# imkaywu/MVSKit

Measured on AMD Instinct MI355X. Metric: patches/s (propagate+optim iteration), 12-view 1080p, higher is better.
Workload: dtype f32

## Files before the change

mvskit_amd/csrc/mvs_engine.cpp:

```cpp
#include <hip/hip_runtime.h>
#include <dlfcn.h>
#include <rccl/rccl.h>

#include <algorithm>
#include <climits>
#include <cmath>
#include <cstdio>
#include <cstdlib>
#include <cstring>
#include <string>
#include <vector>

#include "mvskit_engine.h"
#include "mvs_kernels.h"
#include "mvs_types.h"

static_assert(sizeof(mvs_patch) == sizeof(DPatch), "mvs_patch and DPatch must be the same bytes");
static_assert((MVS_LISTCAP == 16 || MVS_LISTCAP == 32 || MVS_LISTCAP == 64) && MVS_LISTCAP <= MVS_MAXI && MVS_MAX_IMAGES == MVS_MAXI, "limits out of sync");

namespace {
thread_local std::string g_err;

#define HIPCHK(expr)                                                                                       \
    do {                                                                                                   \
        hipError_t _e = (expr);                                                                            \
        if (_e != hipSuccess) {                                                                            \
            g_err = std::string(#expr) + ": " + hipGetErrorString(_e);                                     \
            return MVS_ERR_HIP;                                                                            \
        }                                                                                                  \
    } while (0)

template <typename T> struct DevBuf {
    T* p = nullptr;
    int64_t cap = 0;
    bool headroom = false;
    DevBuf() = default;
    DevBuf(const DevBuf&) = delete;
    DevBuf(DevBuf&& o) noexcept : p(o.p), cap(o.cap), headroom(o.headroom) { o.p = nullptr; o.cap = 0; }
    ~DevBuf() { release(); }
    void swap(DevBuf& o) { std::swap(p, o.p); std::swap(cap, o.cap); }
    int ensure(int64_t n) {
        if (n <= cap) return MVS_OK;
        const int64_t exact = std::max<int64_t>(n, 16);
        int64_t want = (p && headroom) ? exact + exact / 2 : exact;
        T* q = nullptr;
        hipError_t e = hipMalloc((void**)&q, (size_t)want * sizeof(T));
        if (e != hipSuccess && want > exact) { (void)hipGetLastError(); want = exact; e = hipMalloc((void**)&q, (size_t)want * sizeof(T)); }
        if (e != hipSuccess && p) {
            (void)hipGetLastError();
            (void)hipFree(p); p = nullptr; cap = 0;
            e = hipMalloc((void**)&q, (size_t)want * sizeof(T));
        }
        if (e != hipSuccess) { (void)hipGetLastError(); g_err = std::string("hipMalloc: ") + hipGetErrorString(e); return MVS_ERR_HIP; }
        if (p) (void)hipFree(p);
        p = q; cap = want;
        return MVS_OK;
    }
    void release() { if (p) (void)hipFree(p); p = nullptr; cap = 0; }
};

namespace misc {
constexpr int stage_counter = 0;
constexpr int fill_evals = 1;
constexpr int neighbor_retry = 4;
constexpr int sweep_retry = 5;
constexpr int geo_bad = 6;
constexpr int group_edges = 7;
constexpr int trim_parts = 8;
constexpr int trim_nparts = 256;
constexpr int words = trim_parts + trim_nparts;
}
namespace fstat {
constexpr int neighbor_parts = 0;
constexpr int neighbor_cycles = 4096;
constexpr int exact_evals = 4112;
constexpr int words = exact_evals + 2048;
}

struct Rccl {
    void* h = nullptr;
    ncclResult_t (*GetUniqueId)(ncclUniqueId*) = nullptr;
    ncclResult_t (*CommInitRank)(ncclComm_t*, int, ncclUniqueId, int) = nullptr;
    ncclResult_t (*CommDestroy)(ncclComm_t) = nullptr;
    ncclResult_t (*CommCount)(const ncclComm_t, int*) = nullptr;
    ncclResult_t (*CommUserRank)(const ncclComm_t, int*) = nullptr;
    ncclResult_t (*AllGather)(const void*, void*, size_t, ncclDataType_t, ncclComm_t, hipStream_t) = nullptr;
    ncclResult_t (*Broadcast)(const void*, void*, size_t, ncclDataType_t, int, ncclComm_t, hipStream_t) = nullptr;
    ncclResult_t (*GroupStart)() = nullptr;
    ncclResult_t (*GroupEnd)() = nullptr;
    const char* (*GetErrorString)(ncclResult_t) = nullptr;
    bool ok = false;
};
Rccl& rccl() {
    static Rccl r;
    static bool tried = false;
    if (tried) return r;
    tried = true;
    if (const char* over = getenv("MVS_CCL_LIBRARY")) {
        if (*over) { r.h = dlopen(over, RTLD_NOW | RTLD_LOCAL); if (!r.h) return r; }
    }
    const char* names[] = {"librccl.so", "librccl.so.1"};
    for (const char* n : names) if (!r.h) r.h = dlopen(n, RTLD_NOW | RTLD_NOLOAD);
    const char* paths[] = {"/opt/rocm/lib/librccl.so.1", "librccl.so.1", "librccl.so"};
    for (const char* n : paths) if (!r.h) r.h = dlopen(n, RTLD_NOW | RTLD_LOCAL);
    if (!r.h) return r;
#define MVS_SYM(field, name) r.field = reinterpret_cast<decltype(r.field)>(dlsym(r.h, name))
    MVS_SYM(GetUniqueId, "ncclGetUniqueId"); MVS_SYM(CommInitRank, "ncclCommInitRank"); MVS_SYM(CommDestroy, "ncclCommDestroy");
    MVS_SYM(AllGather, "ncclAllGather"); MVS_SYM(Broadcast, "ncclBroadcast"); MVS_SYM(GroupStart, "ncclGroupStart");
    MVS_SYM(GroupEnd, "ncclGroupEnd"); MVS_SYM(GetErrorString, "ncclGetErrorString");
    MVS_SYM(CommCount, "ncclCommCount"); MVS_SYM(CommUserRank, "ncclCommUserRank");
#undef MVS_SYM
    r.ok = r.GetUniqueId && r.CommInitRank && r.CommDestroy && r.AllGather && r.Broadcast && r.GroupStart && r.GroupEnd && r.GetErrorString;
    return r;
}
#define NCCLCHK(expr)                                                                                      \
    do {                                                                                                   \
        ncclResult_t _r = (expr);                                                                          \
        if (_r != ncclSuccess) {                                                                           \
            g_err = std::string(#expr) + ": " + rccl().GetErrorString(_r);                                 \
            return MVS_ERR_HIP;                                                                            \
        }                                                                                                  \
    } while (0)

struct Roctx {
    int (*push)(const char*) = nullptr;
    int (*pop)() = nullptr;
};
Roctx& roctx() {
    static Roctx r;
    static bool tried = false;
    if (tried) return r;
    tried = true;
    void* h = nullptr;
    const char* names[] = {"libroctx64.so", "libroctx64.so.4", "/opt/rocm/lib/libroctx64.so.4"};
    for (const char* n : names) if (!h) h = dlopen(n, RTLD_NOW | RTLD_NOLOAD);
    for (const char* n : names) if (!h) h = dlopen(n, RTLD_NOW | RTLD_LOCAL);
    if (!h) return r;
    r.push = reinterpret_cast<int (*)(const char*)>(dlsym(h, "roctxRangePushA"));
    r.pop = reinterpret_cast<int (*)()>(dlsym(h, "roctxRangePop"));
    if (!r.push || !r.pop) { r.push = nullptr; r.pop = nullptr; }
    return r;
}
struct Range {
    bool on;
    explicit Range(const char* name) : on(roctx().push != nullptr) { if (on) roctx().push(name); }
    ~Range() { if (on) roctx().pop(); }
    Range(const Range&) = delete;
    Range& operator=(const Range&) = delete;
};
}

struct mvs_engine {
    mvs_config cfg{};
    mvs_refiner refiner{MVS_REFINE_HALVING, 500, 1e-4f};
    DParams prm{};
    hipStream_t stream = nullptr;
    bool have_views = false;
    std::vector<DView> hviews;
    DevBuf<DView> dviews;
    std::vector<DevBuf<uint32_t>> img_bufs;
    std::vector<DevBuf<uint8_t>> mask_bufs;
    int total_cells = 0;
    DevBuf<DPatch> pool, pool_alt;
    DevBuf<uint8_t> kill;
    int64_t pool_n = 0;
    bool ncc_dirty = false;
    DevBuf<int32_t> cnt, cursor, vcnt, vcursor;
    DevBuf<csr_off_t> start, vstart;
    DevBuf<csr_off_t> start_raw;
    DevBuf<int32_t> id32_raw;
    DevBuf<int64_t> scan_tmp;
    DevBuf<unsigned long long> ids;
    DevBuf<ListKey> key;
    DevBuf<int32_t> id32, vid32;
    DevBuf<int32_t> uf_parent, uf_size;
    DevBuf<int32_t> group_edges;
    DevBuf<int32_t> cnt_alive, vcnt_alive;
    DevBuf<unsigned long long> dpgrid, best;
    DevBuf<uint32_t> dirty;
    bool dirty_marked = false;
    DevBuf<float4> geo;
    DevBuf<uint8_t> geo_ref;
    bool geo_valid = false;
    bool lists_dense[2] = {false, false};
    DevBuf<DPatch> staging;
    DevBuf<int32_t> job_stage, job_nstage, job_cnt, job_base_scan, kill_cnt, kill_base;
    DevBuf<unsigned long long> misc;
    DevBuf<DCounters> counters;
    DevBuf<int32_t> error_flag;
    DevBuf<int32_t> big_tables, retry_jobs;
    int64_t retried_cells = 0;
    int64_t pass_retried = 0;
    SweepArgs sa{};
    bool staged = false;
    bool counted = false;
    int64_t n_new = 0, n_kill = 0;
    std::vector<int32_t> h_per_view;
    DevBuf<DPatch> tmp_rec_in, tmp_rec_out;
    DevBuf<float> tmp_f_in, tmp_f_out;
    DevBuf<int32_t> tmp_i;
    DevBuf<uint8_t> tmp_bytes;
    hipEvent_t ev[6] = {nullptr, nullptr, nullptr, nullptr, nullptr, nullptr};
    mvs_timing timing{};
    mvs_filter_stats fstats{};
    int64_t fstats_exchange_bytes = 0;
    DevBuf<unsigned long long> fstat_buf;
    hipEvent_t fev[10] = {nullptr, nullptr, nullptr, nullptr, nullptr, nullptr, nullptr, nullptr, nullptr, nullptr};
    ncclComm_t comm = nullptr;
    bool comm_owned = false;
    int comm_rank = 0, comm_world = 1;
    DevBuf<int64_t> comm_counts;
    DevBuf<int32_t> comm_kill_ids;
    int pass_status = MVS_OK;
    std::string pass_error;
    bool fault_fired = false;
};

namespace {

RefineSel refine_sel(const mvs_engine* e) {
    return RefineSel{e->refiner.mode == MVS_REFINE_CONVERGED ? 1 : 0, e->refiner.max_evals, e->refiner.xtol};
}

void derive_params(mvs_engine* e) {
    const mvs_config& c = e->cfg;
    DParams& p = e->prm;
    p.nviews = c.nviews; p.level = c.level; p.csize = c.csize; p.wsize = c.wsize; p.wsz = c.wsize * c.wsize;
    p.minImageNum = c.minImageNum;
    p.tau = std::min(c.minImageNum * 2, c.nviews);
    p.max_propag = c.max_propag;
    p.cap = c.max_propag * c.csize * c.csize;
    p.depth = c.depth; p.enable_check = c.enable_check; p.view_propagation = c.view_propagation ? 1 : 0;
    p.seed = c.seed; p.refine_steps = c.refine_steps; p.rd0 = c.refine_rd0; p.ra0 = c.refine_ra0;
    p.nccThreshold = c.nccThreshold;
    p.nccThresholdBefore = c.nccThreshold - 0.3f;
    volatile float a0 = (float)(60.0f * M_PI / 180.0f), a1 = (float)(60.0f * M_PI / 180.0f);
    volatile double amin = (double)c.maxAngleThreshold, amax = (double)a1;
    volatile float typo = (float)(120.0f / M_PI * 180.0f);
    volatile double d120 = 120.0f * M_PI / 180.0f, d10 = 10.0f * M_PI / 180.0f;
    p.cosAngle0 = cosf(a0);
    p.cosAngle1 = cosf(a1);
    p.cosMinAngle = (float)cos(amin);
    p.cosMaxAngle = (float)cos(amax);
    p.cosNeighborTypo = cosf(typo);
    p.cosNeighbor120 = (float)cos(d120);
    p.sortThreshold = (float)(1.0f - cos(d10));
    p.ascaleConst = (float)(M_PI / 48.0f);
    p.inv_sz = 1.0f / (float)(c.wsize * c.wsize);
    p.inv_3sz = 1.0f / (float)(3 * c.wsize * c.wsize);
    p.neighborThreshold = 0.5f; p.neighborThreshold1 = 1.0f;
    p.quadThreshold = c.quadThreshold;
    p.list_n = std::min<int>(MVS_LISTCAP, c.nviews);
    p.gram_ld = (p.list_n + 15) / 16 * 16;
}

void invert3(const float* P, float* Minv) {
    double a = P[0], b = P[1], c = P[2], d = P[4], e = P[5], f = P[6], g = P[8], h = P[9], i = P[10];
    double A = e * i - f * h, B = -(d * i - f * g), C = d * h - e * g;
    double det = a * A + b * B + c * C;
    double inv[9] = {A, -(b * i - c * h), b * f - c * e, B, a * i - c * g, -(a * f - c * d), C, -(a * h - b * g), a * e - b * d};
    for (int k = 0; k < 9; ++k) Minv[k] = (float)(inv[k] / det);
}
inline float hfma(float a, float b, float c) { return __builtin_fmaf(a, b, c); }
inline float hdot3(const float* a, const float* b) { return hfma(a[2], b[2], hfma(a[1], b[1], a[0] * b[0])); }
inline float hdot4(const float* a, const float* b) { return hfma(a[3], b[3], hfma(a[2], b[2], hfma(a[1], b[1], a[0] * b[0]))); }
inline void hcross(const float* a, const float* b, float* o) {
    o[0] = a[1] * b[2] - a[2] * b[1]; o[1] = a[2] * b[0] - a[0] * b[2]; o[2] = a[0] * b[1] - a[1] * b[0];
}

void setup_camera(const mvs_engine* e, DView& vw, const float* P0) {
    const int maxLevel = e->cfg.level + 3;
    for (int k = 0; k < 12; ++k) vw.P[0][k] = P0[k];
    for (int l = 1; l < maxLevel; ++l) {
        for (int k = 0; k < 12; ++k) vw.P[l][k] = vw.P[l - 1][k];
        for (int k = 0; k < 8; ++k) vw.P[l][k] /= 2.0f;
    }
    invert3(vw.P[e->cfg.level], vw.Minv);
    const float* r2 = &vw.P[0][8];
    const float n = sqrtf(hdot3(r2, r2));
    for (int k = 0; k < 4; ++k) vw.oaxis[k] = r2[k] / n;
    {
        const float* P = vw.P[0];
        double a = P[0], b = P[1], c = P[2], d = P[4], ee = P[5], f = P[6], g = P[8], h = P[9], i = P[10];
        double A = ee * i - f * h, B = -(d * i - f * g), C = d * h - ee * g;
        double det = a * A + b * B + c * C;
        double inv[9] = {A, -(b * i - c * h), b * f - c * ee, B, a * i - c * g, -(a * f - c * d), C, -(a * h - b * g), a * ee - b * d};
        double q[3] = {P[3], P[7], P[11]};
        vw.center[0] = (float)(-(inv[0] * q[0] + inv[1] * q[1] + inv[2] * q[2]) / det);
        vw.center[1] = (float)(-(inv[3] * q[0] + inv[4] * q[1] + inv[5] * q[2]) / det);
        vw.center[2] = (float)(-(inv[6] * q[0] + inv[7] * q[1] + inv[8] * q[2]) / det);
        vw.center[3] = 1.0f;
    }
    for (int k = 0; k < 3; ++k) vw.zaxis[k] = vw.oaxis[k];
    float xa[3] = {vw.P[0][0], vw.P[0][1], vw.P[0][2]};
    hcross(vw.zaxis, xa, vw.yaxis);
    const float yn = sqrtf(hdot3(vw.yaxis, vw.yaxis));
    for (int k = 0; k < 3; ++k) vw.yaxis[k] /= yn;
    hcross(vw.yaxis, vw.zaxis, vw.xaxis);
    const float x4[4] = {vw.xaxis[0], vw.xaxis[1], vw.xaxis[2], 0.0f}, y4[4] = {vw.yaxis[0], vw.yaxis[1], vw.yaxis[2], 0.0f};
    vw.ipscale = hdot4(&vw.P[0][0], x4) + hdot4(&vw.P[0][4], y4);
}

DParams current_params(mvs_engine* e) {
    DParams p = e->prm;
    p.views = e->dviews.p;
    p.pool = e->pool.p;
    p.pool_n = e->pool_n;
    p.total_cells = e->total_cells;
    p.csr_start = e->start.p; p.csr_cnt = e->cnt_alive.p; p.csr_key = e->key.p; p.csr_id32 = e->id32.p;
    p.vcsr_start = e->vstart.p; p.vcsr_cnt = e->vcnt_alive.p; p.vcsr_id32 = e->vid32.p;
    p.dpgrid = e->dpgrid.p;
    p.geo = e->geo_valid ? e->geo.p : nullptr;
    p.geo_ref = e->geo_valid ? e->geo_ref.p : nullptr;
    return p;
}

bool want_vgrid(const mvs_engine* e) { return e->prm.depth >= 2 && e->prm.enable_check; }

int build_list(mvs_engine* e, bool vgrid, bool trim, bool unordered = false) {
    hipStream_t st = e->stream;
    const int64_t nc = e->total_cells;
    DParams p = current_params(e);
    DevBuf<int32_t>& cnt = vgrid ? e->vcnt : e->cnt;
    DevBuf<csr_off_t>& start = vgrid ? e->vstart : e->start;
    DevBuf<int32_t>& cursor = vgrid ? e->vcursor : e->cursor;
    DevBuf<unsigned long long>& ids = e->ids;
    DevBuf<int32_t>& id32 = vgrid ? e->vid32 : e->id32;
    DevBuf<int32_t>& cnt_alive = vgrid ? e->vcnt_alive : e->cnt_alive;
    HIPCHK(hipMemsetAsync(cnt.p, 0, (size_t)(nc + 1) * sizeof(int32_t), st));
    mvsk_index_count(p, vgrid ? nullptr : cnt.p, vgrid ? cnt.p : nullptr, nullptr, st);
    const bool direct = unordered && !trim;
    DevBuf<csr_off_t>& raw = e->start_raw;
    csr_off_t* const first_scan = direct ? start.p : raw.p;
    mvsk_exclusive_scan_off(cnt.p, first_scan, nc, reinterpret_cast<csr_off_t*>(e->scan_tmp.p), st);
    csr_off_t tot64 = 0;
    HIPCHK(hipMemcpyAsync(&tot64, first_scan + nc, sizeof tot64, hipMemcpyDeviceToHost, st));
    HIPCHK(hipStreamSynchronize(st));
    const int64_t tot = (int64_t)tot64;
    if (!unordered) { if (int r = ids.ensure(tot + 16)) return r; }
    if (!vgrid && !unordered) { if (int r = e->key.ensure(tot + 16)) return r; }
    if (int r = id32.ensure(tot + 16)) return r;
    p = current_params(e);
    HIPCHK(hipMemsetAsync(cursor.p, 0, (size_t)(nc + 1) * sizeof(int32_t), st));
    if (direct) {
        mvsk_index_fill_direct(p, vgrid ? 1 : 0, start.p, cursor.p, id32.p, st);
        cnt.swap(cnt_alive);
        e->lists_dense[vgrid ? 1 : 0] = true;
        return MVS_OK;
    }
    if (int r = e->id32_raw.ensure(tot + 16)) return r;
    mvsk_index_fill(p, vgrid ? 1 : 0, raw.p, cursor.p, ids.p, st);
    mvsk_index_sort_trim(p, raw.p, ids.p, trim ? 1 : 0, e->misc.p + misc::trim_parts, st);
    mvsk_index_finalize(p, vgrid ? 1 : 0, raw.p, ids.p, e->id32_raw.p, cnt_alive.p, st);
    mvsk_exclusive_scan_off(cnt_alive.p, start.p, nc, reinterpret_cast<csr_off_t*>(e->scan_tmp.p), st);
    mvsk_index_pack(p, raw.p, start.p, cnt_alive.p, ids.p, e->id32_raw.p, vgrid ? nullptr : e->key.p, id32.p, st);
    e->lists_dense[vgrid ? 1 : 0] = true;
    return MVS_OK;
}
int build_depth(mvs_engine* e) {
    const DParams p = current_params(e);
    HIPCHK(hipMemsetAsync(e->dpgrid.p, 0xff, (size_t)e->total_cells * sizeof(unsigned long long), e->stream));
    mvsk_depth_maps(p, e->dpgrid.p, nullptr, e->stream);
    return MVS_OK;
}
int build_index(mvs_engine* e, unsigned long long* trimmed_out) {
    hipStream_t st = e->stream;
    const DParams p = current_params(e);
    HIPCHK(hipMemsetAsync(e->misc.p + misc::fill_evals, 0, 2 * sizeof(unsigned long long), st));
    HIPCHK(hipMemsetAsync(e->misc.p + misc::trim_parts, 0, misc::trim_nparts * sizeof(unsigned long long), st));
    mvsk_fill_ncc(p, e->misc.p + misc::fill_evals, st);
    e->ncc_dirty = false;
    if (int r = build_list(e, false, true)) return r;
    if (want_vgrid(e)) if (int r = build_list(e, true, false, true)) return r;
    if (int r = build_depth(e)) return r;
    if (trimmed_out) {
        unsigned long long part[misc::trim_nparts];
        HIPCHK(hipMemcpyAsync(part, e->misc.p + misc::trim_parts, sizeof part, hipMemcpyDeviceToHost, st));
        HIPCHK(hipStreamSynchronize(st));
        *trimmed_out = 0;
        for (unsigned long long v : part) *trimmed_out += v;
    }
    HIPCHK(hipGetLastError());
    return MVS_OK;
}
void filter_range(const mvs_engine* e, int64_t& first, int64_t& last) {
    first = 0; last = e->pool_n;
    if (e->comm && e->comm_world > 1) {
        first = e->pool_n * e->comm_rank / e->comm_world;
        last = e->pool_n * (e->comm_rank + 1) / e->comm_world;
    }
}
struct FilterRun {
    mvs_engine* e;
    int local = MVS_OK;
    std::string err;
    int agreed = MVS_OK;
    bool multi() const { return e->comm && e->comm_world > 1; }
    bool live() const { return local == MVS_OK && agreed == MVS_OK; }
    void note(int r) { if (r != MVS_OK && local == MVS_OK) { local = r; err = g_err; } }
};
#define FR(expr) do { if (fr.live()) fr.note(expr); } while (0)
int hip_status(hipError_t e, const char* what) {
    if (e == hipSuccess) return MVS_OK;
    g_err = std::string(what) + ": " + hipGetErrorString(e);
    return MVS_ERR_HIP;
}
#define FRHIP(expr) FR(hip_status((expr), #expr))
#ifdef MVS_FAULT_INJECTION
void filter_fault_point(FilterRun& fr, int point) {
    const char* f = getenv("MVS_FAULT_FILTER");
    int r = -1, p = -1;
    if (f && fr.live() && sscanf(f, "%d:%d", &r, &p) == 2 && r == fr.e->comm_rank && p == point) {
        g_err = "mvs_engine_filter: failure injected by MVS_FAULT_FILTER";
        fr.note(MVS_ERR_CAPACITY);
    }
}
#else
inline void filter_fault_point(FilterRun&, int) {}
#endif
int filter_agree(FilterRun& fr) {
    mvs_engine* e = fr.e;
    if (fr.agreed != MVS_OK) return fr.agreed;
    if (!fr.multi()) {
        if (fr.local != MVS_OK) { fr.agreed = fr.local; g_err = fr.err; }
        return fr.agreed;
    }
    const int64_t mine = fr.local;
    std::vector<int64_t> all((size_t)e->comm_world, 0);
    hipStream_t st = e->stream;
    if (hipMemcpyAsync(e->comm_counts.p, &mine, sizeof mine, hipMemcpyHostToDevice, st) != hipSuccess ||
        rccl().AllGather(e->comm_counts.p, e->comm_counts.p + 1, 1, ncclInt64, e->comm, st) != ncclSuccess ||
        hipMemcpyAsync(all.data(), e->comm_counts.p + 1, all.size() * sizeof(int64_t), hipMemcpyDeviceToHost, st) != hipSuccess ||
        hipStreamSynchronize(st) != hipSuccess) {
        g_err = "mvs_engine_filter: the status all-gather itself failed (the communicator is unusable; the job must be torn down)";
        fr.agreed = MVS_ERR_HIP;
        return fr.agreed;
    }
    for (int r = 0; r < e->comm_world; ++r) {
        if (all[r] == MVS_OK) continue;
        fr.agreed = (int)all[r];
        if (r == e->comm_rank) g_err = fr.err.empty() ? std::string("mvs_engine_filter: this rank failed") : fr.err;
        else g_err = "mvs_engine_filter: rank " + std::to_string(r) + " reported status " + std::to_string((int)all[r]) + "; all ranks give the call up";
        break;
    }
    return fr.agreed;
}
template <typename Blocks> ncclResult_t broadcast_blocks(mvs_engine* e, Blocks&& blocks) {
    const Rccl& R = rccl();
    ncclResult_t first = R.GroupStart();
    for (int r = 0; r < e->comm_world && first == ncclSuccess; ++r)
        blocks(r, [&](void* p, int64_t n, ncclDataType_t type) {
            if (n > 0 && first == ncclSuccess) first = R.Broadcast(p, p, (size_t)n, type, r, e->comm, e->stream);
        });
    const ncclResult_t end = R.GroupEnd();
    return first == ncclSuccess ? end : first;
}
int filter_exchange(FilterRun& fr, bool kills, bool records) {
    mvs_engine* e = fr.e;
    if (!fr.multi()) return filter_agree(fr);
    if (int a = filter_agree(fr)) return a;
    if (e->pool_n == 0) return MVS_OK;
    const int N = e->comm_world;
    const ncclResult_t first_err = broadcast_blocks(e, [&](int r, auto&& send) {
        const int64_t lo = e->pool_n * r / N, hi = e->pool_n * (r + 1) / N;
        if (kills) send(e->kill.p + lo, hi - lo, ncclUint8);
        if (records) send(e->pool.p + lo, (hi - lo) * (int64_t)sizeof(DPatch), ncclUint8);
        e->fstats_exchange_bytes += (r == e->comm_rank) ? 0 : (kills ? (hi - lo) : 0) + (records ? (hi - lo) * (int64_t)sizeof(DPatch) : 0);
    });
    if (first_err != ncclSuccess) {
        g_err = std::string("Filter::run exchange: ") + rccl().GetErrorString(first_err);
        fr.note(MVS_ERR_HIP); fr.agreed = MVS_ERR_HIP;
        return fr.agreed;
    }
    return MVS_OK;
}
int literal_small_groups(mvs_engine* e, int threshold) {
    hipStream_t st = e->stream;
    const DParams p = current_params(e);
    const int cap = 8 << 20;
    if (int r = e->group_edges.ensure(2 * (int64_t)cap)) return r;
    int32_t* nedges = reinterpret_cast<int32_t*>(e->misc.p + misc::group_edges);
    HIPCHK(hipMemsetAsync(nedges, 0, sizeof(unsigned long long), st));
    mvsk_groups_literal_edges(p, e->uf_parent.p, e->uf_size.p, e->group_edges.p, nedges, cap, st);
    int32_t ne = 0;
    HIPCHK(hipMemcpyAsync(&ne, nedges, sizeof ne, hipMemcpyDeviceToHost, st));
    HIPCHK(hipStreamSynchronize(st));
    HIPCHK(hipGetLastError());
    if (ne > cap) { g_err = "Filter::filterSmallGroups (literal labelling): more than 8 M one-way edges between sets"; return MVS_ERR_CAPACITY; }
    if (ne > 0) {
        std::vector<int32_t> pairs(2 * (size_t)ne);
        HIPCHK(hipMemcpy(pairs.data(), e->group_edges.p, pairs.size() * sizeof(int32_t), hipMemcpyDeviceToHost));
        std::vector<int32_t> nodes(pairs);
        std::sort(nodes.begin(), nodes.end());
        nodes.erase(std::unique(nodes.begin(), nodes.end()), nodes.end());
        const size_t nn = nodes.size();
        auto idx = [&](int32_t root) { return (size_t)(std::lower_bound(nodes.begin(), nodes.end(), root) - nodes.begin()); };
        std::vector<int32_t> sizes(nn);
        if (int r = e->tmp_i.ensure((int64_t)2 * nn + 16)) return r;
        HIPCHK(hipMemcpy(e->tmp_i.p, nodes.data(), nn * sizeof(int32_t), hipMemcpyHostToDevice));
        mvsk_gather_i32(e->uf_size.p, e->tmp_i.p, e->tmp_i.p + nn, (int64_t)nn, st);
        HIPCHK(hipMemcpyAsync(sizes.data(), e->tmp_i.p + nn, nn * sizeof(int32_t), hipMemcpyDeviceToHost, st));
        HIPCHK(hipStreamSynchronize(st));
        std::vector<std::vector<uint32_t>> adj(nn);
        for (int32_t k = 0; k < ne; ++k) adj[idx(pairs[2 * k])].push_back((uint32_t)idx(pairs[2 * k + 1]));
        std::vector<int32_t> label(nn, -1), gsize;
        std::vector<uint32_t> queue;
        for (size_t r0 = 0; r0 < nn; ++r0) {
            if (label[r0] != -1) continue;
            const int32_t gid = (int32_t)gsize.size();
            int64_t total = 0;
            queue.assign(1, (uint32_t)r0);
            label[r0] = gid;
            for (size_t qh = 0; qh < queue.size(); ++qh) {
                const uint32_t u = queue[qh];
                total += sizes[u];
                for (uint32_t v : adj[u]) if (label[v] == -1) { label[v] = gid; queue.push_back(v); }
            }
            gsize.push_back((int32_t)std::min<int64_t>(total, INT32_MAX));
        }
        std::vector<int32_t> newsize(nn);
        for (size_t u = 0; u < nn; ++u) newsize[u] = gsize[label[u]];
        HIPCHK(hipMemcpy(e->tmp_i.p + nn, newsize.data(), nn * sizeof(int32_t), hipMemcpyHostToDevice));
        mvsk_scatter_i32(e->uf_size.p, e->tmp_i.p, e->tmp_i.p + nn, (int64_t)nn, st);
    }
    mvsk_groups_kill(p, e->uf_parent.p, e->uf_size.p, threshold, e->kill.p, st);
    return MVS_OK;
}
int rebuild_head(mvs_engine* e, int additive, bool need_pgrid, int incr) {
    if (need_pgrid) { if (int r = build_list(e, false, false, true)) return r; }
    if (incr && e->dirty_marked) mvsk_depth_maps(current_params(e), e->dpgrid.p, e->dirty.p, e->stream);
    else { incr = 0; if (int r = build_depth(e)) return r; }
    e->dirty_marked = false;
    int64_t first, last;
    filter_range(e, first, last);
    mvsk_filter_vimages(current_params(e), additive, first, last, incr == 2 && additive ? e->dirty.p : nullptr, e->stream);
    return MVS_OK;
}
int rebuild_tail(mvs_engine* e, bool need_vpgrid) {
    if (need_vpgrid) { if (int r = build_list(e, true, false, true)) return r; }
    HIPCHK(hipGetLastError());
    return MVS_OK;
}
int pack_geometry(mvs_engine* e) {
    e->geo_valid = false;
    if (e->pool_n <= 0) return MVS_OK;
#ifdef MVS_FAULT_INJECTION
    if (const char* f = getenv("MVS_FAULT_NOPACK")) { if (atoi(f)) return MVS_OK; }
#endif
    if (e->geo.ensure(2 * e->pool_n) != MVS_OK || e->geo_ref.ensure(e->pool_n) != MVS_OK) { (void)hipGetLastError(); return MVS_OK; }
    hipStream_t st = e->stream;
    int32_t* bad = reinterpret_cast<int32_t*>(e->misc.p + misc::geo_bad);
    HIPCHK(hipMemsetAsync(bad, 0, sizeof(unsigned long long), st));
    mvsk_geo_pack(e->pool.p, e->pool_n, e->geo.p, e->geo_ref.p, bad, st);
    int32_t hbad = 1;
    HIPCHK(hipMemcpyAsync(&hbad, bad, sizeof hbad, hipMemcpyDeviceToHost, st));
    HIPCHK(hipStreamSynchronize(st));
    HIPCHK(hipGetLastError());
    e->geo_valid = hbad == 0;
    return MVS_OK;
}
int filter_rebuild(FilterRun& fr, int additive, bool need_pgrid, bool need_vpgrid, int incr = 0) {
    FR(rebuild_head(fr.e, additive, need_pgrid, incr));
    filter_fault_point(fr, 2);
    if (int a = filter_exchange(fr, false, true)) return a;
    FR(rebuild_tail(fr.e, need_vpgrid));
    return MVS_OK;
}
enum class Count { alive, kills, apply_kills };
int count_pool(mvs_engine* e, Count what, int64_t* total) {
    hipStream_t st = e->stream;
    *total = 0;
    if (e->pool_n == 0) return MVS_OK;
    if (what == Count::alive) mvsk_alive_count(e->pool.p, e->pool_n, e->kill_cnt.p, st);
    else mvsk_kill_count(e->kill.p, e->pool_n, e->kill_cnt.p, st);
    mvsk_exclusive_scan(e->kill_cnt.p, e->kill_base.p, e->pool_n, reinterpret_cast<int32_t*>(e->scan_tmp.p), st);
    int32_t n = 0;
    HIPCHK(hipMemcpyAsync(&n, e->kill_base.p + e->pool_n, sizeof n, hipMemcpyDeviceToHost, st));
    if (what == Count::apply_kills) mvsk_apply_kill_flags(e->pool.p, e->kill.p, e->pool_n, st);
    HIPCHK(hipStreamSynchronize(st));
    *total = n;
    return MVS_OK;
}
int apply_kills(mvs_engine* e, int64_t* removed, bool mark = false) {
    hipStream_t st = e->stream;
    *removed = 0;
    e->dirty_marked = false;
    if (e->pool_n == 0) return MVS_OK;
    if (mark) {
        const int64_t words = (e->total_cells + 31) / 32;
        if (int r = e->dirty.ensure(words + 1)) return r;
        HIPCHK(hipMemsetAsync(e->dirty.p, 0, (size_t)words * sizeof(uint32_t), st));
        mvsk_depth_mark_dirty(current_params(e), e->kill.p, e->dpgrid.p, e->dirty.p, st);
        e->dirty_marked = true;
    }
    return count_pool(e, Count::apply_kills, removed);
}

int ensure_counts(mvs_engine* e) {
    if (e->counted) return MVS_OK;
    hipStream_t st = e->stream;
    const int64_t nj = e->sa.njobs;
    e->n_new = 0; e->n_kill = 0;
    e->h_per_view.assign(e->cfg.nviews, 0);
    if (nj > 0) {
        mvsk_commit_count(e->sa, e->job_cnt.p, st);
        mvsk_exclusive_scan(e->job_cnt.p, e->job_base_scan.p, nj, reinterpret_cast<int32_t*>(e->scan_tmp.p), st);
        std::vector<int32_t> bounds(e->sa.nsweep_views + 1);
        for (int s = 0; s < e->sa.nsweep_views; ++s)
            HIPCHK(hipMemcpyAsync(&bounds[s], e->job_base_scan.p + e->sa.job_base[s], sizeof(int32_t), hipMemcpyDeviceToHost, st));
        HIPCHK(hipMemcpyAsync(&bounds[e->sa.nsweep_views], e->job_base_scan.p + nj, sizeof(int32_t), hipMemcpyDeviceToHost, st));
        HIPCHK(hipStreamSynchronize(st));
        e->n_new = bounds[e->sa.nsweep_views];
        for (int s = 0; s < e->sa.nsweep_views; ++s) e->h_per_view[e->sa.sweep_views[s]] = bounds[s + 1] - bounds[s];
    }
    if (int r = count_pool(e, Count::kills, &e->n_kill)) return r;
    e->counted = true;
    return MVS_OK;
}

int compact_pool(mvs_engine* e) {
    int64_t alive = 0;
    if (int r = count_pool(e, Count::alive, &alive)) return r;
    if (alive == e->pool_n) return MVS_OK;
    mvsk_alive_gather(e->pool.p, e->pool_n, e->kill_base.p, e->pool_alt.p, e->pool_alt.cap, e->stream);
    e->pool.swap(e->pool_alt);
    e->pool_n = alive;
    return MVS_OK;
}

template <typename Apply> int commit_pool(mvs_engine* e, Apply&& apply) {
    hipStream_t st = e->stream;
    HIPCHK(hipEventRecord(e->ev[2], st));
    int64_t n_new = 0;
    if (int r = apply(&n_new)) return r;
    e->pool_n += n_new;
    if (int r = compact_pool(e)) return r;
    HIPCHK(hipEventRecord(e->ev[3], st));
    HIPCHK(hipStreamSynchronize(st));
    float ms = 0.0f;
    (void)hipEventElapsedTime(&ms, e->ev[2], e->ev[3]);
    e->timing.commit_ms = ms;
    e->staged = false; e->counted = false;
    return MVS_OK;
}

template <typename C> void add_counters(mvs_counters& a, const C& b) {
    a.candidates += b.candidates; a.prefiltered += b.prefiltered; a.patches += b.patches; a.fail0 += b.fail0; a.fail1 += b.fail1;
    a.inserted += b.inserted; a.replaced += b.replaced; a.evals += b.evals; a.view_evals += b.view_evals; a.trimmed += b.trimmed;
}

}

extern "C" {

const char* mvs_last_error(void) { return g_err.c_str(); }

int mvs_list_cap(void) { return MVS_LISTCAP; }
int mvs_patch_bytes(void) { return (int)sizeof(mvs_patch); }

int mvs_device_count(void) {
    int n = 0;
    if (hipGetDeviceCount(&n) != hipSuccess) return 0;
    return n;
}

void mvs_default_refiner(mvs_refiner* r) {
    if (!r) return;
    r->mode = MVS_REFINE_HALVING; r->max_evals = 500; r->xtol = 1e-4f;
}

int mvs_engine_set_refiner(mvs_engine* e, const mvs_refiner* r) {
    if (!e || !r) { g_err = "mvs_engine_set_refiner: null argument"; return MVS_ERR_ARG; }
    if ((r->mode != MVS_REFINE_HALVING && r->mode != MVS_REFINE_CONVERGED) || r->max_evals < 5 || r->max_evals > 4096 ||
        !std::isfinite(r->xtol) || !(r->xtol > 0.0f)) {
        g_err = "mvs_engine_set_refiner: unknown mode, max_evals outside 5..4096, or xtol not finite and > 0";
        return MVS_ERR_ARG;
    }
    e->refiner = *r;
    return MVS_OK;
}

void mvs_default_config(mvs_config* c) {
    memset(c, 0, sizeof *c);
    c->level = 1; c->csize = 2; c->wsize = 7; c->minImageNum = 3; c->max_propag = 2;
    c->nccThreshold = 0.7f; c->maxAngleThreshold = (float)(10.0f * M_PI / 180.0f); c->quadThreshold = 2.5f;
    c->depth = 1; c->seed = 1; c->refine_steps = 6; c->refine_rd0 = 4.0f; c->refine_ra0 = 4.0f; c->enable_check = 1;
    c->view_begin = 0; c->view_stride = 1; c->device = 0; c->max_patches = 0;
}

int mvs_engine_create(const mvs_config* cfg, mvs_engine** out) {
    if (!cfg || !out) { g_err = "mvs_engine_create: null argument"; return MVS_ERR_ARG; }
    if (cfg->shard_count > 1 && (cfg->shard_index < 0 || cfg->shard_index >= cfg->shard_count)) { g_err = "mvs_engine_create: bad shard_index"; return MVS_ERR_ARG; }
    if (cfg->nviews < 1 || cfg->nviews > MVS_MAXVIEWS || cfg->wsize < 1 || cfg->wsize > 7 || cfg->csize < 1 || cfg->level < 0 ||
        cfg->level > 4 || cfg->max_propag < 1 || cfg->max_propag > 16 || cfg->max_propag * cfg->csize * cfg->csize > MVS_CAPMAX ||
        cfg->view_stride < 1 || cfg->view_begin < 0 || cfg->minImageNum < 1 ||
        std::min(cfg->minImageNum * 2, cfg->nviews) > 16 ) {
        g_err = "mvs_engine_create: configuration out of range (nviews <= 64, wsize <= 7, min(2 minImageNum, nviews) <= 16, max_propag*csize^2 <= 32)";
        return MVS_ERR_ARG;
    }
    int ndev = 0;
    if (hipGetDeviceCount(&ndev) != hipSuccess || ndev < 1) { g_err = "mvs_engine_create: no HIP device (the engine has no CPU path)"; return MVS_ERR_NO_DEVICE; }
    if (cfg->device < 0 || cfg->device >= ndev) { g_err = "mvs_engine_create: bad device ordinal"; return MVS_ERR_ARG; }
    HIPCHK(hipSetDevice(cfg->device));
    mvs_engine* e = new mvs_engine();
    e->cfg = *cfg;
    derive_params(e);
    hipError_t he = hipStreamCreate(&e->stream);
    if (he != hipSuccess) { g_err = std::string("hipStreamCreate: ") + hipGetErrorString(he); delete e; return MVS_ERR_HIP; }
    for (auto& ev : e->ev) (void)hipEventCreate(&ev);
    for (auto& ev : e->fev) (void)hipEventCreate(&ev);
    if (e->misc.ensure(misc::words) || e->counters.ensure(MVS_COUNTER_SLOTS) || e->error_flag.ensure(1)) { delete e; return MVS_ERR_HIP; }
    (void)hipMemset(e->misc.p, 0, misc::words * sizeof(unsigned long long));
    (void)hipMemset(e->error_flag.p, 0, sizeof(int32_t));
    *out = e;
    return MVS_OK;
}

int mvs_engine_destroy(mvs_engine* e) {
    if (!e) return MVS_OK;
    (void)hipSetDevice(e->cfg.device);
    (void)hipStreamSynchronize(e->stream);
    (void)mvs_engine_comm_release(e);
    for (auto& ev : e->ev) if (ev) (void)hipEventDestroy(ev);
    for (auto& ev : e->fev) if (ev) (void)hipEventDestroy(ev);
    (void)hipStreamDestroy(e->stream);
    delete e;
    return MVS_OK;
}

int mvs_engine_set_views(mvs_engine* e, int nviews, const mvs_view_desc* views) {
    if (!e || !views || nviews != e->cfg.nviews) { g_err = "mvs_engine_set_views: nviews must equal the configured number of views"; return MVS_ERR_ARG; }
    HIPCHK(hipSetDevice(e->cfg.device));
    hipStream_t st = e->stream;
    Range rg("mvs:set_views (upload + pyramids)");
    e->img_bufs.clear(); e->mask_bufs.clear();
    e->have_views = false;
    const int maxLevel = e->cfg.level + 3;
    e->hviews.assign(nviews, DView{});
    int cell_base = 0;
    size_t max_bytes = 0;
    for (int v = 0; v < nviews; ++v) {
        if (views[v].width < 8 || views[v].height < 8 || !views[v].rgb) { g_err = "mvs_engine_set_views: bad view"; return MVS_ERR_ARG; }
        max_bytes = std::max(max_bytes, (size_t)views[v].width * views[v].height * 3);
    }
    if (int r = e->tmp_bytes.ensure((int64_t)max_bytes)) return r;
    for (int v = 0; v < nviews; ++v) {
        DView& vw = e->hviews[v];
        vw.W[0] = views[v].width; vw.H[0] = views[v].height;
        for (int l = 1; l < maxLevel; ++l) { vw.W[l] = vw.W[l - 1] / 2; vw.H[l] = vw.H[l - 1] / 2; }
        setup_camera(e, vw, views[v].P);
        const size_t n0 = (size_t)vw.W[0] * vw.H[0];
        HIPCHK(hipMemcpyAsync(e->tmp_bytes.p, views[v].rgb, n0 * 3, hipMemcpyHostToDevice, st));
        for (int l = 0; l < maxLevel; ++l) {
            e->img_bufs.emplace_back();
            if (int r = e->img_bufs.back().ensure(std::max<int64_t>((int64_t)vw.W[l] * vw.H[l], 1))) return r;
            uint32_t* buf = e->img_bufs.back().p;
            vw.img[l] = buf;
            if (l == 0) mvsk_rgb_to_rgba(e->tmp_bytes.p, buf, (int64_t)n0, st);
            else mvsk_pyr_down(vw.img[l - 1], vw.W[l - 1], vw.H[l - 1], buf, vw.W[l], vw.H[l], st);
        }
        vw.mask = nullptr;
        if (views[v].mask) {
            HIPCHK(hipStreamSynchronize(st));
            uint8_t* prev = nullptr;
            for (int l = 0; l <= e->cfg.level; ++l) {
                e->mask_bufs.emplace_back();
                if (int r = e->mask_bufs.back().ensure(std::max<int64_t>((int64_t)vw.W[l] * vw.H[l], 1))) return r;
                uint8_t* m = e->mask_bufs.back().p;
                if (l == 0) {
                    HIPCHK(hipMemcpyAsync(m, views[v].mask, n0, hipMemcpyHostToDevice, st));
                    mvsk_mask_binarise(m, (int64_t)n0, st);
                } else mvsk_mask_down(prev, vw.W[l - 1], vw.H[l - 1], m, vw.W[l], vw.H[l], st);
                prev = m;
            }
            vw.mask = prev;
        }
        HIPCHK(hipStreamSynchronize(st));
        vw.gh = (vw.H[e->cfg.level] + e->cfg.csize - 1) / e->cfg.csize;
        vw.gw = (vw.W[e->cfg.level] + e->cfg.csize - 1) / e->cfg.csize;
        vw.cell_base = cell_base;
        cell_base += vw.gw * vw.gh;
    }
    e->total_cells = cell_base;
    if (int r = e->dviews.ensure(nviews)) return r;
    HIPCHK(hipMemcpyAsync(e->dviews.p, e->hviews.data(), sizeof(DView) * nviews, hipMemcpyHostToDevice, st));
    const int64_t nc = e->total_cells;
    if (e->cnt.ensure(nc + 2) || e->start.ensure(nc + 2) || e->cursor.ensure(nc + 2) || e->vcnt.ensure(nc + 2) || e->vstart.ensure(nc + 2) ||
        e->vcursor.ensure(nc + 2) || e->start_raw.ensure(nc + 2) || e->dpgrid.ensure(nc + 2) || e->best.ensure(nc + 2) || e->cnt_alive.ensure(nc + 2) || e->vcnt_alive.ensure(nc + 2))
        return MVS_ERR_HIP;
    int64_t pool_cap = e->cfg.max_patches > 0 ? e->cfg.max_patches : 4 * nc;
    if (e->cfg.max_patches <= 0) {
        size_t free_b = 0, total_b = 0;
        if (hipMemGetInfo(&free_b, &total_b) == hipSuccess && total_b > 0) {
            pool_cap = std::max<int64_t>(std::min<int64_t>(pool_cap, (int64_t)(total_b / 6 / sizeof(DPatch))), std::min<int64_t>(pool_cap, nc));
            const double per_patch = 2.5 * (double)sizeof(DPatch) + 17.0;
            const int64_t fit = (int64_t)(0.6 * (double)free_b / per_patch);
            if (fit < pool_cap) pool_cap = std::max<int64_t>(fit, std::min<int64_t>(pool_cap, nc / 4 + 1024));
        }
    }
    e->ids.headroom = e->key.headroom = e->id32.headroom = e->id32_raw.headroom = e->vid32.headroom = true;
    e->geo.headroom = e->geo_ref.headroom = true;
    if (e->pool.ensure(pool_cap) || e->pool_alt.ensure(pool_cap) || e->kill.ensure(pool_cap) || e->kill_cnt.ensure(pool_cap + 2) || e->kill_base.ensure(pool_cap + 2)) return MVS_ERR_HIP;
    HIPCHK(hipMemsetAsync(e->kill.p, 0, (size_t)pool_cap, st));
    int64_t njobs_max = 0;
    for (int v = 0; v < nviews; ++v) njobs_max += (int64_t)((e->hviews[v].gw + 1) / 2) * e->hviews[v].gh;
    const int maxstage = (e->prm.view_propagation ? 3 : 2) * e->prm.cap * e->prm.max_propag;
    if (e->job_stage.ensure(njobs_max * maxstage) || e->job_nstage.ensure(njobs_max + 2) || e->job_cnt.ensure(njobs_max + 2) ||
        e->job_base_scan.ensure(njobs_max + 2))
        return MVS_ERR_HIP;
    const int64_t scan_n = std::max<int64_t>(std::max<int64_t>(nc, pool_cap), njobs_max);
    if (e->scan_tmp.ensure(scan_n / 256 + 4096)) return MVS_ERR_HIP;
    if (e->big_tables.ensure((int64_t)256 * 16384) || e->retry_jobs.ensure(std::max<int64_t>(njobs_max, 16))) return MVS_ERR_HIP;
    if (e->uf_parent.ensure(pool_cap) || e->uf_size.ensure(pool_cap) || e->dirty.ensure((nc + 31) / 32 + 1) || e->fstat_buf.ensure(fstat::words)) return MVS_ERR_HIP;
    if (e->staging.ensure(std::max<int64_t>(pool_cap / 2, 1024))) return MVS_ERR_HIP;
    if (e->tmp_rec_out.ensure(16)) return MVS_ERR_HIP;
    HIPCHK(hipStreamSynchronize(st));
    e->pool_n = 0;
    e->have_views = true;
    e->staged = false;
    return MVS_OK;
}

int mvs_engine_grid_dims(mvs_engine* e, int view, int* gw, int* gh) {
    if (!e || !e->have_views || view < 0 || view >= e->cfg.nviews) { g_err = "mvs_engine_grid_dims: bad view / views not set"; return MVS_ERR_STATE; }
    if (gw) *gw = e->hviews[view].gw;
    if (gh) *gh = e->hviews[view].gh;
    return MVS_OK;
}

int mvs_engine_get_pyramid(mvs_engine* e, int view, int level, uint8_t* rgb_out, int* W, int* H) {
    if (!e || !e->have_views || view < 0 || view >= e->cfg.nviews || level < 0 || level >= e->cfg.level + 3) { g_err = "mvs_engine_get_pyramid: bad argument"; return MVS_ERR_ARG; }
    HIPCHK(hipSetDevice(e->cfg.device));
    const DView& vw = e->hviews[view];
    if (W) *W = vw.W[level];
    if (H) *H = vw.H[level];
    if (!rgb_out) return MVS_OK;
    const int64_t n = (int64_t)vw.W[level] * vw.H[level];
    if (int r = e->tmp_bytes.ensure(n * 3)) return r;
    mvsk_rgba_to_rgb(vw.img[level], e->tmp_bytes.p, n, e->stream);
    HIPCHK(hipMemcpyAsync(rgb_out, e->tmp_bytes.p, (size_t)n * 3, hipMemcpyDeviceToHost, e->stream));
    HIPCHK(hipStreamSynchronize(e->stream));
    return MVS_OK;
}

int mvs_engine_set_thresholds(mvs_engine* e, float ncc, float before, int depth) {
    if (!e) return MVS_ERR_ARG;
    e->prm.nccThreshold = ncc; e->prm.nccThresholdBefore = before; e->prm.depth = depth;
    return MVS_OK;
}
int mvs_engine_get_thresholds(mvs_engine* e, float* ncc, float* before, int* depth) {
    if (!e) return MVS_ERR_ARG;
    if (ncc) *ncc = e->prm.nccThreshold;
    if (before) *before = e->prm.nccThresholdBefore;
    if (depth) *depth = e->prm.depth;
    return MVS_OK;
}
int mvs_engine_update_threshold(mvs_engine* e) {
    if (!e) return MVS_ERR_ARG;
    e->prm.nccThreshold -= 0.05f; e->prm.nccThresholdBefore -= 0.05f; ++e->prm.depth;
    return MVS_OK;
}

int mvs_engine_upload_patches(mvs_engine* e, int64_t n, const mvs_patch* patches) {
    if (!e || !e->have_views) { g_err = "mvs_engine_upload_patches: views not set"; return MVS_ERR_STATE; }
    if (n < 0 || (n > 0 && !patches)) return MVS_ERR_ARG;
    if (e->staged) { g_err = "mvs_engine_upload_patches: a pass is waiting for its commit"; return MVS_ERR_STATE; }
    HIPCHK(hipSetDevice(e->cfg.device));
    Range rg("mvs:upload_patches");
    std::vector<mvs_patch> recs;
    recs.reserve((size_t)n);
    for (int64_t i = 0; i < n; ++i) {
        mvs_patch p = patches[i];
        p.nimages = std::min(p.nimages, MVS_LISTCAP);
        if (p.nimages <= 0) continue;
        memset(p.images + p.nimages, 0, sizeof p.images - (size_t)p.nimages);
        p.nvimages = 0;
        memset(p.vimages, 0, sizeof p.vimages);
        p.tmp = std::max(0.0f, p.ncc - e->prm.nccThreshold) * p.nimages;
        p.flags = 1;
        p.id = 0;
        recs.push_back(p);
    }
    if (e->pool_n + (int64_t)recs.size() > e->pool.cap) { g_err = "mvs_engine_upload_patches: patch pool capacity exceeded (raise mvs_config.max_patches)"; return MVS_ERR_CAPACITY; }
    if (!recs.empty()) HIPCHK(hipMemcpyAsync(e->pool.p + e->pool_n, recs.data(), recs.size() * sizeof(mvs_patch), hipMemcpyHostToDevice, e->stream));
    HIPCHK(hipStreamSynchronize(e->stream));
    e->pool_n += (int64_t)recs.size();
    e->ncc_dirty = true;
    return MVS_OK;
}

namespace {
SeedCam seed_camera(const float* P) {
    SeedCam c;
    const double m[9] = {P[0], P[1], P[2], P[4], P[5], P[6], P[8], P[9], P[10]};
    const double det = m[0] * (m[4] * m[8] - m[5] * m[7]) - m[1] * (m[3] * m[8] - m[5] * m[6]) + m[2] * (m[3] * m[7] - m[4] * m[6]);
    const double inv[9] = {(m[4] * m[8] - m[5] * m[7]) / det, (m[2] * m[7] - m[1] * m[8]) / det, (m[1] * m[5] - m[2] * m[4]) / det,
                           (m[5] * m[6] - m[3] * m[8]) / det, (m[0] * m[8] - m[2] * m[6]) / det, (m[2] * m[3] - m[0] * m[5]) / det,
                           (m[3] * m[7] - m[4] * m[6]) / det, (m[1] * m[6] - m[0] * m[7]) / det, (m[0] * m[4] - m[1] * m[3]) / det};
    const double q[3] = {P[3], P[7], P[11]};
    for (int r = 0; r < 3; ++r) c.center[r] = (float)-(inv[3 * r] * q[0] + inv[3 * r + 1] * q[1] + inv[3 * r + 2] * q[2]);
    c.center[3] = 1.0f;
    const float on = sqrtf(P[8] * P[8] + P[9] * P[9] + P[10] * P[10]);
    const float z[3] = {P[8] / on, P[9] / on, P[10] / on};
    float x[3] = {P[0], P[1], P[2]};
    float y[3] = {z[1] * x[2] - z[2] * x[1], z[2] * x[0] - z[0] * x[2], z[0] * x[1] - z[1] * x[0]};
    const float yn = sqrtf(y[0] * y[0] + y[1] * y[1] + y[2] * y[2]);
    for (int k = 0; k < 3; ++k) y[k] /= yn;
    x[0] = y[1] * z[2] - y[2] * z[1]; x[1] = y[2] * z[0] - y[0] * z[2]; x[2] = y[0] * z[1] - y[1] * z[0];
    c.ipscale = (P[0] * x[0] + P[1] * x[1] + P[2] * x[2]) + (P[4] * y[0] + P[5] * y[1] + P[6] * y[2]);
    return c;
}
}

int mvs_engine_seed_patches(mvs_engine* e, int64_t npoints, const float* xyz, const mvs_seed_view* views, int64_t* n_added) {
    if (npoints < 0 || (npoints > 0 && !xyz) || !views) { g_err = "mvs_engine_seed_patches: negative npoints, or xyz / views null"; return MVS_ERR_ARG; }
    if (npoints > (int64_t)INT32_MAX - 4096) { g_err = "mvs_engine_seed_patches: more than 2^31 - 4097 points in one call"; return MVS_ERR_ARG; }
    if (!e) { g_err = "mvs_engine_seed_patches: no engine"; return MVS_ERR_ARG; }
    if (!e->have_views) { g_err = "mvs_engine_seed_patches: views not set"; return MVS_ERR_STATE; }
    if (e->staged) { g_err = "mvs_engine_seed_patches: a pass is waiting for its commit"; return MVS_ERR_STATE; }
    if (n_added) *n_added = 0;
    if (npoints == 0) return MVS_OK;
    HIPCHK(hipSetDevice(e->cfg.device));
    Range rg("mvs:seed_patches");
    hipStream_t st = e->stream;
    const int nviews = e->cfg.nviews;
    const int64_t n = npoints;
    int64_t max_pix = 0;
    for (int v = 0; v < nviews; ++v)
        if (views[v].normals && views[v].mask) max_pix = std::max(max_pix, (int64_t)e->hviews[v].W[0] * e->hviews[v].H[0]);
    DevBuf<float> d_xyz, d_sum, d_map;
    DevBuf<unsigned long long> d_bits;
    DevBuf<int32_t> d_keep, d_base, d_scan;
    DevBuf<uint8_t> d_mask;
    DevBuf<SeedCam> d_cams;
    if (d_xyz.ensure(3 * n) || d_sum.ensure(3 * n) || d_bits.ensure(n) || d_keep.ensure(n + 1) || d_base.ensure(n + 1) || d_scan.ensure(n / 256 + 4096) ||
        d_cams.ensure(nviews) || (max_pix > 0 && (d_map.ensure(3 * max_pix) || d_mask.ensure(max_pix))))
        return MVS_ERR_HIP;
    std::vector<SeedCam> cams((size_t)nviews);
    for (int v = 0; v < nviews; ++v) cams[(size_t)v] = seed_camera(e->hviews[v].P[0]);
    HIPCHK(hipMemcpyAsync(d_cams.p, cams.data(), sizeof(SeedCam) * (size_t)nviews, hipMemcpyHostToDevice, st));
    HIPCHK(hipMemcpyAsync(d_xyz.p, xyz, sizeof(float) * 3 * (size_t)n, hipMemcpyHostToDevice, st));
    HIPCHK(hipMemsetAsync(d_sum.p, 0, sizeof(float) * 3 * (size_t)n, st));
    HIPCHK(hipMemsetAsync(d_bits.p, 0, sizeof(unsigned long long) * (size_t)n, st));
    for (int v = 0; v < nviews; ++v) {
        if (!views[v].normals || !views[v].mask) continue;
        const DView& vw = e->hviews[v];
        const size_t pix = (size_t)vw.W[0] * vw.H[0];
        SeedView sv;
        memcpy(sv.P, vw.P[0], sizeof sv.P);
        sv.W = vw.W[0]; sv.H = vw.H[0]; sv.view = v;
        HIPCHK(hipMemcpyAsync(d_map.p, views[v].normals, sizeof(float) * 3 * pix, hipMemcpyHostToDevice, st));
        HIPCHK(hipMemcpyAsync(d_mask.p, views[v].mask, pix, hipMemcpyHostToDevice, st));
        mvsk_seed_accumulate(sv, d_map.p, d_mask.p, d_xyz.p, n, d_sum.p, d_bits.p, st);
        HIPCHK(hipStreamSynchronize(st));
    }
    mvsk_seed_flags(d_cams.p, e->cfg.level, d_xyz.p, d_sum.p, d_bits.p, n, d_keep.p, st);
    mvsk_exclusive_scan(d_keep.p, d_base.p, n, d_scan.p, st);
    int32_t total = 0;
    HIPCHK(hipMemcpyAsync(&total, d_base.p + n, sizeof total, hipMemcpyDeviceToHost, st));
    HIPCHK(hipStreamSynchronize(st));
    HIPCHK(hipGetLastError());
    if (e->pool_n + (int64_t)total > e->pool.cap) { g_err = "mvs_engine_seed_patches: patch pool capacity exceeded (raise mvs_config.max_patches)"; return MVS_ERR_CAPACITY; }
    if (total > 0) {
        volatile float deg10 = 10.0f * (float)M_PI / 180.0f;
        const float thr = 1.0f - cosf(deg10);
        const float tmp_unit = std::max(0.0f, -1.0f - e->prm.nccThreshold);
        mvsk_seed_emit(d_cams.p, nviews, e->cfg.level, thr, tmp_unit, d_xyz.p, d_sum.p, d_bits.p, d_keep.p, d_base.p, n, e->pool.p + e->pool_n, st);
        HIPCHK(hipStreamSynchronize(st));
        HIPCHK(hipGetLastError());
        e->pool_n += (int64_t)total;
        e->ncc_dirty = true;
    }
    if (n_added) *n_added = (int64_t)total;
    return MVS_OK;
}

int mvs_engine_reserve(mvs_engine* e, int64_t list_entries) {
    if (!e || !e->have_views || list_entries < 0) { g_err = "mvs_engine_reserve: views not set, or a negative size"; return MVS_ERR_ARG; }
    HIPCHK(hipSetDevice(e->cfg.device));
    int64_t n = list_entries > 0 ? list_entries : e->total_cells * (int64_t)(e->cfg.max_propag * e->cfg.csize * e->cfg.csize);
    auto take = [&](auto& buf, int64_t want) -> int {
        const int64_t before = buf.cap;
        if (int r = buf.ensure(want)) return r;
        if (buf.cap != before && hipMemsetAsync(buf.p, 0, (size_t)buf.cap * sizeof(*buf.p), e->stream) != hipSuccess) { (void)hipGetLastError(); return MVS_ERR_HIP; }
        return MVS_OK;
    };
    if (take(e->ids, n + 16) || take(e->key, n + 16) || take(e->id32, n + 16) || take(e->id32_raw, n + 16) || take(e->vid32, n + 16)) return MVS_ERR_HIP;
    HIPCHK(hipStreamSynchronize(e->stream));
    return MVS_OK;
}

int mvs_engine_clear_patches(mvs_engine* e) {
    if (!e) return MVS_ERR_ARG;
    HIPCHK(hipSetDevice(e->cfg.device));
    if (e->kill.p) HIPCHK(hipMemsetAsync(e->kill.p, 0, (size_t)e->kill.cap, e->stream));
    e->pool_n = 0; e->staged = false; e->counted = false;
    return MVS_OK;
}

int mvs_engine_num_patches(mvs_engine* e, int64_t* n_alive) {
    if (!e || !n_alive) return MVS_ERR_ARG;
    HIPCHK(hipSetDevice(e->cfg.device));
    return count_pool(e, Count::alive, n_alive);
}

int mvs_engine_download_patches(mvs_engine* e, int64_t cap, mvs_patch* out, int64_t* n) {
    if (!e || !n) return MVS_ERR_ARG;
    int64_t alive = 0;
    if (int r = mvs_engine_num_patches(e, &alive)) return r;
    *n = alive;
    if (!out || alive == 0) return MVS_OK;
    const int64_t m = std::min(cap, alive);
    if (int r = e->tmp_rec_out.ensure(alive)) return r;
    mvsk_alive_gather(e->pool.p, e->pool_n, e->kill_base.p, e->tmp_rec_out.p, alive, e->stream);
    HIPCHK(hipMemcpyAsync(out, e->tmp_rec_out.p, (size_t)m * sizeof(mvs_patch), hipMemcpyDeviceToHost, e->stream));
    HIPCHK(hipStreamSynchronize(e->stream));
    return MVS_OK;
}

#define PLY_CHUNK ((int64_t)1 << 20)
#define PLY_ASCII_LINE_MAX 90
static void ply_header(int64_t n, bool ascii, std::string* out) {
    char head[512];
    snprintf(head, sizeof head,
             "ply\nformat %s 1.0\nelement vertex %lld\nproperty float x\nproperty float y\nproperty float z\nproperty float nx\n"
             "property float ny\nproperty float nz\nproperty uchar diffuse_red\nproperty uchar diffuse_green\nproperty uchar diffuse_blue\n"
             "end_header\n",
             ascii ? "ascii" : "binary_little_endian", (long long)n);
    *out = head;
}
struct PlyBufs {
    DevBuf<int32_t> idx, len;
    DevBuf<int64_t> off;
    DevBuf<uint32_t> rgb;
    DevBuf<uint8_t> bytes;
};

int mvs_engine_export_ply(mvs_engine* e, int format, int64_t cap, uint8_t* out, int64_t* nbytes) {
    if (format != MVS_PLY_ASCII && format != MVS_PLY_BINARY_LE) { g_err = "mvs_engine_export_ply: format must be MVS_PLY_ASCII or MVS_PLY_BINARY_LE"; return MVS_ERR_ARG; }
    if (!nbytes || cap < 0) { g_err = "mvs_engine_export_ply: nbytes is null or cap negative"; return MVS_ERR_ARG; }
    if (!e) { g_err = "mvs_engine_export_ply: no engine"; return MVS_ERR_ARG; }
    if (!e->have_views) { g_err = "mvs_engine_export_ply: views not set"; return MVS_ERR_STATE; }
    if (e->staged) { g_err = "mvs_engine_export_ply: a pass is waiting for its commit"; return MVS_ERR_STATE; }
    HIPCHK(hipSetDevice(e->cfg.device));
    Range rg("mvs:export_ply");
    hipStream_t st = e->stream;
    const bool ascii = format == MVS_PLY_ASCII;
    int64_t alive = 0;
    if (int r = mvs_engine_num_patches(e, &alive)) return r;
    std::string head;
    ply_header(alive, ascii, &head);
    const int64_t chunk = std::min<int64_t>(PLY_CHUNK, std::max<int64_t>(e->pool_n, 1));
    PlyBufs b;
    if (alive > 0 && (b.idx.ensure(chunk) || b.rgb.ensure(chunk) || (ascii && (b.len.ensure(chunk + 1) || b.off.ensure(chunk + 1))))) return MVS_ERR_HIP;
    auto measure = [&](int64_t i0, int64_t i1, int64_t* nv, int64_t* cb) -> int {
        int32_t ends[2] = {0, 0};
        HIPCHK(hipMemcpyAsync(&ends[0], e->kill_base.p + i0, sizeof(int32_t), hipMemcpyDeviceToHost, st));
        HIPCHK(hipMemcpyAsync(&ends[1], e->kill_base.p + i1, sizeof(int32_t), hipMemcpyDeviceToHost, st));
        HIPCHK(hipStreamSynchronize(st));
        *nv = ends[1] - ends[0];
        *cb = 27 * *nv;
        if (*nv == 0) return MVS_OK;
        mvsk_ply_select(e->pool.p, e->kill_base.p, i0, i1, b.idx.p, st);
        mvsk_ply_colour(e->pool.p, b.idx.p, *nv, e->dviews.p, e->cfg.nviews, e->cfg.level, ascii ? 1 : 0, b.rgb.p, b.len.p, st);
        if (!ascii) return MVS_OK;
        mvsk_exclusive_scan_off(b.len.p, b.off.p, *nv, reinterpret_cast<csr_off_t*>(e->scan_tmp.p), st);
        HIPCHK(hipMemcpyAsync(cb, b.off.p + *nv, sizeof(int64_t), hipMemcpyDeviceToHost, st));
        HIPCHK(hipStreamSynchronize(st));
        return MVS_OK;
    };
    const int64_t upper = (int64_t)head.size() + (ascii ? PLY_ASCII_LINE_MAX : 27) * alive;
    if (!out || cap < upper) {
        int64_t total = (int64_t)head.size() + 27 * alive;
        if (ascii) {
            total = (int64_t)head.size();
            for (int64_t i0 = 0; i0 < e->pool_n; i0 += chunk) {
                int64_t nv = 0, cb = 0;
                if (int r = measure(i0, std::min(e->pool_n, i0 + chunk), &nv, &cb)) return r;
                total += cb;
            }
        }
        *nbytes = total;
        if (!out) return MVS_OK;
        if (cap < total) { g_err = "mvs_engine_export_ply: cap is smaller than the file (*nbytes)"; return MVS_ERR_CAPACITY; }
    }
    if (alive > 0 && b.bytes.ensure(chunk * (ascii ? PLY_ASCII_LINE_MAX : 27))) return MVS_ERR_HIP;
    memcpy(out, head.data(), head.size());
    int64_t pos = (int64_t)head.size();
    for (int64_t i0 = 0; i0 < e->pool_n; i0 += chunk) {
        int64_t nv = 0, cb = 0;
        if (int r = measure(i0, std::min(e->pool_n, i0 + chunk), &nv, &cb)) return r;
        if (nv == 0) continue;
        if (pos + cb > cap || cb > b.bytes.cap) { g_err = "mvs_engine_export_ply: a chunk outgrew its bound"; return MVS_ERR_CAPACITY; }
        mvsk_ply_emit(e->pool.p, b.idx.p, nv, b.rgb.p, ascii ? b.off.p : nullptr, b.bytes.p, st);
        HIPCHK(hipMemcpyAsync(out + pos, b.bytes.p, (size_t)cb, hipMemcpyDeviceToHost, st));
        HIPCHK(hipStreamSynchronize(st));
        pos += cb;
    }
    *nbytes = pos;
    return MVS_OK;
}

static int pass_impl(mvs_engine* e, int iter, int pass, mvs_counters* out);
int mvs_engine_pass(mvs_engine* e, int iter, int pass, mvs_counters* out) {
    const int r = pass_impl(e, iter, pass, out);
    if (e) { e->pass_status = r; e->pass_error = r ? g_err : std::string(); }
    return r;
}
static void discard_pass(mvs_engine* e) {
    if (e->kill.p && e->pool_n > 0) (void)hipMemsetAsync(e->kill.p, 0, (size_t)e->pool_n, e->stream);
    (void)hipStreamSynchronize(e->stream);
    e->staged = false; e->counted = false;
}
static int pass_impl(mvs_engine* e, int iter, int pass, mvs_counters* out) {
    if (!e || !e->have_views) { g_err = "mvs_engine_pass: views not set"; return MVS_ERR_STATE; }
    if (e->staged) { g_err = "mvs_engine_pass: the previous pass was not committed"; return MVS_ERR_STATE; }
    HIPCHK(hipSetDevice(e->cfg.device));
    hipStream_t st = e->stream;
    HIPCHK(hipEventRecord(e->ev[0], st));
    unsigned long long trimmed = 0;
    {
        Range rg("mvs:index");
        if (int r = build_index(e, &trimmed)) return r;
    }
    HIPCHK(hipEventRecord(e->ev[1], st));
    Range rg_sweep(pass & 1 ? "mvs:sweep colour 1" : "mvs:sweep colour 0");
    SweepArgs& a = e->sa;
    memset(&a, 0, sizeof a);
    a.iter = iter; a.inc = (iter % 2 == 0) ? 1 : -1; a.colour = pass & 1;
    int64_t nj = 0;
    const bool ranged = e->cfg.shard_count > 1;
    for (int v = ranged ? 0 : e->cfg.view_begin; v < e->cfg.nviews; v += ranged ? 1 : e->cfg.view_stride) {
        a.sweep_views[a.nsweep_views] = v;
        a.job_base[a.nsweep_views] = (int32_t)nj;
        ++a.nsweep_views;
        nj += (int64_t)((e->hviews[v].gw + 1) / 2) * e->hviews[v].gh;
    }
    a.njobs = nj;
    a.job_lo = 0; a.job_hi = nj;
    if (ranged) {
        const int split_mode = getenv("MVS_SPLIT_PROXY") ? atoi(getenv("MVS_SPLIT_PROXY")) : 2;
        const int N = e->cfg.shard_count, R = e->cfg.shard_index;
        std::vector<int32_t> cuts(N + 1, -1);
        int64_t total_work = 0;
        if (split_mode > 0 && nj > 0) {
            const DParams p0 = current_params(e);
            int shift = 0;
            while ((((int64_t)3 * e->prm.cap * e->prm.max_propag * 32 * nj) >> shift) + nj >= (int64_t)INT32_MAX) ++shift;
            mvsk_job_work(p0, a, split_mode, shift, e->job_cnt.p, st);
            mvsk_exclusive_scan(e->job_cnt.p, e->job_base_scan.p, nj, reinterpret_cast<int32_t*>(e->scan_tmp.p), st);
            if (int r = e->tmp_i.ensure(N + 1)) return r;
            HIPCHK(hipMemsetAsync(e->tmp_i.p, 0xff, (size_t)(N + 1) * sizeof(int32_t), st));
            mvsk_job_cuts(e->job_base_scan.p, nj, N, e->tmp_i.p, st);
            int32_t tw = 0;
            HIPCHK(hipMemcpyAsync(cuts.data(), e->tmp_i.p, (size_t)(N + 1) * sizeof(int32_t), hipMemcpyDeviceToHost, st));
            HIPCHK(hipMemcpyAsync(&tw, e->job_base_scan.p + nj, sizeof tw, hipMemcpyDeviceToHost, st));
            HIPCHK(hipStreamSynchronize(st));
            total_work = tw;
        }
        cuts[0] = 0; cuts[N] = (int32_t)nj;
        for (int r = 1; r < N; ++r) {
            if (total_work <= 0 || cuts[r] < 0) cuts[r] = (int32_t)(nj * r / N);
            cuts[r] = std::max(cuts[r], cuts[r - 1]);
        }
        a.job_lo = cuts[R];
        a.job_hi = cuts[R + 1];
        HIPCHK(hipMemsetAsync(e->job_nstage.p, 0, (size_t)nj * sizeof(int32_t), st));
    }
    a.staging = e->staging.p; a.staging_cap = e->staging.cap;
    a.stage_counter = e->misc.p + misc::stage_counter;
    a.job_stage = e->job_stage.p; a.job_nstage = e->job_nstage.p;
    a.maxstage = (e->prm.view_propagation ? 3 : 2) * e->prm.cap * e->prm.max_propag;
    a.kill = e->kill.p;
    a.counters = e->counters.p;
    a.error_flag = e->error_flag.p;
    if (want_vgrid(e)) {
        if (int r = e->big_tables.ensure((int64_t)256 * 16384)) return r;
        if (int r = e->retry_jobs.ensure(std::max<int64_t>(nj, 16))) return r;
    }
    a.big_tables = e->big_tables.p; a.retry_jobs = e->retry_jobs.p; a.nretry = reinterpret_cast<int32_t*>(e->misc.p + misc::sweep_retry);
    HIPCHK(hipMemsetAsync(e->misc.p + misc::sweep_retry, 0, sizeof(unsigned long long), st));
    HIPCHK(hipMemsetAsync(e->misc.p + misc::stage_counter, 0, sizeof(unsigned long long), st));
    HIPCHK(hipMemsetAsync(e->counters.p, 0, MVS_COUNTER_SLOTS * sizeof(DCounters), st));
    HIPCHK(hipMemsetAsync(e->error_flag.p, 0, sizeof(int32_t), st));
    const DParams p = current_params(e);
    const RefineSel rs = refine_sel(e);
    mvsk_sweep(p, a, rs, st);
    e->pass_retried = 0;
    if (want_vgrid(e)) {
        int32_t nretry = 0;
        HIPCHK(hipMemcpyAsync(&nretry, a.nretry, sizeof nretry, hipMemcpyDeviceToHost, st));
        HIPCHK(hipStreamSynchronize(st));
        e->pass_retried = nretry;
        if (nretry > 0) { mvsk_sweep_retry(p, a, nretry, rs, st); e->retried_cells += nretry; }
    }
    HIPCHK(hipEventRecord(e->ev[2], st));
    std::vector<DCounters> hcs(MVS_COUNTER_SLOTS);
    int32_t herr = 0;
    unsigned long long fill[2] = {0, 0};
    HIPCHK(hipMemcpyAsync(fill, e->misc.p + misc::fill_evals, sizeof fill, hipMemcpyDeviceToHost, st));
    HIPCHK(hipMemcpyAsync(hcs.data(), e->counters.p, hcs.size() * sizeof(DCounters), hipMemcpyDeviceToHost, st));
    HIPCHK(hipMemcpyAsync(&herr, e->error_flag.p, sizeof herr, hipMemcpyDeviceToHost, st));
    HIPCHK(hipStreamSynchronize(st));
    HIPCHK(hipGetLastError());
    mvs_counters sum{};
    for (const DCounters& c : hcs) add_counters(sum, c);
    sum.evals += fill[0]; sum.view_evals += fill[1]; sum.trimmed = (int64_t)trimmed;
    float ms = 0.0f;
    (void)hipEventElapsedTime(&ms, e->ev[0], e->ev[1]); e->timing.index_ms = ms;
    (void)hipEventElapsedTime(&ms, e->ev[1], e->ev[2]); e->timing.sweep_ms = ms;
    e->timing.commit_ms = 0.0f; e->timing.sweep_launches = 1; e->timing.exchange_ms = 0.0f; e->timing.exchange_bytes = 0;
    e->timing.check_retried_cells = e->pass_retried;
    e->staged = true; e->counted = false;
    if (out) *out = sum;
#ifdef MVS_STAGE_TIMING
    {
        unsigned long long stage[16] = {0};
        for (const DCounters& c : hcs)
            for (int k = 0; k < 16; ++k) stage[k] = (k == 12 || k == 13) ? std::max(stage[k], c.stage[k]) : stage[k] + c.stage[k];
        static const char* nm[8] = {"wave", "generate", "pre", "refine", "post", "check", "stage", "prologue"};
        fprintf(stderr, "[stage cycles]");
        for (int k = 0; k < 8; ++k) fprintf(stderr, " %s %.1f%%", nm[k], 100.0 * (double)stage[k] / (double)(stage[0] ? stage[0] : 1));
        static const char* nm2[4] = {"gain", "search", "sort", "quad"};
        for (int k = 0; k < 4; ++k) fprintf(stderr, " %s %.1f%%", nm2[k], 100.0 * (double)stage[8 + k] / (double)(stage[0] ? stage[0] : 1));
        fprintf(stderr, " setRefImage pairs %.1f%% choice %.1f%%", 100.0 * (double)stage[14] / (double)(stage[0] ? stage[0] : 1), 100.0 * (double)stage[15] / (double)(stage[0] ? stage[0] : 1));
        fprintf(stderr, "  (wave cycles %.3e; max visited %llu, max neighbours %llu)\n", (double)stage[0], stage[12], stage[13]);
    }
#endif
#ifdef MVS_FAULT_INJECTION
    if (const char* f = getenv("MVS_FAULT_PASS")) {
        int fr = -1, fi = -1, fp = -1;
        if (!e->fault_fired && sscanf(f, "%d:%d:%d", &fr, &fi, &fp) == 3 && fr == (e->cfg.shard_count > 1 ? e->cfg.shard_index : 0) && fi == iter && fp == pass) {
            e->fault_fired = true;
            g_err = "mvs_engine_pass: capacity failure injected by MVS_FAULT_PASS";
            return MVS_ERR_CAPACITY;
        }
    }
#endif
    if (herr & 3) { g_err = "mvs_engine_pass: staging capacity exceeded (raise mvs_config.max_patches)"; return MVS_ERR_CAPACITY; }
    if (herr & 4) {
        g_err = "mvs_engine_pass: Optim::check met more than 14336 patches around one patch, or more than 4064 neighbours (engine limit)";
        return MVS_ERR_CAPACITY;
    }
    return MVS_OK;
}

int mvs_engine_export_counts(mvs_engine* e, int64_t* n_new, int64_t* n_kill, int32_t* per_view_new) {
    if (!e || !e->staged) { g_err = "mvs_engine_export_counts: no pass to export"; return MVS_ERR_STATE; }
    HIPCHK(hipSetDevice(e->cfg.device));
    if (int r = ensure_counts(e)) return r;
    if (n_new) *n_new = e->n_new;
    if (n_kill) *n_kill = e->n_kill;
    if (per_view_new) for (int v = 0; v < e->cfg.nviews; ++v) per_view_new[v] = e->h_per_view[v];
    return MVS_OK;
}

int mvs_engine_export_device(mvs_engine* e, void* d_new, int64_t cap_new, void* d_kill, int64_t cap_kill) {
    if (!e || !e->staged) { g_err = "mvs_engine_export_device: no pass to export"; return MVS_ERR_STATE; }
    HIPCHK(hipSetDevice(e->cfg.device));
    if (int r = ensure_counts(e)) return r;
    if (e->n_new > cap_new || e->n_kill > cap_kill) { g_err = "mvs_engine_export_device: buffers too small"; return MVS_ERR_CAPACITY; }
    if (e->n_new > 0) mvsk_commit_copy(e->sa, e->job_base_scan.p, (DPatch*)d_new, cap_new, nullptr, 1, e->stream);
    if (e->n_kill > 0) mvsk_kill_export(e->kill.p, e->pool_n, e->kill_base.p, (int32_t*)d_kill, cap_kill, e->stream);
    HIPCHK(hipStreamSynchronize(e->stream));
    return MVS_OK;
}

int mvs_engine_commit_device(mvs_engine* e, const void* d_new, int64_t n_new, const void* d_kill, int64_t n_kill) {
    if (!e || !e->have_views) return MVS_ERR_STATE;
    HIPCHK(hipSetDevice(e->cfg.device));
    hipStream_t st = e->stream;
    if (e->pool_n + n_new > e->pool.cap) { g_err = "mvs_engine_commit_device: patch pool capacity exceeded (raise mvs_config.max_patches)"; return MVS_ERR_CAPACITY; }
    return commit_pool(e, [&](int64_t* added) -> int {
        mvsk_apply_kill_ids(e->pool.p, (const int32_t*)d_kill, n_kill, e->pool_n, st);
        mvsk_append_records(e->pool.p, e->pool_n, (const DPatch*)d_new, n_new, st);
        if (e->pool_n > 0) HIPCHK(hipMemsetAsync(e->kill.p, 0, (size_t)e->pool_n, st));
        *added = n_new;
        return MVS_OK;
    });
}

int mvs_engine_commit_local(mvs_engine* e) {
    if (!e || !e->staged) { g_err = "mvs_engine_commit_local: no pass to commit"; return MVS_ERR_STATE; }
    HIPCHK(hipSetDevice(e->cfg.device));
    hipStream_t st = e->stream;
    Range rg("mvs:commit");
    return commit_pool(e, [&](int64_t* added) -> int {
        if (int r = ensure_counts(e)) return r;
        if (e->pool_n + e->n_new > e->pool.cap) { g_err = "mvs_engine_commit_local: patch pool capacity exceeded (raise mvs_config.max_patches)"; return MVS_ERR_CAPACITY; }
        if (e->n_new > 0) mvsk_commit_copy(e->sa, e->job_base_scan.p, e->pool.p + e->pool_n, e->pool.cap - e->pool_n, nullptr, 0, st);
// ... 395 lines not shown
```

mvskit_amd/csrc/mvs_kernels.h:

```cpp
#pragma once
#include <hip/hip_runtime.h>
#include "mvs_types.h"

void mvsk_rgb_to_rgba(const uint8_t* rgb, uint32_t* out, int64_t n, hipStream_t st);
void mvsk_rgba_to_rgb(const uint32_t* in, uint8_t* rgb, int64_t n, hipStream_t st);
void mvsk_pyr_down(const uint32_t* src, int pw, int ph, uint32_t* dst, int w, int h, hipStream_t st);
void mvsk_mask_down(const uint8_t* src, int pw, int ph, uint8_t* dst, int w, int h, hipStream_t st);
void mvsk_mask_binarise(uint8_t* m, int64_t n, hipStream_t st);
void mvsk_exclusive_scan(const int32_t* in, int32_t* out, int64_t n, int32_t* tmp, hipStream_t st);
void mvsk_index_count(const DParams& prm, int32_t* cnt, int32_t* vcnt, unsigned long long* total, hipStream_t st);
void mvsk_exclusive_scan_off(const int32_t* in, csr_off_t* out, int64_t n, csr_off_t* tmp, hipStream_t st);
void mvsk_index_fill(const DParams& prm, int vgrid, const csr_off_t* start, int32_t* cursor, unsigned long long* ids, hipStream_t st);
void mvsk_index_fill_direct(const DParams& prm, int vgrid, const csr_off_t* start, int32_t* cursor, int32_t* id32, hipStream_t st);
void mvsk_index_sort_trim(const DParams& prm, const csr_off_t* start, unsigned long long* ids, int do_trim, unsigned long long* trimmed, hipStream_t st);
void mvsk_index_finalize(const DParams& prm, int vgrid, const csr_off_t* start, unsigned long long* ids, int32_t* id32, int32_t* cnt_alive, hipStream_t st);
void mvsk_index_pack(const DParams& prm, const csr_off_t* start, const csr_off_t* start2, const int32_t* cnt_alive, const unsigned long long* ids, const int32_t* id32_in,
                     ListKey* key, int32_t* id32_out, hipStream_t st);
void mvsk_depth_maps(const DParams& prm, unsigned long long* dp, const uint32_t* dirty, hipStream_t st);
void mvsk_depth_mark_dirty(const DParams& prm, const uint8_t* kill, unsigned long long* dp, uint32_t* dirty, hipStream_t st);
void mvsk_best_ncc_map(const DParams& prm, int view, unsigned long long* best, hipStream_t st);
void mvsk_map_extract(const DParams& prm, int view, int kind, const unsigned long long* sel, float* depth, float* normal, int32_t* ids, int ncells, hipStream_t st);
void mvsk_fill_ncc(const DParams& prm, unsigned long long* evals, hipStream_t st);
struct RefineSel { int simplex; int max_evals; float xtol; };
size_t mvsk_sweep_lds_bytes(const DParams& prm);
void mvsk_sweep(const DParams& prm, const SweepArgs& a, const RefineSel& rs, hipStream_t st);
void mvsk_sweep_retry(const DParams& prm, const SweepArgs& a, int nretry, const RefineSel& rs, hipStream_t st);
void mvsk_job_work(const DParams& prm, const SweepArgs& a, int mode, int shift, int32_t* work, hipStream_t st);
void mvsk_job_cuts(const int32_t* scan, int64_t njobs, int n, int32_t* cuts, hipStream_t st);
void mvsk_commit_count(const SweepArgs& a, int32_t* cnt, hipStream_t st);
void mvsk_commit_copy(const SweepArgs& a, const int32_t* base, DPatch* dst, int64_t dst_cap, int32_t* per_view, int keep_key, hipStream_t st);
void mvsk_kill_count(const uint8_t* kill, int64_t n, int32_t* cnt, hipStream_t st);
void mvsk_kill_export(const uint8_t* kill, int64_t n, const int32_t* base, int32_t* ids, int64_t cap, hipStream_t st);
void mvsk_apply_kill_flags(DPatch* pool, uint8_t* kill, int64_t n, hipStream_t st);
void mvsk_apply_kill_ids(DPatch* pool, const int32_t* ids, int64_t n, int64_t pool_n, hipStream_t st);
void mvsk_append_records(DPatch* pool, int64_t pool_n, const DPatch* recs, int64_t n, hipStream_t st);
void mvsk_alive_count(const DPatch* pool, int64_t n, int32_t* cnt, hipStream_t st);
void mvsk_alive_gather(const DPatch* pool, int64_t n, const int32_t* base, DPatch* out, int64_t cap, hipStream_t st);
void mvsk_filter_vimages(const DParams& prm, int additive, int64_t first, int64_t last, const uint32_t* dirty, hipStream_t st);
void mvsk_geo_pack(const DPatch* pool, int64_t n, float4* geo, uint8_t* ref, int* bad, hipStream_t st);
void mvsk_filter_outside(const DParams& prm, uint8_t* kill, int64_t first, int64_t last, hipStream_t st);
void mvsk_filter_exact(const DParams& prm, uint8_t* kill, unsigned long long* evals, unsigned long long* stage, int64_t first, int64_t last, hipStream_t st);
void mvsk_filter_neighbor(const DParams& prm, uint8_t* kill, int32_t* retry, int32_t* nretry, int32_t* overflow, unsigned long long* stats, int64_t first, int64_t last, hipStream_t st);
void mvsk_filter_neighbor_retry(const DParams& prm, uint8_t* kill, const int32_t* todo, int32_t ntodo, int32_t* overflow, unsigned long long* stats, hipStream_t st);
void mvsk_groups(const DParams& prm, int* parent, int* size, int threshold, uint8_t* kill, hipStream_t st);
void mvsk_groups_literal_edges(const DParams& prm, int* parent, int* size, int* edges2, int* nedges, int cap, hipStream_t st);
void mvsk_gather_i32(const int32_t* src, const int32_t* idx, int32_t* out, int64_t n, hipStream_t st);
void mvsk_scatter_i32(int32_t* dst, const int32_t* idx, const int32_t* val, int64_t n, hipStream_t st);
void mvsk_groups_kill(const DParams& prm, const int* parent, const int* size, int threshold, uint8_t* kill, hipStream_t st);
void mvsk_probe(const DParams& prm, int op, int64_t n, const DPatch* in, const float* in_f, DPatch* out, float* out_f, int32_t* out_i, const RefineSel& rs,
                hipStream_t st);
void mvsk_ply_select(const DPatch* pool, const int32_t* base, int64_t i0, int64_t i1, int32_t* idx, hipStream_t st);
void mvsk_ply_colour(const DPatch* pool, const int32_t* idx, int64_t n, const DView* views, int nviews, int level, int ascii, uint32_t* rgb, int32_t* len,
                     hipStream_t st);
void mvsk_ply_emit(const DPatch* pool, const int32_t* idx, int64_t n, const uint32_t* rgb, const int64_t* off, uint8_t* out, hipStream_t st);
struct SeedView { float P[12]; int32_t W, H, view; };
struct SeedCam { float center[4]; float ipscale; };
void mvsk_seed_accumulate(const SeedView& sv, const float* map, const uint8_t* mask, const float* xyz, int64_t n, float* sum, unsigned long long* bits,
                          hipStream_t st);
void mvsk_seed_flags(const SeedCam* cams, int level, const float* xyz, const float* sum, const unsigned long long* bits, int64_t n, int32_t* keep,
                     hipStream_t st);
void mvsk_seed_emit(const SeedCam* cams, int nviews, int level, float thr, float tmp_unit, const float* xyz, const float* sum, const unsigned long long* bits,
                    const int32_t* keep, const int32_t* base, int64_t n, DPatch* dst, hipStream_t st);
```

mvskit_amd/csrc/mvs_kernels.hip:

```cpp
#include <hip/hip_runtime.h>
#include <algorithm>
#include "mvs_device.cuh"
#include "mvs_check.cuh"
#include "mvs_kernels.h"

using namespace mvsdev;

__global__ void k_rgb_to_rgba(const uint8_t* __restrict__ rgb, uint32_t* __restrict__ out, int64_t n) {
    const int64_t i = (int64_t)blockIdx.x * blockDim.x + threadIdx.x;
    if (i >= n) return;
    const uint8_t* p = rgb + 3 * i;
    out[i] = (uint32_t)p[0] | ((uint32_t)p[1] << 8) | ((uint32_t)p[2] << 16);
}
__global__ void k_rgba_to_rgb(const uint32_t* __restrict__ in, uint8_t* __restrict__ rgb, int64_t n) {
    const int64_t i = (int64_t)blockIdx.x * blockDim.x + threadIdx.x;
    if (i >= n) return;
    const uint32_t t = in[i];
    rgb[3 * i] = t & 255u; rgb[3 * i + 1] = (t >> 8) & 255u; rgb[3 * i + 2] = (t >> 16) & 255u;
}
__global__ void k_pyr_down(const uint32_t* __restrict__ src, int pw, int ph, uint32_t* __restrict__ dst, int w, int h) {
    const int x = blockIdx.x * blockDim.x + threadIdx.x, y = blockIdx.y * blockDim.y + threadIdx.y;
    if (x >= w || y >= h) return;
    const float base[4] = {1.0f, 3.0f, 3.0f, 1.0f};
    float c0 = 0.0f, c1 = 0.0f, c2 = 0.0f;
    for (int i = -1; i < 3; ++i) {
        const int yt = 2 * y + i;
        if (yt < 0 || ph - 1 < yt) continue;
        for (int j = -1; j < 3; ++j) {
            const int xt = 2 * x + j;
            if (xt < 0 || pw - 1 < xt) continue;
            const float m = (base[i + 1] * base[j + 1]) / 64.0f;
            const uint32_t t = src[(size_t)yt * pw + xt];
            c0 += m * (float)(t & 255u); c1 += m * (float)((t >> 8) & 255u); c2 += m * (float)((t >> 16) & 255u);
        }
    }
    const uint32_t r = (uint8_t)((int)floorf(c0 + 0.5f)), g = (uint8_t)((int)floorf(c1 + 0.5f)), b = (uint8_t)((int)floorf(c2 + 0.5f));
    dst[(size_t)y * w + x] = r | (g << 8) | (b << 16);
}
__global__ void k_mask_down(const uint8_t* __restrict__ src, int pw, int ph, uint8_t* __restrict__ dst, int w, int h) {
    const int x = blockIdx.x * blockDim.x + threadIdx.x, y = blockIdx.y * blockDim.y + threadIdx.y;
    if (x >= w || y >= h) return;
    const int ys[2] = {2 * y, min(ph - 1, 2 * y + 1)}, xs[2] = {2 * x, min(pw - 1, 2 * x + 1)};
    int inside = 0;
    for (int j = 0; j < 2; ++j) for (int i = 0; i < 2; ++i) inside += src[(size_t)ys[j] * pw + xs[i]] ? 1 : 0;
    dst[(size_t)y * w + x] = inside > 0 ? 255 : 0;
}
__global__ void k_mask_binarise(uint8_t* m, int64_t n) {
    const int64_t i = (int64_t)blockIdx.x * blockDim.x + threadIdx.x;
    if (i < n) m[i] = m[i] > 127 ? 255 : 0;
}

#define SCAN_BLOCK 256
#define SCAN_ITEMS 4
template <typename TI, typename TO>
__global__ void k_scan_block(const TI* __restrict__ in, TO* __restrict__ out, TO* __restrict__ block_sums, int64_t n_in) {
    __shared__ TO s[SCAN_BLOCK];
    const int64_t base = ((int64_t)blockIdx.x * SCAN_BLOCK + threadIdx.x) * SCAN_ITEMS;
    TO v[SCAN_ITEMS], sum = 0;
    for (int k = 0; k < SCAN_ITEMS; ++k) { v[k] = (base + k < n_in) ? (TO)in[base + k] : (TO)0; sum += v[k]; }
    s[threadIdx.x] = sum;
    __syncthreads();
    for (int off = 1; off < SCAN_BLOCK; off <<= 1) {
        TO t = (threadIdx.x >= (unsigned)off) ? s[threadIdx.x - off] : (TO)0;
        __syncthreads();
        s[threadIdx.x] += t;
        __syncthreads();
    }
    TO excl = s[threadIdx.x] - sum;
    for (int k = 0; k < SCAN_ITEMS; ++k) { if (base + k <= n_in) out[base + k] = excl; excl += v[k]; }
    if (threadIdx.x == SCAN_BLOCK - 1) block_sums[blockIdx.x] = s[threadIdx.x];
}
template <typename TO>
__global__ void k_scan_add(TO* __restrict__ out, const TO* __restrict__ block_offsets, int64_t n_out) {
    const int64_t base = ((int64_t)blockIdx.x * SCAN_BLOCK + threadIdx.x) * SCAN_ITEMS;
    const TO o = block_offsets[blockIdx.x];
    for (int k = 0; k < SCAN_ITEMS; ++k) if (base + k < n_out) out[base + k] += o;
}
template <typename TI, typename TO>
void launch_exclusive_scan(const TI* in, TO* out, int64_t n, TO* tmp, hipStream_t st) {
    const int64_t per = (int64_t)SCAN_BLOCK * SCAN_ITEMS;
    const int64_t nb = (n + 1 + per - 1) / per;
    hipLaunchKernelGGL((k_scan_block<TI, TO>), dim3((unsigned)nb), dim3(SCAN_BLOCK), 0, st, in, out, tmp, n);
    if (nb > 1) {
        TO* tmp2 = tmp + nb + 1;
        launch_exclusive_scan<TO, TO>(tmp, tmp, nb, tmp2, st);
        hipLaunchKernelGGL((k_scan_add<TO>), dim3((unsigned)nb), dim3(SCAN_BLOCK), 0, st, out, tmp, n + 1);
    }
}

DEV uint32_t sortable_f32(float f) {
    uint32_t u = __float_as_uint(f);
    return (u & 0x80000000u) ? ~u : (u | 0x80000000u);
}
__device__ __forceinline__ unsigned long long list_key(float ncc, int64_t id) {
    return ((unsigned long long)(~sortable_f32(ncc + 0.0f)) << 32) | (unsigned long long)(uint32_t)id;
}
DEV int pgrid_id(const DParams& prm, csr_off_t pos) {
    return prm.csr_id32[pos];
}
DEV float pgrid_ncc(const DParams& prm, csr_off_t pos) {
    return prm.csr_key[pos].ncc;
}
DEV int pgrid_ref(const DParams& prm, csr_off_t pos) {
    return prm.csr_key[pos].ref;
}
__global__ void k_index_count(DParams prm, int32_t* __restrict__ cnt, int32_t* __restrict__ vcnt, unsigned long long* __restrict__ total) {
    const int64_t id = (int64_t)blockIdx.x * blockDim.x + threadIdx.x;
    int mine = 0;
    if (id < prm.pool_n && (prm.pool[id].flags & 1)) {
        const DPatch* p = prm.pool + id;
        const F4 coord = ld4(p->coord);
        const int n = cnt ? min(p->nimages, MVS_LISTCAP) : 0;
        for (int i = 0; i < n; ++i) {
            const DView* vw = prm.views + p->images[i];
            int ix, iy;
            cell_of(prm, vw, coord, ix, iy);
            if (ix < 0 || vw->gw <= ix || iy < 0 || vw->gh <= iy) continue;
            atomicAdd(&cnt[vw->cell_base + iy * vw->gw + ix], 1);
            ++mine;
        }
        if (vcnt) {
            const int nv = min(p->nvimages, MVS_LISTCAP);
            for (int i = 0; i < nv; ++i) {
                const DView* vw = prm.views + p->vimages[i];
                int ix, iy;
                cell_of(prm, vw, coord, ix, iy);
                if (ix < 0 || vw->gw <= ix || iy < 0 || vw->gh <= iy) continue;
                atomicAdd(&vcnt[vw->cell_base + iy * vw->gw + ix], 1);
                ++mine;
            }
        }
    }
    for (int d = 32; d >= 1; d >>= 1) mine += __shfl_xor(mine, d);
    if (total && (threadIdx.x & 63) == 0 && mine) atomicAdd(total, (unsigned long long)mine);
}
__global__ void k_index_fill(DParams prm, int vgrid, const csr_off_t* __restrict__ start, int32_t* __restrict__ cursor, unsigned long long* __restrict__ ids) {
    const int64_t id = (int64_t)blockIdx.x * blockDim.x + threadIdx.x;
    if (id >= prm.pool_n) return;
    const DPatch* p = prm.pool + id;
    if (!(p->flags & 1)) return;
    const F4 coord = ld4(p->coord);
    const unsigned long long key = list_key(p->ncc, id);
    const int n = vgrid ? min(p->nvimages, MVS_LISTCAP) : min(p->nimages, MVS_LISTCAP);
    for (int i = 0; i < n; ++i) {
        const DView* vw = prm.views + (vgrid ? p->vimages[i] : p->images[i]);
        int ix, iy;
        cell_of(prm, vw, coord, ix, iy);
        if (ix < 0 || vw->gw <= ix || iy < 0 || vw->gh <= iy) continue;
        const int g = vw->cell_base + iy * vw->gw + ix;
        ids[start[g] + atomicAdd(&cursor[g], 1)] = key;
    }
}
__global__ void k_index_fill_direct(DParams prm, int vgrid, const csr_off_t* __restrict__ start, int32_t* __restrict__ cursor, int32_t* __restrict__ id32) {
    const int64_t id = (int64_t)blockIdx.x * blockDim.x + threadIdx.x;
    if (id >= prm.pool_n) return;
    const DPatch* p = prm.pool + id;
    if (!(p->flags & 1)) return;
    const F4 coord = ld4(p->coord);
    const int n = vgrid ? min(p->nvimages, MVS_LISTCAP) : min(p->nimages, MVS_LISTCAP);
    for (int i = 0; i < n; ++i) {
        const DView* vw = prm.views + (vgrid ? p->vimages[i] : p->images[i]);
        int ix, iy;
        cell_of(prm, vw, coord, ix, iy);
        if (ix < 0 || vw->gw <= ix || iy < 0 || vw->gh <= iy) continue;
        const int g = vw->cell_base + iy * vw->gw + ix;
        const csr_off_t slot = start[g] + atomicAdd(&cursor[g], 1);
        id32[slot] = (int32_t)id;
    }
}
__global__ void k_index_sort_trim(DParams prm, const csr_off_t* __restrict__ start, unsigned long long* __restrict__ ids, int do_trim,
                                  unsigned long long* __restrict__ trimmed) {
    const int g = blockIdx.x * blockDim.x + threadIdx.x;
    const bool in = g < prm.total_cells;
    const csr_off_t b = in ? start[g] : 0, e = in ? start[g + 1] : 0;
    for (csr_off_t i = b + 1; i < e; ++i) {
        const unsigned long long k = ids[i];
        csr_off_t j = i - 1;
        while (j >= b) {
            const unsigned long long o = ids[j];
            if (o < k) break;
            ids[j + 1] = o;
            --j;
        }
        ids[j + 1] = k;
    }
    if (do_trim) {
        int mine = 0;
        for (csr_off_t k = b + prm.cap; k < e; ++k) {
            const int old = atomicAnd(&prm.pool[(uint32_t)ids[k]].flags, ~1);
            mine += old & 1;
        }
        for (int d = 32; d >= 1; d >>= 1) mine += __shfl_xor(mine, d);
        if ((threadIdx.x & 63) == 0 && mine) atomicAdd(trimmed + (blockIdx.x & 255u), (unsigned long long)mine);
    }
}
__global__ void k_index_finalize(DParams prm, int vgrid, const csr_off_t* __restrict__ start, unsigned long long* __restrict__ ids,
                                 int32_t* __restrict__ id32, int32_t* __restrict__ cnt_alive) {
    const int g = blockIdx.x * blockDim.x + threadIdx.x;
    if (g >= prm.total_cells) return;
    const csr_off_t b = start[g], e = start[g + 1];
    int n = 0;
    for (csr_off_t k = b; k < e; ++k) {
        const int id = (int)(uint32_t)ids[k];
        const DPatch* p = prm.pool + id;
        if (!(p->flags & 1)) continue;
        if (!vgrid) ids[b + n] = ((unsigned long long)(uint32_t)p->images[0] << 32) | (unsigned long long)__float_as_uint(p->ncc);
        id32[b + n] = id;
        ++n;
    }
    cnt_alive[g] = n;
}
__global__ void k_index_pack(DParams prm, const csr_off_t* __restrict__ start, const csr_off_t* __restrict__ start2, const int32_t* __restrict__ cnt_alive,
                             const unsigned long long* __restrict__ ids, const int32_t* __restrict__ id32_in, ListKey* __restrict__ key, int32_t* __restrict__ id32_out) {
    const int g = blockIdx.x * blockDim.x + threadIdx.x;
    if (g >= prm.total_cells) return;
    const csr_off_t b = start[g], b2 = start2[g];
    const int n = cnt_alive[g];
    for (int k = 0; k < n; ++k) {
        id32_out[b2 + k] = id32_in[b + k];
        if (key) {
            const unsigned long long w = ids[b + k];
            ListKey lk;
            lk.ncc = __uint_as_float((uint32_t)w); lk.ref = (int32_t)(w >> 32);
            key[b2 + k] = lk;
        }
    }
}
__global__ __launch_bounds__(256) void k_depth_maps(DParams prm, unsigned long long* __restrict__ dp, const uint32_t* __restrict__ dirty) {
    const int64_t id = (int64_t)blockIdx.x * 64 + (threadIdx.x & 63u);
    if (id >= prm.pool_n) return;
    const DPatch* p = prm.pool + id;
    if (!(p->flags & 1)) return;
    const F4 coord = ld4(p->coord);
    for (int image = (int)(threadIdx.x >> 6); image < prm.nviews; image += 4) {
        const DView* vw = prm.views + image;
        const F3 ic = project(vw, coord, prm.level);
        const float fx = ic.x / (float)prm.csize, fy = ic.y / (float)prm.csize;
        const int xs[2] = {(int)floorf(fx), (int)ceilf(fx)}, ys[2] = {(int)floorf(fy), (int)ceilf(fy)};
        const float depth = dot4(ld4(vw->oaxis), coord);
        const unsigned long long key = ((unsigned long long)sortable_f32(depth) << 32) | (unsigned long long)(uint32_t)id;
        for (int j = 0; j < 2; ++j) for (int i = 0; i < 2; ++i) {
            if (xs[i] < 0 || vw->gw <= xs[i] || ys[j] < 0 || vw->gh <= ys[j]) continue;
            if (i == 1 && xs[1] == xs[0]) continue;
            if (j == 1 && ys[1] == ys[0]) continue;
            const int cell = vw->cell_base + ys[j] * vw->gw + xs[i];
            if (dirty && !((dirty[cell >> 5] >> (cell & 31)) & 1u)) continue;
            unsigned long long* cellp = &dp[cell];
            if (key < __builtin_nontemporal_load(cellp)) atomicMin(cellp, key);
        }
    }
}
__global__ __launch_bounds__(256) void k_depth_mark_dirty(DParams prm, const uint8_t* __restrict__ kill, unsigned long long* __restrict__ dp, uint32_t* __restrict__ dirty) {
    const int64_t id = (int64_t)blockIdx.x * 64 + (threadIdx.x & 63u);
    if (id >= prm.pool_n || !kill[id]) return;
    const DPatch* p = prm.pool + id;
    if (!(p->flags & 1)) return;
    const F4 coord = ld4(p->coord);
    for (int image = (int)(threadIdx.x >> 6); image < prm.nviews; image += 4) {
        const DView* vw = prm.views + image;
        const F3 ic = project(vw, coord, prm.level);
        const float fx = ic.x / (float)prm.csize, fy = ic.y / (float)prm.csize;
        const int xs[2] = {(int)floorf(fx), (int)ceilf(fx)}, ys[2] = {(int)floorf(fy), (int)ceilf(fy)};
        for (int j = 0; j < 2; ++j) for (int i = 0; i < 2; ++i) {
            if (xs[i] < 0 || vw->gw <= xs[i] || ys[j] < 0 || vw->gh <= ys[j]) continue;
            if (i == 1 && xs[1] == xs[0]) continue;
            if (j == 1 && ys[1] == ys[0]) continue;
            const int cell = vw->cell_base + ys[j] * vw->gw + xs[i];
            if ((uint32_t)(dp[cell] & 0xffffffffull) != (uint32_t)id) continue;
            dp[cell] = ~0ull;
            atomicOr(&dirty[cell >> 5], 1u << (cell & 31));
        }
    }
}
__global__ void k_best_ncc_map(DParams prm, int view, unsigned long long* __restrict__ best) {
    const int64_t id = (int64_t)blockIdx.x * blockDim.x + threadIdx.x;
    if (id >= prm.pool_n) return;
    const DPatch* p = prm.pool + id;
    if (!(p->flags & 1) || p->nimages == 0 || p->images[0] != view) return;
    const DView* vw = prm.views + view;
    int ix, iy;
    cell_of(prm, vw, ld4(p->coord), ix, iy);
    if (ix < 0 || vw->gw <= ix || iy < 0 || vw->gh <= iy) return;
    const unsigned long long key = ((unsigned long long)sortable_f32(p->ncc) << 32) | (unsigned long long)(0xffffffffu - (uint32_t)id);
    atomicMax(&best[iy * vw->gw + ix], key);
}
__global__ void k_map_extract(DParams prm, int view, int kind, const unsigned long long* __restrict__ sel, float* __restrict__ depth,
                              float* __restrict__ normal, int32_t* __restrict__ ids, int ncells) {
    const int c = blockIdx.x * blockDim.x + threadIdx.x;
    if (c >= ncells) return;
    const unsigned long long k = sel[c];
    const bool empty = kind == 0 ? (k == ~0ull) : (k == 0ull);
    if (empty) {
        depth[c] = __int_as_float(0x7fc00000);
        normal[3 * c] = normal[3 * c + 1] = normal[3 * c + 2] = __int_as_float(0x7fc00000);
        ids[c] = -1;
        return;
    }
    const uint32_t id = kind == 0 ? (uint32_t)(k & 0xffffffffull) : 0xffffffffu - (uint32_t)(k & 0xffffffffull);
    const DPatch* p = prm.pool + id;
    depth[c] = dot4(ld4((prm.views + view)->oaxis), ld4(p->coord));
    normal[3 * c] = p->normal[0]; normal[3 * c + 1] = p->normal[1]; normal[3 * c + 2] = p->normal[2];
    ids[c] = (int32_t)id;
}

__global__ __launch_bounds__(64) void k_fill_ncc(DParams prm, unsigned long long* evals) {
    WaveCtx wc = make_wave_ctx(prm);
    const int64_t mine = (int64_t)blockIdx.x * 64 + wc.lane;
    bool need = false;
    if (mine < prm.pool_n) need = (prm.pool[mine].flags & 1) && (prm.pool[mine].ncc < 0.0f);
    unsigned long long todo = ballot(need);
    while (todo) {
        const int l = __ffsll((long long)todo) - 1;
        todo &= todo - 1ull;
        DPatch* p = prm.pool + ((int64_t)blockIdx.x * 64 + l);
        Cand c;
        load_cand(p, wc, c);
        const float ncc = compute_ncc(prm, wc, c.coord, c.normal, c.img, c.nimg);
        if (wc.lane == 0) p->ncc = ncc;
    }
    if (wc.lane == 0 && wc.evals) { atomicAdd(evals, (unsigned long long)wc.evals); atomicAdd(evals + 1, (unsigned long long)wc.view_evals); }
}

DEV bool rank_before(float na, int a, float nb, int b) { return (na != nb) ? (na > nb) : (a < b); }
DEV void job_cell(const DParams& prm, const SweepArgs& a, int64_t job, int& v, int& cx, int& cy) {
    int s = 0;
    while (s + 1 < a.nsweep_views && job >= a.job_base[s + 1]) ++s;
    v = a.sweep_views[s];
    const int gw = (prm.views + v)->gw, halfw = (gw + 1) / 2;
    const int local = (int)(job - a.job_base[s]);
    cy = local / halfw;
    cx = 2 * (local % halfw) + ((a.colour + cy) & 1);
}
__global__ void k_job_work(DParams prm, SweepArgs a, int mode, int shift, int32_t* __restrict__ work) {
    const int64_t job = (int64_t)blockIdx.x * blockDim.x + threadIdx.x;
    if (job >= a.njobs) return;
    int v, cx, cy;
    job_cell(prm, a, job, v, cx, cy);
    const DView* vw = prm.views + v;
    const int gw = vw->gw, gh = vw->gh;
    int w = 0;
    if (cx < gw && cy < gh) {
        const int sxs[3] = {cx, cx - a.inc, cx}, sys[3] = {cy - a.inc, cy, cy};
        const int nsrc = prm.view_propagation ? 3 : 2;
        int n = 0;
        for (int k = 0; k < nsrc; ++k) {
            if (sxs[k] < 0 || gw <= sxs[k] || sys[k] < 0 || gh <= sys[k]) continue;
            const int g = vw->cell_base + sys[k] * gw + sxs[k];
            const csr_off_t sb = prm.csr_start[g];
            const int sn = prm.csr_cnt[g];
            for (int j = 0; j < sn; ++j) n += ((pgrid_ref(prm, sb + j) == v) != (k == 2)) ? 1 : 0;
        }
        if (mode == 1) w = n;
        else {
            const int trials = n * prm.max_propag;
            const int room = max(prm.cap - prm.csr_cnt[vw->cell_base + cy * gw + cx], 0);
            const int full = min(trials, (room * 5 + 3) / 4);
            w = 32 * full + 2 * (trials - full);
        }
    }
    work[job] = (w + (1 << shift) - 1) >> shift;
}
__global__ void k_job_cuts(const int32_t* __restrict__ scan, int64_t njobs, int n, int32_t* __restrict__ cuts) {
    const int64_t job = (int64_t)blockIdx.x * blockDim.x + threadIdx.x;
    if (job >= njobs) return;
    const long long total = scan[njobs], p0 = scan[job], p1 = scan[job + 1];
    if (p0 == p1) return;
    for (int r = 1; r < n; ++r) {
        const long long target = total * r / n;
        if (p0 <= target && target < p1) cuts[r] = (int32_t)job;
    }
}

#ifndef MVS_SWEEP_WAVES
#define MVS_SWEEP_WAVES 3
#endif
#ifdef MVS_STAGE_TIMING
#define ST_NOW() ((unsigned long long)__builtin_amdgcn_s_memtime())
#define ST_ADD(k, t0) { const unsigned long long t1_ = ST_NOW(); st_acc[k] += t1_ - (t0); (t0) = t1_; }
#else
#define ST_ADD(k, t0)
#endif
#ifndef MVS_XCD_CHUNK
#define MVS_XCD_CHUNK 128
#endif
template <bool BIG, bool SIMPLEX = false>
DEV void sweep_cell(const DParams& prm, const SweepArgs& a, const int64_t job, int* s_scratch, float* s_texs, int* big_table,
                    int max_evals = 0, float xtol = 0.0f) {
#ifdef MVS_STAGE_TIMING
    unsigned long long st_acc[16] = {0, 0, 0, 0, 0, 0, 0, 0, 0, 0, 0, 0, 0, 0, 0, 0};
    const unsigned long long st_begin = ST_NOW();
    unsigned long long st_t = st_begin;
#endif
    int v, cx, cy;
    job_cell(prm, a, job, v, cx, cy);
    const DView* vw = prm.views + v;
    const int gw = vw->gw, gh = vw->gh;
    WaveCtx wc = make_wave_ctx(prm);
    if (wc.lane == 0) a.job_nstage[job] = 0;
    if (cx >= gw || cy >= gh) return;
    const int cell = cy * gw + cx;
    const int inc = a.inc;
    const int sxs[2] = {cx, cx - inc}, sys[2] = {cy - inc, cy};
    bool has = false;
    for (int k = 0; k < 2; ++k) {
        if (sxs[k] < 0 || gw <= sxs[k] || sys[k] < 0 || gh <= sys[k]) continue;
        const int g = vw->cell_base + sys[k] * gw + sxs[k];
        has |= prm.csr_cnt[g] > 0;
    }
    if (prm.view_propagation) has |= prm.csr_cnt[vw->cell_base + cy * gw + cx] > 0;
    if (!has) return;

    const int tstride = prm.wsz;
    unsigned n_cand = 0, n_pref = 0, n_patch = 0, n_f0 = 0, n_f1 = 0, n_ins = 0, n_rep = 0;
    int L_id = -1;
    float L_ncc = 0.0f;
    int L_n = 0;
    {
        const int g = vw->cell_base + cell;
        const csr_off_t fb = prm.csr_start[g];
        L_n = min(prm.csr_cnt[g], MVS_CAPMAX);
        if (wc.lane < L_n) { L_id = pgrid_id(prm, fb + wc.lane); L_ncc = pgrid_ncc(prm, fb + wc.lane); }
    }
    int ns = 0;
    bool gave_up = false;
    const float icx = (float)(prm.csize * (2 * cx + 1) - 1) / 2.0f, icy = (float)(prm.csize * (2 * cy + 1) - 1) / 2.0f;

    const int nsrc = prm.view_propagation ? 3 : 2;
    for (int sidx = 0; sidx < nsrc; ++sidx) {
        const int scx = sidx < 2 ? sxs[sidx] : cx, scy = sidx < 2 ? sys[sidx] : cy;
        if (scx < 0 || gw <= scx || scy < 0 || gh <= scy) continue;
        const int g = vw->cell_base + scy * gw + scx;
        const csr_off_t sb = prm.csr_start[g];
        const int sn = min(prm.csr_cnt[g], MVS_CAPMAX);
        const int as_view = sidx == 2 ? v : -1;
        int E_id = 0;
        bool E_take = false;
        if (wc.lane < sn) { E_id = pgrid_id(prm, sb + wc.lane); E_take = (pgrid_ref(prm, sb + wc.lane) == v) != (sidx == 2); }
        unsigned todo = (unsigned)ballot(E_take);
        while (todo) {
            const int n = __ffs((int)todo) - 1;
            todo &= todo - 1u;
            const DPatch* sp = prm.pool + rli(E_id, n);
            const int srcslot = sidx * prm.cap + n;
            for (int it = 0; it < prm.max_propag; ++it) {
                ST_ADD(7, st_t)
                const int np = L_n;
                const uint32_t k0 = (uint32_t)a.iter, k1 = (uint32_t)v, k2 = (uint32_t)cell, k3 = (uint32_t)(srcslot * 16 + it);
                Cand c;
                int worst = -1;
                float worst_ncc = 0.0f;
                F3 ic;
                if (np < prm.cap) {
                    const float ra = rng_uniform(prm.seed, k0, k1, k2, k3, 0) * (float)prm.csize;
                    const float rb = rng_uniform(prm.seed, k0, k1, k2, k3, 1) * (float)prm.csize;
                    ic = {icx + ra, icy + rb, 1.0f};
                } else {
                    worst = rli(L_id, prm.cap - 1);
                    worst_ncc = rlf(L_ncc, prm.cap - 1);
                    const DPatch* wp = worst >= MVS_NEWBASE ? a.staging + (worst - MVS_NEWBASE) : prm.pool + worst;
                    ic = project(vw, ld4(wp->coord), prm.level);
                }
                {
                    Cand src;
                    load_cand(sp, wc, src);
                    const bool gen_ok = generate_patch(prm, wc, s_scratch, src, ic, c, as_view, np >= prm.cap);
                    ST_ADD(1, st_t)
                    if (!gen_ok) continue;
                }
                ++n_cand;
                if (np >= prm.cap && c.ncc < worst_ncc) { ++n_pref; continue; }
                ++n_patch;
                const int pre_r = pre_process(prm, wc, s_scratch, c);
                ST_ADD(2, st_t)
                if (pre_r == -1) { ++n_f0; continue; }
                float keep_w;
                if constexpr (SIMPLEX) (void)refine_patch_simplex(prm, wc, c, max_evals, xtol, &keep_w);
                else refine_patch(prm, wc, c, k0, k1, k2, k3, &keep_w);
                ST_ADD(3, st_t)
                const int post_r = post_process(prm, wc, s_scratch, s_texs, tstride, c, keep_w, true);
                ST_ADD(4, st_t)
                if (post_r == -1) { ++n_f1; continue; }
                if (prm.depth >= 2 && prm.enable_check) {
                    __syncthreads();
                    if (wc.lane < MVS_CAPMAX) s_scratch[wc.lane] = L_id;
                    __syncthreads();
                    #ifdef MVS_STAGE_TIMING
                    const CheckCtx cx{a.staging, v, cell, L_n, s_scratch, st_acc};
#else
                    const CheckCtx cx{a.staging, v, cell, L_n, s_scratch, nullptr};
#endif
                    const int chk_r = check_patch<BIG>(prm, wc, cx, c, s_texs, a.error_flag, big_table);
                    ST_ADD(5, st_t)
                    if (!BIG && chk_r < 0) { gave_up = true; break; }
                    if (chk_r) { ++n_f1; continue; }
                }
                unsigned long long slot64 = 0;
                if (wc.lane == 0) slot64 = atomicAdd(a.stage_counter, 1ull);
                const int64_t slot = ((int64_t)rfl((int)(slot64 >> 32)) << 32) | (uint32_t)rfl((int)(slot64 & 0xffffffffull));
                if (slot >= a.staging_cap || ns >= a.maxstage) {
                    if (wc.lane == 0) atomicOr(a.error_flag, 1);
                    continue;
                }
                if (np == prm.cap) {
                    if (wc.lane == 0) {
                        if (worst >= MVS_NEWBASE) a.staging[worst - MVS_NEWBASE].flags &= ~1;
                        else a.kill[worst] = 1;
                    }
                    --L_n;
                    ++n_rep;
                } else ++n_ins;
                store_cand(a.staging + slot, wc, c, 1 | (v << 8), cell);
                if (wc.lane == 0) a.job_stage[job * a.maxstage + ns] = (int32_t)slot;
                ++ns;
                const bool lands = ballot(wc.lane < c.nimg && c.img == v && c.gy * gw + c.gx == cell) != 0ull;
                if (lands) {
                    const int nid = MVS_NEWBASE + (int)slot;
                    const int pos = __popcll(ballot(wc.lane < L_n && rank_before(L_ncc, L_id, c.ncc, nid)));
                    const int up_id = __shfl_up(L_id, 1);
                    const float up_ncc = __shfl_up(L_ncc, 1);
                    if (wc.lane > pos) { L_id = up_id; L_ncc = up_ncc; }
                    if (wc.lane == pos) { L_id = nid; L_ncc = c.ncc; }
                    ++L_n;
                }
                ST_ADD(6, st_t)
            }
            if (gave_up) break;
        }
        if (gave_up) break;
    }
    if (!BIG && gave_up) {
        if (wc.lane == 0) { a.job_nstage[job] = 0; a.retry_jobs[atomicAdd(a.nretry, 1)] = (int32_t)job; }
        return;
    }
    if (wc.lane == 0) {
        a.job_nstage[job] = ns;
        DCounters* C = a.counters + (job & (MVS_COUNTER_SLOTS - 1));
        if (n_cand) atomicAdd(&C->candidates, (unsigned long long)n_cand);
        if (n_pref) atomicAdd(&C->prefiltered, (unsigned long long)n_pref);
        if (n_patch) atomicAdd(&C->patches, (unsigned long long)n_patch);
        if (n_f0) atomicAdd(&C->fail0, (unsigned long long)n_f0);
        if (n_f1) atomicAdd(&C->fail1, (unsigned long long)n_f1);
        if (n_ins) atomicAdd(&C->inserted, (unsigned long long)n_ins);
        if (n_rep) atomicAdd(&C->replaced, (unsigned long long)n_rep);
        if (wc.evals) atomicAdd(&C->evals, (unsigned long long)wc.evals);
        if (wc.view_evals) atomicAdd(&C->view_evals, (unsigned long long)wc.view_evals);
#ifdef MVS_STAGE_TIMING
        st_acc[0] = ST_NOW() - st_begin;
        for (int k = 0; k < 12; ++k) if (st_acc[k]) atomicAdd(&C->stage[k], st_acc[k]);
        atomicMax(&C->stage[12], st_acc[12]); atomicMax(&C->stage[13], st_acc[13]);
        atomicAdd(&C->stage[14], wc.st_acc[3]); atomicAdd(&C->stage[15], wc.st_acc[4]);
#endif
    }
}

DEV int64_t sweep_job(const SweepArgs& a) {
    const int64_t bi = blockIdx.x >> 3;
    const int64_t job = a.job_lo + (bi / MVS_XCD_CHUNK) * (8 * MVS_XCD_CHUNK) + (int64_t)(blockIdx.x & 7u) * MVS_XCD_CHUNK + (bi % MVS_XCD_CHUNK);
    return job;
}
__global__ __launch_bounds__(64, MVS_SWEEP_WAVES) void k_sweep(DParams prm, SweepArgs a) {
    __shared__ int s_scratch[192];
    extern __shared__ float s_texs[];
    const int64_t bi = blockIdx.x >> 3;
    const int64_t job = a.job_lo + (bi / MVS_XCD_CHUNK) * (8 * MVS_XCD_CHUNK) + (int64_t)(blockIdx.x & 7u) * MVS_XCD_CHUNK + (bi % MVS_XCD_CHUNK);
    if (job >= a.job_hi) return;
    sweep_cell<false>(prm, a, job, s_scratch, s_texs, nullptr);
}
__global__ __launch_bounds__(64, MVS_SWEEP_WAVES) void k_sweep_simplex(DParams prm, SweepArgs a, int max_evals, float xtol) {
    __shared__ int s_scratch[192];
    extern __shared__ float s_texs[];
    const int64_t job = sweep_job(a);
    if (job >= a.job_hi) return;
    sweep_cell<false, true>(prm, a, job, s_scratch, s_texs, nullptr, max_evals, xtol);
}
__global__ __launch_bounds__(64, 1) void k_sweep_retry(DParams prm, SweepArgs a, int nretry) {
    __shared__ int s_scratch[192];
    extern __shared__ float s_texs[];
    int* big_table = a.big_tables + (size_t)blockIdx.x * MVS_FILTER2_HASH_CAP;
    for (int k = blockIdx.x; k < nretry; k += gridDim.x) {
        __syncthreads();
        sweep_cell<true>(prm, a, (int64_t)a.retry_jobs[k], s_scratch, s_texs, big_table);
    }
}
__global__ __launch_bounds__(64, 1) void k_sweep_retry_simplex(DParams prm, SweepArgs a, int nretry, int max_evals, float xtol) {
    __shared__ int s_scratch[192];
    extern __shared__ float s_texs[];
    int* big_table = a.big_tables + (size_t)blockIdx.x * MVS_FILTER2_HASH_CAP;
    for (int k = blockIdx.x; k < nretry; k += gridDim.x) {
        __syncthreads();
        sweep_cell<true, true>(prm, a, (int64_t)a.retry_jobs[k], s_scratch, s_texs, big_table, max_evals, xtol);
    }
}

__global__ void k_commit_count(SweepArgs a, int32_t* __restrict__ cnt) {
    const int64_t job = (int64_t)blockIdx.x * blockDim.x + threadIdx.x;
    if (job >= a.njobs) return;
    const int ns = a.job_nstage[job];
    int c = 0;
    for (int k = 0; k < ns; ++k) c += a.staging[a.job_stage[job * a.maxstage + k]].flags & 1;
    cnt[job] = c;
}
__global__ void k_commit_copy(SweepArgs a, const int32_t* __restrict__ base, DPatch* __restrict__ dst, int64_t dst_cap, int32_t* __restrict__ per_view,
                              int keep_key) {
    const int64_t job = (int64_t)blockIdx.x * blockDim.x + threadIdx.x;
    if (job >= a.njobs) return;
    const int ns = a.job_nstage[job];
    int r = 0;
    for (int k = 0; k < ns; ++k) {
        const DPatch* sp = a.staging + a.job_stage[job * a.maxstage + k];
        if (!(sp->flags & 1)) continue;
        const int64_t o = (int64_t)base[job] + r++;
        if (o >= dst_cap) { atomicOr(a.error_flag, 2); return; }
        const uint4* s4 = reinterpret_cast<const uint4*>(sp);
        uint4* d4 = reinterpret_cast<uint4*>(dst + o);
        for (int w = 0; w < (int)MVS_REC_U4; ++w) d4[w] = s4[w];
        if (per_view) atomicAdd(&per_view[(sp->flags >> 8) & 0xff], 1);
        if (!keep_key) { dst[o].flags = 1; dst[o].id = 0; }
// ... 184 lines not shown
            get_paxes(prm, prm.views + (vmin == INT_MAX ? 0 : vmin), coord, normal, px, py);
            fpre = make_frame(prm, coord, px, py, normal, image, safe);
        }
    }
    WC_ADD(wc, 1)
    for (int g = 0; g < MVS_FE_PATCHES; ++g) {
        if (!((alive_b >> ((MVS_FE_LANES * g) & 63)) & 1ull)) continue;
        DPatch* p = prm.pool + (first + (int64_t)blockIdx.x * MVS_FE_PATCHES + g);
        const int pflags = p->flags;
        Cand c;
        load_cand(p, wc, c);
        const vmask_t sm = (vmask_t)((safe_b >> ((MVS_FE_LANES * g) & 63)) & (MVS_FE_LANES == 64 ? ~0ull : (1ull << (MVS_FE_LANES & 63)) - 1ull));
        if ((pflags & MVS_FLAG_SETTLED) && (int)vpop(sm) == c.nimg) continue;
        __syncthreads();
        if (wc.lane < MVS_MAXVIEWS) s_scratch[wc.lane] = 0;
        __syncthreads();
        if (wc.lane < c.nimg && ((sm >> wc.lane) & 1u)) s_scratch[c.img] = 1 + MVS_FE_LANES * g + wc.lane;
        __syncthreads();
        const int src1 = s_scratch[wc.lane];
        const bool present = src1 != 0;
        const unsigned long long pm = ballot(present);
        const int pos = __popcll(pm & ((1ull << wc.lane) - 1ull));
        __syncthreads();
        if (present && pos < MVS_LISTCAP) { s_scratch[64 + pos] = wc.lane; s_scratch[128 + pos] = src1 - 1; }
        __syncthreads();
        c.nimg = min((int)__popcll(pm), MVS_LISTCAP);
        c.img = s_scratch[64 + wc.lane];
        if (prm.minImageNum <= c.nimg) {
            Frame f;
            {
                const bool mine = wc.lane < c.nimg;
                const int src = mine ? s_scratch[128 + wc.lane] : MVS_FE_LANES * g;
                f.tlx = __shfl(fpre.tlx, src); f.tly = __shfl(fpre.tly, src);
                f.dxx = __shfl(fpre.dxx, src); f.dxy = __shfl(fpre.dxy, src); f.dyx = __shfl(fpre.dyx, src); f.dyy = __shfl(fpre.dyy, src);
                f.w = __shfl(fpre.w, src); f.ok = __shfl(fpre.ok, src);
                f.img_lo = (unsigned)__shfl((int)fpre.img_lo, src); f.img_hi = (unsigned)__shfl((int)fpre.img_hi, src);
                if (!mine) { f.tlx = f.tly = f.dxx = f.dxy = f.dyx = f.dyy = 0.0f; f.ok = 0; }
            }
            WC_ADD(wc, 7)
            set_ref_image(prm, wc, s_texs, tstride, c, nullptr, &f);
            store_lists(p, wc, c);
            if (wc.lane == 0) p->flags = pflags | MVS_FLAG_SETTLED;
            WC_ADD(wc, 7)
        } else {
            if (wc.lane == 0) kill[first + (int64_t)blockIdx.x * MVS_FE_PATCHES + g] = 1;
        }
    }
    if (wc.lane == 0 && wc.evals) { atomicAdd(evals + 2 * (blockIdx.x & 1023u), (unsigned long long)wc.evals); atomicAdd(evals + 2 * (blockIdx.x & 1023u) + 1, (unsigned long long)wc.view_evals); }
#ifdef MVS_STAGE_TIMING
    if (stage && wc.lane == 0) {
        atomicAdd(stage, (unsigned long long)__builtin_amdgcn_s_memtime() - fe_begin);
        for (int k = 1; k < 8; ++k) atomicAdd(stage + k, wc.st_acc[k]);
    }
#endif
}
template <int HCAP, int RCAP>
__global__ __launch_bounds__(64) void k_filter_neighbor(DParams prm, uint8_t* kill, const int32_t* todo, int32_t ntodo, int32_t* retry, int32_t* nretry,
                                                        int32_t* overflow, unsigned long long* stats , int64_t first) {
    extern __shared__ float s_lds[];
    int* const s_dummy = reinterpret_cast<int*>(s_lds);
    const int64_t id = todo ? (blockIdx.x < (unsigned)ntodo ? todo[blockIdx.x] : -1) : first + (int64_t)blockIdx.x;
    if (id < 0 || id >= prm.pool_n) return;
    const DPatch* p = prm.pool + id;
    if (!(p->flags & 1)) return;
    WaveCtx wc = make_wave_ctx(prm);
#ifdef MVS_STAGE_TIMING
    unsigned long long st_acc[16] = {0, 0, 0, 0, 0, 0, 0, 0, 0, 0, 0, 0, 0, 0, 0, 0};
    const unsigned long long st_begin = CK_NOW();
    auto st_flush = [&]() { st_acc[0] = CK_NOW() - st_begin; if (wc.lane == 0) for (int k = 0; k < 12; ++k) if (st_acc[k]) atomicAdd(stats + 4096 + k, st_acc[k]); };
#endif
    Cand c;
    load_cand(p, wc, c);
    set_grids(prm, wc, c);
#ifdef MVS_STAGE_TIMING
    const CheckCtx cx{prm.pool, -1, -1, 0, s_dummy, st_acc};
    st_acc[1] = CK_NOW() - st_begin;
#else
    const CheckCtx cx{prm.pool, -1, -1, 0, s_dummy, nullptr};
#endif
    int* table = reinterpret_cast<int*>(s_lds);
    unsigned st4[4] = {0u, 0u, 0u, 0u};
    const bool pk = prm.geo != nullptr;
    constexpr bool MK = HCAP == MVS_FILTER_HASH_CAP;
    int* const marks = reinterpret_cast<int*>(s_lds) + MVS_SET_LDS_FLOATS(HCAP, RCAP);
    const int n = pk ? find_neighbors<HCAP, false, true, MK>(prm, wc, cx, c, table, 4.0f, 2, st4, marks) : find_neighbors<HCAP, false, false, MK>(prm, wc, cx, c, table, 4.0f, 2, st4, marks);
    if (n < 0 || n > RCAP) {
        if (wc.lane == 0) {
            if (retry) retry[atomicAdd(nretry, 1)] = (int32_t)id;
            else atomicOr(overflow, 4);
        }
#ifdef MVS_STAGE_TIMING
        st_flush();
#endif
        return;
    }
    if (wc.lane < 4) atomicAdd(stats + 4 * (blockIdx.x & 1023u) + wc.lane, (unsigned long long)(wc.lane == 0 ? st4[0] : wc.lane == 1 ? st4[1] : wc.lane == 2 ? st4[2] : st4[3]));
    const bool reject = n < 6 || (pk ? filter_quad<false, true>(prm, wc, cx, c, table, n, s_lds + rows_offset(n)) : filter_quad<false, false>(prm, wc, cx, c, table, n, s_lds + rows_offset(n))) != 0;
    if (wc.lane == 0 && reject) kill[id] = 1;
#ifdef MVS_STAGE_TIMING
    st_acc[11] = CK_NOW() - st_begin - st_acc[1] - st_acc[9] - st_acc[10];
    st_flush();
#endif
}
DEV int uf_find(int* parent, int a) {
    while (true) {
        const int pa = __atomic_load_n(&parent[a], __ATOMIC_RELAXED);
        if (pa == a) return a;
        const int gp = __atomic_load_n(&parent[pa], __ATOMIC_RELAXED);
        if (gp != pa) __atomic_store_n(&parent[a], gp, __ATOMIC_RELAXED);
        a = pa;
    }
}
DEV void uf_union(int* parent, int a, int b) {
    while (true) {
        a = uf_find(parent, a);
        b = uf_find(parent, b);
        if (a == b) return;
        if (a > b) { const int t = a; a = b; b = t; }
        if (atomicCAS(&parent[b], b, a) == b) return;
    }
}
__global__ void k_groups_init(int* parent, int* size, int64_t n) {
    const int64_t i = (int64_t)blockIdx.x * blockDim.x + threadIdx.x;
    if (i < n) { parent[i] = (int)i; size[i] = 0; }
}
template <int MODE>
__global__ __launch_bounds__(256) void k_groups_edges(DParams prm, int* parent, int2* edges, int* nedges, int cap) {
    const int64_t id = (int64_t)blockIdx.x * 4 + (threadIdx.x >> 6);
    const int lane = (int)(threadIdx.x & 63u);
    if (id >= prm.pool_n) return;
    const DPatch* p = prm.pool + id;
    if (!(p->flags & 1)) return;
    const PGeo me = load_geo(p);
    const DView* vw = prm.views + me.ref;
    unsigned long long listed = 0ull;
    if (MODE == 1) {
        for (int i = 0; i < min(p->nimages, MVS_LISTCAP); ++i) listed |= 1ull << p->images[i];
        for (int i = 0; i < min(p->nvimages, MVS_LISTCAP); ++i) listed |= 1ull << p->vimages[i];
    }
    int gx, gy;
    cell_of(prm, vw, me.coord, gx, gy);
    csr_off_t lstart = 0;
    int ln = 0;
    if (lane < 18) {
        const int kind = lane / 9, yt = gy + (lane % 9) / 3 - 1, xt = gx + lane % 3 - 1;
        if (!(yt < 0 || vw->gh <= yt || xt < 0 || vw->gw <= xt)) {
            const int g = vw->cell_base + yt * vw->gw + xt;
            lstart = kind == 0 ? prm.csr_start[g] : prm.vcsr_start[g];
            ln = kind == 0 ? prm.csr_cnt[g] : prm.vcsr_cnt[g];
        }
    }
    int before = ln;
    for (int d = 1; d < 32; d <<= 1) { const int o = __shfl_up(before, d); if (lane >= d) before += o; }
    const int total = __builtin_amdgcn_readlane(before, 17);
    before -= ln;
    int myroot = -1;
    auto entry_at = [&](int k, int& eid) -> bool {
        int lo = 0;
#pragma unroll
        for (int step = 16; step >= 1; step >>= 1) { const int pc = __shfl(before, lo + step); if (pc <= k) lo += step; }
        const int l_first = __shfl(before, lo);
        const csr_off_t l_start = __shfl(lstart, lo);
        if (k >= total) return false;
        eid = (lo >= 9 ? prm.vcsr_id32 : prm.csr_id32)[l_start + (k - l_first)];
        return true;
    };
    auto edge = [&](const int eid) {
        if (eid == (int)id) return;
        if (MODE != 2 && __atomic_load_n(&parent[eid], __ATOMIC_RELAXED) == __atomic_load_n(&parent[id], __ATOMIC_RELAXED)) return;
        if (!(prm.pool[eid].flags & 1)) return;
        const PGeo q = load_geo(prm.pool + eid);
        if (!is_neighbor(prm, me, q, 1.0f )) return;
        if (MODE == 0) uf_union(parent, (int)id, eid);
        else if (MODE == 1) {
            if (!((listed >> q.ref) & 1ull)) return;
            const DView* qw = prm.views + q.ref;
            int px, py, qx, qy;
            cell_of(prm, qw, me.coord, px, py);
            cell_of(prm, qw, q.coord, qx, qy);
            if (px < 0 || qw->gw <= px || py < 0 || qw->gh <= py) return;
            if (abs(px - qx) <= 1 && abs(py - qy) <= 1) uf_union(parent, (int)id, eid);
        } else {
            if (myroot < 0) myroot = uf_find(parent, (int)id);
            const int rq = uf_find(parent, eid);
            if (rq != myroot) {
                const int k2 = atomicAdd(nedges, 1);
                if (k2 < cap) edges[k2] = make_int2(myroot, rq);
            }
        }
    };
    for (int k0 = 0; k0 < total; k0 += 128) {
        int e0 = -1, e1 = -1;
        const bool h0 = entry_at(k0 + lane, e0), h1 = entry_at(k0 + 64 + lane, e1);
        if (h0) edge(e0);
        if (h1) edge(e1);
    }
}
__global__ void k_groups_count(DParams prm, int* parent, int* size, int sat) {
    const int64_t id = (int64_t)blockIdx.x * blockDim.x + threadIdx.x;
    if (id >= prm.pool_n || !(prm.pool[id].flags & 1)) return;
    const int r = uf_find(parent, (int)id);
    parent[id] = r;
    const int r0 = __builtin_amdgcn_readfirstlane(r);
    const unsigned long long same = __ballot(r == r0);
    if (r == r0) { if ((int)(threadIdx.x & 63u) == __ffsll((long long)same) - 1 && __atomic_load_n(&size[r0], __ATOMIC_RELAXED) < sat) atomicAdd(&size[r0], (int)__popcll(same)); }
    else if (__atomic_load_n(&size[r], __ATOMIC_RELAXED) < sat) atomicAdd(&size[r], 1);
}
__global__ void k_groups_kill(DParams prm, const int* parent, const int* size, int threshold, uint8_t* kill) {
    const int64_t id = (int64_t)blockIdx.x * blockDim.x + threadIdx.x;
    if (id >= prm.pool_n || !(prm.pool[id].flags & 1)) return;
    if (size[parent[id]] < threshold) kill[id] = 1;
}

__global__ __launch_bounds__(64) void k_probe(DParams prm, int op, int64_t n, const DPatch* __restrict__ in, const float* __restrict__ in_f,
                                              DPatch* __restrict__ out, float* __restrict__ out_f, int32_t* __restrict__ out_i) {
    __shared__ int s_scratch[192];
    extern __shared__ float s_texs[];
    const int64_t i = blockIdx.x;
    if (i >= n) return;
    WaveCtx wc = make_wave_ctx(prm);
    const int tstride = prm.wsz;
    if (op == 5) {
        if (wc.lane == 0) {
            const float x = in_f[i];
            out_f[5 * i] = pm_sinf(x); out_f[5 * i + 1] = pm_cosf(x); out_f[5 * i + 2] = pm_asinf(x); out_f[5 * i + 3] = pm_acosf(x);
            out_f[5 * i + 4] = pm_atanf(x);
        }
        return;
    }
    Cand c;
    load_cand(in + i, wc, c);
    if (op == 0) {
        const float ncc = compute_ncc(prm, wc, c.coord, c.normal, c.img, c.nimg);
        if (wc.lane == 0) out_f[i] = ncc;
    } else if (op == 1) {
        const int f = pre_process(prm, wc, s_scratch, c);
        store_cand(out + i, wc, c, 1, (int)i);
        if (wc.lane == 0) out_i[i] = f;
    } else if (op == 2) {
        refine_patch(prm, wc, c, 0u, 0u, (uint32_t)i, 0u);
        store_cand(out + i, wc, c, 1, (int)i);
    } else if (op == 3) {
        int f = post_process(prm, wc, s_scratch, s_texs, tstride, c);
        if (f == 0 && prm.depth >= 2 && prm.enable_check) {
            const CheckCtx cx{in, -1, -1, 0, s_scratch, nullptr};
            const int chk = check_patch(prm, wc, cx, c, s_texs, out_i + n);
            if (chk < 0) { if (wc.lane == 0) atomicOr(out_i + n, 4); }
            else if (chk) f = -1;
        }
        store_cand(out + i, wc, c, 1, (int)i);
        if (wc.lane == 0) out_i[i] = f;
    } else if (op == 4) {
        RefineCtx rc;
        rc.center = c.coord; rc.ref = rli(c.img, 0);
        rc.ray = nrm4(sub4(c.coord, ld4((prm.views + rc.ref)->center)));
        rc.dscale = c.dscale; rc.ascale = prm.ascaleConst;
        float x[3];
        encode(prm, rc, c.coord, c.normal, x);
        double fv[4];
        cost_func4(prm, wc, rc, __shfl(c.img, wc.lane & 15), c.nimg, false, x[0], x[1], x[2], fv);
        if (wc.lane == 0) out_f[i] = (float)fv[0];
    }
}

__global__ __launch_bounds__(64, MVS_SWEEP_WAVES) void k_probe_refine(DParams prm, int64_t n, const DPatch* __restrict__ in, DPatch* __restrict__ out) {
    const int64_t i = blockIdx.x;
    if (i >= n) return;
    WaveCtx wc = make_wave_ctx(prm);
    Cand c;
    load_cand(in + i, wc, c);
    refine_patch(prm, wc, c, 0u, 0u, (uint32_t)i, 0u);
    store_cand(out + i, wc, c, 1, (int)i);
}
__global__ __launch_bounds__(64, MVS_SWEEP_WAVES) void k_probe_refine_simplex(DParams prm, int64_t n, const DPatch* __restrict__ in, DPatch* __restrict__ out,
                                                                              float* __restrict__ out_f, int32_t* __restrict__ out_i, int max_evals, float xtol) {
    const int64_t i = blockIdx.x;
    if (i >= n) return;
    WaveCtx wc = make_wave_ctx(prm);
    Cand c;
    load_cand(in + i, wc, c);
    float x[3];
    double f;
    const int r = refine_patch_simplex(prm, wc, c, max_evals, xtol, nullptr, x, &f);
    store_cand(out + i, wc, c, 1, (int)i);
    if (wc.lane == 0) {
        out_f[4 * i] = x[0]; out_f[4 * i + 1] = x[1]; out_f[4 * i + 2] = x[2]; out_f[4 * i + 3] = (float)f;
        out_i[i] = r;
    }
}

static inline unsigned nblk(int64_t n, int b) { return (unsigned)((n + b - 1) / b); }

void mvsk_rgb_to_rgba(const uint8_t* rgb, uint32_t* out, int64_t n, hipStream_t st) { hipLaunchKernelGGL(k_rgb_to_rgba, dim3(nblk(n, 256)), dim3(256), 0, st, rgb, out, n); }
void mvsk_rgba_to_rgb(const uint32_t* in, uint8_t* rgb, int64_t n, hipStream_t st) { hipLaunchKernelGGL(k_rgba_to_rgb, dim3(nblk(n, 256)), dim3(256), 0, st, in, rgb, n); }
void mvsk_pyr_down(const uint32_t* src, int pw, int ph, uint32_t* dst, int w, int h, hipStream_t st) {
    hipLaunchKernelGGL(k_pyr_down, dim3((w + 63) / 64, (h + 3) / 4), dim3(64, 4), 0, st, src, pw, ph, dst, w, h);
}
void mvsk_mask_down(const uint8_t* src, int pw, int ph, uint8_t* dst, int w, int h, hipStream_t st) {
    hipLaunchKernelGGL(k_mask_down, dim3((w + 63) / 64, (h + 3) / 4), dim3(64, 4), 0, st, src, pw, ph, dst, w, h);
}
void mvsk_mask_binarise(uint8_t* m, int64_t n, hipStream_t st) { hipLaunchKernelGGL(k_mask_binarise, dim3(nblk(n, 256)), dim3(256), 0, st, m, n); }
void mvsk_exclusive_scan(const int32_t* in, int32_t* out, int64_t n, int32_t* tmp, hipStream_t st) { launch_exclusive_scan<int32_t, int32_t>(in, out, n, tmp, st); }
void mvsk_exclusive_scan_off(const int32_t* in, csr_off_t* out, int64_t n, csr_off_t* tmp, hipStream_t st) { launch_exclusive_scan<int32_t, csr_off_t>(in, out, n, tmp, st); }
void mvsk_index_count(const DParams& prm, int32_t* cnt, int32_t* vcnt, unsigned long long* total, hipStream_t st) {
    if (prm.pool_n > 0) hipLaunchKernelGGL(k_index_count, dim3(nblk(prm.pool_n, 256)), dim3(256), 0, st, prm, cnt, vcnt, total);
}
void mvsk_index_fill(const DParams& prm, int vgrid, const csr_off_t* start, int32_t* cursor, unsigned long long* ids, hipStream_t st) {
    if (prm.pool_n > 0) hipLaunchKernelGGL(k_index_fill, dim3(nblk(prm.pool_n, 256)), dim3(256), 0, st, prm, vgrid, start, cursor, ids);
}
void mvsk_index_fill_direct(const DParams& prm, int vgrid, const csr_off_t* start, int32_t* cursor, int32_t* id32, hipStream_t st) {
    if (prm.pool_n > 0) hipLaunchKernelGGL(k_index_fill_direct, dim3(nblk(prm.pool_n, 256)), dim3(256), 0, st, prm, vgrid, start, cursor, id32);
}
void mvsk_index_sort_trim(const DParams& prm, const csr_off_t* start, unsigned long long* ids, int do_trim, unsigned long long* trimmed, hipStream_t st) {
    hipLaunchKernelGGL(k_index_sort_trim, dim3(nblk(prm.total_cells, 256)), dim3(256), 0, st, prm, start, ids, do_trim, trimmed);
}
void mvsk_index_finalize(const DParams& prm, int vgrid, const csr_off_t* start, unsigned long long* ids, int32_t* id32, int32_t* cnt_alive, hipStream_t st) {
    hipLaunchKernelGGL(k_index_finalize, dim3(nblk(prm.total_cells, 256)), dim3(256), 0, st, prm, vgrid, start, ids, id32, cnt_alive);
}
void mvsk_index_pack(const DParams& prm, const csr_off_t* start, const csr_off_t* start2, const int32_t* cnt_alive, const unsigned long long* ids, const int32_t* id32_in,
                     ListKey* key, int32_t* id32_out, hipStream_t st) {
    hipLaunchKernelGGL(k_index_pack, dim3(nblk(prm.total_cells, 256)), dim3(256), 0, st, prm, start, start2, cnt_alive, ids, id32_in, key, id32_out);
}
void mvsk_depth_maps(const DParams& prm, unsigned long long* dp, const uint32_t* dirty, hipStream_t st) {
    if (prm.pool_n > 0) hipLaunchKernelGGL(k_depth_maps, dim3(nblk(prm.pool_n, 64)), dim3(256), 0, st, prm, dp, dirty);
}
void mvsk_depth_mark_dirty(const DParams& prm, const uint8_t* kill, unsigned long long* dp, uint32_t* dirty, hipStream_t st) {
    if (prm.pool_n > 0) hipLaunchKernelGGL(k_depth_mark_dirty, dim3(nblk(prm.pool_n, 64)), dim3(256), 0, st, prm, kill, dp, dirty);
}
void mvsk_best_ncc_map(const DParams& prm, int view, unsigned long long* best, hipStream_t st) {
    if (prm.pool_n > 0) hipLaunchKernelGGL(k_best_ncc_map, dim3(nblk(prm.pool_n, 256)), dim3(256), 0, st, prm, view, best);
}
void mvsk_map_extract(const DParams& prm, int view, int kind, const unsigned long long* sel, float* depth, float* normal, int32_t* ids, int ncells, hipStream_t st) {
    hipLaunchKernelGGL(k_map_extract, dim3(nblk(ncells, 256)), dim3(256), 0, st, prm, view, kind, sel, depth, normal, ids, ncells);
}
void mvsk_fill_ncc(const DParams& prm, unsigned long long* evals, hipStream_t st) {
    if (prm.pool_n > 0) hipLaunchKernelGGL(k_fill_ncc, dim3((unsigned)((prm.pool_n + 63) / 64)), dim3(64), MVS_FRAME_LDS_BYTES, st, prm, evals);
}
size_t mvsk_sweep_lds_bytes(const DParams& prm) {
#if MVS_PAIR_MFMA
    const size_t tex_f = (size_t)MVS_GRAM_CH * 3 * prm.wsz, gram_f = (size_t)prm.gram_ld * prm.gram_ld;
    const size_t texs = MVS_FRAME1_LDS_BYTES + (tex_f > gram_f ? tex_f : gram_f) * sizeof(float);
#else
    const size_t ln = (size_t)prm.list_n;
    const size_t texs = MVS_FRAME1_LDS_BYTES + (ln * 3 * prm.wsz + ln * (ln - 1) / 2) * sizeof(float);
#endif
    const size_t chk = (size_t)MVS_CHECK_LDS_FLOATS * sizeof(float);
    const size_t need = texs > chk ? texs : chk;
    return need > (size_t)MVS_FRAME_LDS_BYTES ? need : (size_t)MVS_FRAME_LDS_BYTES;
}
void mvsk_sweep(const DParams& prm, const SweepArgs& a, const RefineSel& rs, hipStream_t st) {
    const int64_t nloc = a.job_hi - a.job_lo;
    if (nloc <= 0) return;
    static const size_t pad = getenv("MVS_SWEEP_LDS_PAD") ? (size_t)atol(getenv("MVS_SWEEP_LDS_PAD")) : 0;
    const int64_t nblocks = (nloc + 8 * MVS_XCD_CHUNK - 1) / (8 * MVS_XCD_CHUNK) * (8 * MVS_XCD_CHUNK);
    if (rs.simplex) hipLaunchKernelGGL(k_sweep_simplex, dim3((unsigned)nblocks), dim3(64), mvsk_sweep_lds_bytes(prm) + pad, st, prm, a, rs.max_evals, rs.xtol);
    else hipLaunchKernelGGL(k_sweep, dim3((unsigned)nblocks), dim3(64), mvsk_sweep_lds_bytes(prm) + pad, st, prm, a);
}
void mvsk_job_work(const DParams& prm, const SweepArgs& a, int mode, int shift, int32_t* work, hipStream_t st) {
    if (a.njobs > 0) hipLaunchKernelGGL(k_job_work, dim3(nblk(a.njobs, 256)), dim3(256), 0, st, prm, a, mode, shift, work);
}
void mvsk_job_cuts(const int32_t* scan, int64_t njobs, int n, int32_t* cuts, hipStream_t st) {
    if (njobs > 0) hipLaunchKernelGGL(k_job_cuts, dim3(nblk(njobs, 256)), dim3(256), 0, st, scan, njobs, n, cuts);
}
void mvsk_sweep_retry(const DParams& prm, const SweepArgs& a, int nretry, const RefineSel& rs, hipStream_t st) {
    if (nretry <= 0) return;
    const dim3 grid((unsigned)std::min(nretry, MVS_BIG_SLOTS));
    if (rs.simplex) hipLaunchKernelGGL(k_sweep_retry_simplex, grid, dim3(64), mvsk_sweep_lds_bytes(prm), st, prm, a, nretry, rs.max_evals, rs.xtol);
    else hipLaunchKernelGGL(k_sweep_retry, grid, dim3(64), mvsk_sweep_lds_bytes(prm), st, prm, a, nretry);
}
void mvsk_commit_count(const SweepArgs& a, int32_t* cnt, hipStream_t st) { hipLaunchKernelGGL(k_commit_count, dim3(nblk(a.njobs, 256)), dim3(256), 0, st, a, cnt); }
void mvsk_commit_copy(const SweepArgs& a, const int32_t* base, DPatch* dst, int64_t dst_cap, int32_t* per_view, int keep_key, hipStream_t st) {
    hipLaunchKernelGGL(k_commit_copy, dim3(nblk(a.njobs, 256)), dim3(256), 0, st, a, base, dst, dst_cap, per_view, keep_key);
}
void mvsk_kill_count(const uint8_t* kill, int64_t n, int32_t* cnt, hipStream_t st) { if (n > 0) hipLaunchKernelGGL(k_kill_count, dim3(nblk(n, 256)), dim3(256), 0, st, kill, n, cnt); }
void mvsk_kill_export(const uint8_t* kill, int64_t n, const int32_t* base, int32_t* ids, int64_t cap, hipStream_t st) {
    if (n > 0) hipLaunchKernelGGL(k_kill_export, dim3(nblk(n, 256)), dim3(256), 0, st, kill, n, base, ids, cap);
}
void mvsk_apply_kill_flags(DPatch* pool, uint8_t* kill, int64_t n, hipStream_t st) { if (n > 0) hipLaunchKernelGGL(k_apply_kill_flags, dim3(nblk(n, 256)), dim3(256), 0, st, pool, kill, n); }
void mvsk_apply_kill_ids(DPatch* pool, const int32_t* ids, int64_t n, int64_t pool_n, hipStream_t st) {
    if (n > 0) hipLaunchKernelGGL(k_apply_kill_ids, dim3(nblk(n, 256)), dim3(256), 0, st, pool, ids, n, pool_n);
}
void mvsk_append_records(DPatch* pool, int64_t pool_n, const DPatch* recs, int64_t n, hipStream_t st) {
    if (n > 0) hipLaunchKernelGGL(k_append_records, dim3(nblk(n, 256)), dim3(256), 0, st, pool, pool_n, recs, n);
}
void mvsk_alive_count(const DPatch* pool, int64_t n, int32_t* cnt, hipStream_t st) { if (n > 0) hipLaunchKernelGGL(k_alive_count, dim3(nblk(n, 256)), dim3(256), 0, st, pool, n, cnt); }
void mvsk_alive_gather(const DPatch* pool, int64_t n, const int32_t* base, DPatch* out, int64_t cap, hipStream_t st) {
    if (n > 0) hipLaunchKernelGGL(k_alive_gather, dim3(nblk(n, 256)), dim3(256), 0, st, pool, n, base, out, cap);
}
void mvsk_filter_vimages(const DParams& prm, int additive, int64_t first, int64_t last, const uint32_t* dirty, hipStream_t st) {
    if (last <= first) return;
    const int gl = std::max(prm.nviews <= 16 ? 16 : (prm.nviews <= 32 ? 32 : 64), (int)MVS_LISTCAP);
    const unsigned nb = (unsigned)((last - first + 64 / gl - 1) / (64 / gl));
    if (gl == 16) hipLaunchKernelGGL(k_filter_vimages<16>, dim3(nb), dim3(64), 0, st, prm, additive, first, last, dirty);
    else if (gl == 32) hipLaunchKernelGGL(k_filter_vimages<32>, dim3(nb), dim3(64), 0, st, prm, additive, first, last, dirty);
    else hipLaunchKernelGGL(k_filter_vimages<64>, dim3(nb), dim3(64), 0, st, prm, additive, first, last, dirty);
}
void mvsk_geo_pack(const DPatch* pool, int64_t n, float4* geo, uint8_t* ref, int* bad, hipStream_t st) {
    if (n <= 0) return;
    hipLaunchKernelGGL(k_geo_pack, dim3((unsigned)((n + 255) / 256)), dim3(256), 0, st, pool, n, geo, ref, bad);
}
void mvsk_filter_outside(const DParams& prm, uint8_t* kill, int64_t first, int64_t last, hipStream_t st) {
    if (last > first) hipLaunchKernelGGL(k_filter_outside, dim3((unsigned)(last - first)), dim3(64), 0, st, prm, kill, first);
}
size_t mvsk_texs_lds_bytes(const DParams& prm) {
#if MVS_PAIR_MFMA
    const size_t tex_f = (size_t)MVS_GRAM_CH * 3 * prm.wsz, gram_f = (size_t)prm.gram_ld * prm.gram_ld;
    const size_t texs = MVS_FRAME1_LDS_BYTES + (tex_f > gram_f ? tex_f : gram_f) * sizeof(float);
#else
    const size_t ln = (size_t)prm.list_n;
    const size_t texs = MVS_FRAME1_LDS_BYTES + (ln * 3 * prm.wsz + ln * (ln - 1) / 2) * sizeof(float);
#endif
    return texs > (size_t)MVS_FRAME_LDS_BYTES ? texs : (size_t)MVS_FRAME_LDS_BYTES;
}
void mvsk_filter_exact(const DParams& prm, uint8_t* kill, unsigned long long* evals, unsigned long long* stage, int64_t first, int64_t last, hipStream_t st) {
    if (last > first) hipLaunchKernelGGL(k_filter_exact, dim3((unsigned)((last - first + MVS_FE_PATCHES - 1) / MVS_FE_PATCHES)), dim3(64), mvsk_texs_lds_bytes(prm), st, prm, kill, evals, stage, first, last);
}
void mvsk_filter_neighbor(const DParams& prm, uint8_t* kill, int32_t* retry, int32_t* nretry, int32_t* overflow, unsigned long long* stats, int64_t first, int64_t last, hipStream_t st) {
    if (last <= first) return;
    hipLaunchKernelGGL((k_filter_neighbor<MVS_FILTER_HASH_CAP, MVS_FILTER_ROW_CAP>), dim3((unsigned)(last - first)), dim3(64),
                       (size_t)(MVS_SET_LDS_FLOATS(MVS_FILTER_HASH_CAP, MVS_FILTER_ROW_CAP) + 64) * sizeof(float), st, prm, kill, (const int32_t*)nullptr, 0, retry, nretry, overflow, stats, first);
}
void mvsk_filter_neighbor_retry(const DParams& prm, uint8_t* kill, const int32_t* todo, int32_t ntodo, int32_t* overflow, unsigned long long* stats, hipStream_t st) {
    if (ntodo <= 0) return;
    hipLaunchKernelGGL((k_filter_neighbor<MVS_FILTER2_HASH_CAP, MVS_FILTER2_ROW_CAP>), dim3((unsigned)ntodo), dim3(64),
                       (size_t)MVS_SET_LDS_FLOATS(MVS_FILTER2_HASH_CAP, MVS_FILTER2_ROW_CAP) * sizeof(float), st, prm, kill, todo, ntodo, (int32_t*)nullptr, (int32_t*)nullptr, overflow, stats, (int64_t)0);
}
void mvsk_groups(const DParams& prm, int* parent, int* size, int threshold, uint8_t* kill, hipStream_t st) {
    if (prm.pool_n <= 0) return;
    hipLaunchKernelGGL(k_groups_init, dim3(nblk(prm.pool_n, 256)), dim3(256), 0, st, parent, size, prm.pool_n);
    hipLaunchKernelGGL(k_groups_edges<0>, dim3(nblk(prm.pool_n, 4)), dim3(256), 0, st, prm, parent, (int2*)nullptr, (int*)nullptr, 0);
    hipLaunchKernelGGL(k_groups_count, dim3(nblk(prm.pool_n, 256)), dim3(256), 0, st, prm, parent, size, threshold);
    hipLaunchKernelGGL(k_groups_kill, dim3(nblk(prm.pool_n, 256)), dim3(256), 0, st, prm, parent, size, threshold, kill);
}
void mvsk_groups_literal_edges(const DParams& prm, int* parent, int* size, int* edges2, int* nedges, int cap, hipStream_t st) {
    if (prm.pool_n <= 0) return;
    hipLaunchKernelGGL(k_groups_init, dim3(nblk(prm.pool_n, 256)), dim3(256), 0, st, parent, size, prm.pool_n);
    hipLaunchKernelGGL(k_groups_edges<1>, dim3(nblk(prm.pool_n, 4)), dim3(256), 0, st, prm, parent, (int2*)nullptr, (int*)nullptr, 0);
    hipLaunchKernelGGL(k_groups_count, dim3(nblk(prm.pool_n, 256)), dim3(256), 0, st, prm, parent, size, INT_MAX);
    hipLaunchKernelGGL(k_groups_edges<2>, dim3(nblk(prm.pool_n, 4)), dim3(256), 0, st, prm, parent, reinterpret_cast<int2*>(edges2), nedges, cap);
}
__global__ void k_gather_i32(const int32_t* __restrict__ src, const int32_t* __restrict__ idx, int32_t* __restrict__ out, int64_t n) {
    const int64_t i = (int64_t)blockIdx.x * blockDim.x + threadIdx.x;
    if (i < n) out[i] = src[idx[i]];
}
__global__ void k_scatter_i32(int32_t* __restrict__ dst, const int32_t* __restrict__ idx, const int32_t* __restrict__ val, int64_t n) {
    const int64_t i = (int64_t)blockIdx.x * blockDim.x + threadIdx.x;
    if (i < n) dst[idx[i]] = val[i];
}
void mvsk_gather_i32(const int32_t* src, const int32_t* idx, int32_t* out, int64_t n, hipStream_t st) { if (n > 0) hipLaunchKernelGGL(k_gather_i32, dim3(nblk(n, 256)), dim3(256), 0, st, src, idx, out, n); }
void mvsk_scatter_i32(int32_t* dst, const int32_t* idx, const int32_t* val, int64_t n, hipStream_t st) { if (n > 0) hipLaunchKernelGGL(k_scatter_i32, dim3(nblk(n, 256)), dim3(256), 0, st, dst, idx, val, n); }
void mvsk_groups_kill(const DParams& prm, const int* parent, const int* size, int threshold, uint8_t* kill, hipStream_t st) {
    if (prm.pool_n > 0) hipLaunchKernelGGL(k_groups_kill, dim3(nblk(prm.pool_n, 256)), dim3(256), 0, st, prm, parent, size, threshold, kill);
}
void mvsk_probe(const DParams& prm, int op, int64_t n, const DPatch* in, const float* in_f, DPatch* out, float* out_f, int32_t* out_i, const RefineSel& rs,
                hipStream_t st) {
    if (n > 0 && (op == 2 || op == 6) && rs.simplex) {
        hipLaunchKernelGGL(k_probe_refine_simplex, dim3((unsigned)n), dim3(64), MVS_FRAME_LDS_BYTES, st, prm, n, in, out, out_f, out_i, rs.max_evals, rs.xtol);
        return;
    }
    if (n > 0 && op == 2) { hipLaunchKernelGGL(k_probe_refine, dim3((unsigned)n), dim3(64), MVS_FRAME_LDS_BYTES, st, prm, n, in, out); return; }
    if (n > 0) hipLaunchKernelGGL(k_probe, dim3((unsigned)n), dim3(64), mvsk_sweep_lds_bytes(prm), st, prm, op, n, in, in_f, out, out_f, out_i);
}
```

Baseline: 27.89 million.

## Record cell membership and rank at count time to drop index-fill recomputation

The count pass now stores each patch's cell and atomic rank per image, so fill kernels write directly to slots without recomputing cell projections or using cursor atomics. Sort/trim, finalize and pack are restructured to use groups of lanes per cell, an alive bitmask and a separate ref array. fill_ncc now runs over a compacted todo list built during counting, and is launched before the host sync so it overlaps the tot readback. This costs extra memory for the membership array (LISTCAP × pool entries) and adds complexity to NCC bit encoding in keys.

```diff
diff --git a/mvskit_amd/csrc/mvs_engine.cpp b/mvskit_amd/csrc/mvs_engine.cpp
--- a/mvskit_amd/csrc/mvs_engine.cpp
+++ b/mvskit_amd/csrc/mvs_engine.cpp
@@ -62,6 +62,7 @@
 namespace misc {
 constexpr int stage_counter = 0;
 constexpr int fill_evals = 1;
+constexpr int ncc_todo = 3;
 constexpr int neighbor_retry = 4;
 constexpr int sweep_retry = 5;
 constexpr int geo_bad = 6;
@@ -165,10 +166,13 @@
     DevBuf<uint8_t> kill;
     int64_t pool_n = 0;
     bool ncc_dirty = false;
-    DevBuf<int32_t> cnt, cursor, vcnt, vcursor;
+    DevBuf<int32_t> cnt, vcnt;
+    DevBuf<uint32_t> alive_mask;
+    DevBuf<IdxMemb> memb;
+    DevBuf<int32_t> ncc_todo;
     DevBuf<csr_off_t> start, vstart;
     DevBuf<csr_off_t> start_raw;
-    DevBuf<int32_t> id32_raw;
+    DevBuf<int32_t> ref_raw;
     DevBuf<int64_t> scan_tmp;
     DevBuf<unsigned long long> ids;
     DevBuf<ListKey> key;
@@ -317,43 +321,46 @@
 
 bool want_vgrid(const mvs_engine* e) { return e->prm.depth >= 2 && e->prm.enable_check; }
 
-int build_list(mvs_engine* e, bool vgrid, bool trim, bool unordered = false) {
+int build_list(mvs_engine* e, bool vgrid, bool trim, bool unordered = false, bool score = false) {
     hipStream_t st = e->stream;
     const int64_t nc = e->total_cells;
     DParams p = current_params(e);
     DevBuf<int32_t>& cnt = vgrid ? e->vcnt : e->cnt;
     DevBuf<csr_off_t>& start = vgrid ? e->vstart : e->start;
-    DevBuf<int32_t>& cursor = vgrid ? e->vcursor : e->cursor;
     DevBuf<unsigned long long>& ids = e->ids;
     DevBuf<int32_t>& id32 = vgrid ? e->vid32 : e->id32;
     DevBuf<int32_t>& cnt_alive = vgrid ? e->vcnt_alive : e->cnt_alive;
     HIPCHK(hipMemsetAsync(cnt.p, 0, (size_t)(nc + 1) * sizeof(int32_t), st));
-    mvsk_index_count(p, vgrid ? nullptr : cnt.p, vgrid ? cnt.p : nullptr, nullptr, st);
+    e->memb.headroom = true;
+    if (int r = e->memb.ensure((int64_t)MVS_LISTCAP * e->pool_n)) return r;
+    if (score) { if (int r = e->ncc_todo.ensure(e->pool_n + 2)) return r; }
+    int32_t* const todo_n = reinterpret_cast<int32_t*>(e->misc.p + misc::ncc_todo);
+    mvsk_index_count(p, vgrid ? 1 : 0, cnt.p, e->memb.p, score ? e->ncc_todo.p : nullptr, score ? todo_n : nullptr, st);
     const bool direct = unordered && !trim;
     DevBuf<csr_off_t>& raw = e->start_raw;
     csr_off_t* const first_scan = direct ? start.p : raw.p;
     mvsk_exclusive_scan_off(cnt.p, first_scan, nc, reinterpret_cast<csr_off_t*>(e->scan_tmp.p), st);
     csr_off_t tot64 = 0;
     HIPCHK(hipMemcpyAsync(&tot64, first_scan + nc, sizeof tot64, hipMemcpyDeviceToHost, st));
+    if (score) mvsk_fill_ncc(p, e->ncc_todo.p, todo_n, e->misc.p + misc::fill_evals, st);
     HIPCHK(hipStreamSynchronize(st));
     const int64_t tot = (int64_t)tot64;
     if (!unordered) { if (int r = ids.ensure(tot + 16)) return r; }
     if (!vgrid && !unordered) { if (int r = e->key.ensure(tot + 16)) return r; }
     if (int r = id32.ensure(tot + 16)) return r;
     p = current_params(e);
-    HIPCHK(hipMemsetAsync(cursor.p, 0, (size_t)(nc + 1) * sizeof(int32_t), st));
     if (direct) {
-        mvsk_index_fill_direct(p, vgrid ? 1 : 0, start.p, cursor.p, id32.p, st);
+        mvsk_index_fill_direct(p, vgrid ? 1 : 0, start.p, e->memb.p, id32.p, st);
         cnt.swap(cnt_alive);
         e->lists_dense[vgrid ? 1 : 0] = true;
         return MVS_OK;
     }
-    if (int r = e->id32_raw.ensure(tot + 16)) return r;
-    mvsk_index_fill(p, vgrid ? 1 : 0, raw.p, cursor.p, ids.p, st);
-    mvsk_index_sort_trim(p, raw.p, ids.p, trim ? 1 : 0, e->misc.p + misc::trim_parts, st);
-    mvsk_index_finalize(p, vgrid ? 1 : 0, raw.p, ids.p, e->id32_raw.p, cnt_alive.p, st);
+    if (int r = e->ref_raw.ensure(tot + 16)) return r;
+    mvsk_index_fill(p, vgrid ? 1 : 0, raw.p, e->memb.p, ids.p, e->ref_raw.p, st);
+    mvsk_index_sort_trim(p, raw.p, ids.p, e->ref_raw.p, trim ? 1 : 0, e->misc.p + misc::trim_parts, st);
+    mvsk_index_finalize(p, raw.p, ids.p, trim ? 1 : 0, cnt_alive.p, e->alive_mask.p, st);
     mvsk_exclusive_scan_off(cnt_alive.p, start.p, nc, reinterpret_cast<csr_off_t*>(e->scan_tmp.p), st);
-    mvsk_index_pack(p, raw.p, start.p, cnt_alive.p, ids.p, e->id32_raw.p, vgrid ? nullptr : e->key.p, id32.p, st);
+    mvsk_index_pack(p, raw.p, start.p, trim ? 1 : 0, e->alive_mask.p, ids.p, e->ref_raw.p, vgrid ? nullptr : e->key.p, id32.p, st);
     e->lists_dense[vgrid ? 1 : 0] = true;
     return MVS_OK;
 }
@@ -365,12 +372,10 @@
 }
 int build_index(mvs_engine* e, unsigned long long* trimmed_out) {
     hipStream_t st = e->stream;
-    const DParams p = current_params(e);
-    HIPCHK(hipMemsetAsync(e->misc.p + misc::fill_evals, 0, 2 * sizeof(unsigned long long), st));
+    HIPCHK(hipMemsetAsync(e->misc.p + misc::fill_evals, 0, 3 * sizeof(unsigned long long), st));
     HIPCHK(hipMemsetAsync(e->misc.p + misc::trim_parts, 0, misc::trim_nparts * sizeof(unsigned long long), st));
-    mvsk_fill_ncc(p, e->misc.p + misc::fill_evals, st);
     e->ncc_dirty = false;
-    if (int r = build_list(e, false, true)) return r;
+    if (int r = build_list(e, false, true, false, true)) return r;
     if (want_vgrid(e)) if (int r = build_list(e, true, false, true)) return r;
     if (int r = build_depth(e)) return r;
     if (trimmed_out) {
@@ -785,8 +790,8 @@
     if (int r = e->dviews.ensure(nviews)) return r;
     HIPCHK(hipMemcpyAsync(e->dviews.p, e->hviews.data(), sizeof(DView) * nviews, hipMemcpyHostToDevice, st));
     const int64_t nc = e->total_cells;
-    if (e->cnt.ensure(nc + 2) || e->start.ensure(nc + 2) || e->cursor.ensure(nc + 2) || e->vcnt.ensure(nc + 2) || e->vstart.ensure(nc + 2) ||
-        e->vcursor.ensure(nc + 2) || e->start_raw.ensure(nc + 2) || e->dpgrid.ensure(nc + 2) || e->best.ensure(nc + 2) || e->cnt_alive.ensure(nc + 2) || e->vcnt_alive.ensure(nc + 2))
+    if (e->cnt.ensure(nc + 2) || e->start.ensure(nc + 2) || e->alive_mask.ensure(nc + 2) || e->vcnt.ensure(nc + 2) || e->vstart.ensure(nc + 2) ||
+        e->start_raw.ensure(nc + 2) || e->dpgrid.ensure(nc + 2) || e->best.ensure(nc + 2) || e->cnt_alive.ensure(nc + 2) || e->vcnt_alive.ensure(nc + 2))
         return MVS_ERR_HIP;
     int64_t pool_cap = e->cfg.max_patches > 0 ? e->cfg.max_patches : 4 * nc;
     if (e->cfg.max_patches <= 0) {
@@ -798,9 +803,11 @@
             if (fit < pool_cap) pool_cap = std::max<int64_t>(fit, std::min<int64_t>(pool_cap, nc / 4 + 1024));
         }
     }
-    e->ids.headroom = e->key.headroom = e->id32.headroom = e->id32_raw.headroom = e->vid32.headroom = true;
+    e->ids.headroom = e->key.headroom = e->id32.headroom = e->ref_raw.headroom = e->vid32.headroom = true;
     e->geo.headroom = e->geo_ref.headroom = true;
-    if (e->pool.ensure(pool_cap) || e->pool_alt.ensure(pool_cap) || e->kill.ensure(pool_cap) || e->kill_cnt.ensure(pool_cap + 2) || e->kill_base.ensure(pool_cap + 2)) return MVS_ERR_HIP;
+    if (e->pool.ensure(pool_cap) || e->pool_alt.ensure(pool_cap) || e->kill.ensure(pool_cap) || e->kill_cnt.ensure(pool_cap + 2) || e->kill_base.ensure(pool_cap + 2) ||
+        e->ncc_todo.ensure(pool_cap + 2))
+        return MVS_ERR_HIP;
     HIPCHK(hipMemsetAsync(e->kill.p, 0, (size_t)pool_cap, st));
     int64_t njobs_max = 0;
     for (int v = 0; v < nviews; ++v) njobs_max += (int64_t)((e->hviews[v].gw + 1) / 2) * e->hviews[v].gh;
@@ -985,7 +992,9 @@
         if (buf.cap != before && hipMemsetAsync(buf.p, 0, (size_t)buf.cap * sizeof(*buf.p), e->stream) != hipSuccess) { (void)hipGetLastError(); return MVS_ERR_HIP; }
         return MVS_OK;
     };
-    if (take(e->ids, n + 16) || take(e->key, n + 16) || take(e->id32, n + 16) || take(e->id32_raw, n + 16) || take(e->vid32, n + 16)) return MVS_ERR_HIP;
+    if (take(e->ids, n + 16) || take(e->key, n + 16) || take(e->id32, n + 16) || take(e->ref_raw, n + 16) || take(e->vid32, n + 16)) return MVS_ERR_HIP;
+    e->memb.headroom = true;
+    if (take(e->memb, (int64_t)MVS_LISTCAP * std::min<int64_t>(n, e->pool.cap))) return MVS_ERR_HIP;
     HIPCHK(hipStreamSynchronize(e->stream));
     return MVS_OK;
 }
diff --git a/mvskit_amd/csrc/mvs_kernels.h b/mvskit_amd/csrc/mvs_kernels.h
--- a/mvskit_amd/csrc/mvs_kernels.h
+++ b/mvskit_amd/csrc/mvs_kernels.h
@@ -8,19 +8,20 @@
 void mvsk_mask_down(const uint8_t* src, int pw, int ph, uint8_t* dst, int w, int h, hipStream_t st);
 void mvsk_mask_binarise(uint8_t* m, int64_t n, hipStream_t st);
 void mvsk_exclusive_scan(const int32_t* in, int32_t* out, int64_t n, int32_t* tmp, hipStream_t st);
-void mvsk_index_count(const DParams& prm, int32_t* cnt, int32_t* vcnt, unsigned long long* total, hipStream_t st);
+struct IdxMemb { int32_t g, rank; };
+void mvsk_index_count(const DParams& prm, int vgrid, int32_t* cnt, IdxMemb* memb, int32_t* todo, int32_t* todo_n, hipStream_t st);
 void mvsk_exclusive_scan_off(const int32_t* in, csr_off_t* out, int64_t n, csr_off_t* tmp, hipStream_t st);
-void mvsk_index_fill(const DParams& prm, int vgrid, const csr_off_t* start, int32_t* cursor, unsigned long long* ids, hipStream_t st);
-void mvsk_index_fill_direct(const DParams& prm, int vgrid, const csr_off_t* start, int32_t* cursor, int32_t* id32, hipStream_t st);
-void mvsk_index_sort_trim(const DParams& prm, const csr_off_t* start, unsigned long long* ids, int do_trim, unsigned long long* trimmed, hipStream_t st);
-void mvsk_index_finalize(const DParams& prm, int vgrid, const csr_off_t* start, unsigned long long* ids, int32_t* id32, int32_t* cnt_alive, hipStream_t st);
-void mvsk_index_pack(const DParams& prm, const csr_off_t* start, const csr_off_t* start2, const int32_t* cnt_alive, const unsigned long long* ids, const int32_t* id32_in,
-                     ListKey* key, int32_t* id32_out, hipStream_t st);
+void mvsk_index_fill(const DParams& prm, int vgrid, const csr_off_t* start, const IdxMemb* memb, unsigned long long* ids, int32_t* ref, hipStream_t st);
+void mvsk_index_fill_direct(const DParams& prm, int vgrid, const csr_off_t* start, const IdxMemb* memb, int32_t* id32, hipStream_t st);
+void mvsk_index_sort_trim(const DParams& prm, const csr_off_t* start, unsigned long long* ids, int32_t* ref, int do_trim, unsigned long long* trimmed, hipStream_t st);
+void mvsk_index_finalize(const DParams& prm, const csr_off_t* start, const unsigned long long* ids, int do_trim, int32_t* cnt_alive, uint32_t* alive_mask, hipStream_t st);
+void mvsk_index_pack(const DParams& prm, const csr_off_t* start, const csr_off_t* start2, int do_trim, const uint32_t* alive_mask, const unsigned long long* ids,
+                     const int32_t* ref, ListKey* key, int32_t* id32_out, hipStream_t st);
 void mvsk_depth_maps(const DParams& prm, unsigned long long* dp, const uint32_t* dirty, hipStream_t st);
 void mvsk_depth_mark_dirty(const DParams& prm, const uint8_t* kill, unsigned long long* dp, uint32_t* dirty, hipStream_t st);
 void mvsk_best_ncc_map(const DParams& prm, int view, unsigned long long* best, hipStream_t st);
 void mvsk_map_extract(const DParams& prm, int view, int kind, const unsigned long long* sel, float* depth, float* normal, int32_t* ids, int ncells, hipStream_t st);
-void mvsk_fill_ncc(const DParams& prm, unsigned long long* evals, hipStream_t st);
+void mvsk_fill_ncc(const DParams& prm, const int32_t* todo, const int32_t* todo_n, unsigned long long* evals, hipStream_t st);
 struct RefineSel { int simplex; int max_evals; float xtol; };
 size_t mvsk_sweep_lds_bytes(const DParams& prm);
 void mvsk_sweep(const DParams& prm, const SweepArgs& a, const RefineSel& rs, hipStream_t st);
diff --git a/mvskit_amd/csrc/mvs_kernels.hip b/mvskit_amd/csrc/mvs_kernels.hip
--- a/mvskit_amd/csrc/mvs_kernels.hip
+++ b/mvskit_amd/csrc/mvs_kernels.hip
@@ -104,125 +104,173 @@
 DEV int pgrid_ref(const DParams& prm, csr_off_t pos) {
     return prm.csr_key[pos].ref;
 }
-__global__ void k_index_count(DParams prm, int32_t* __restrict__ cnt, int32_t* __restrict__ vcnt, unsigned long long* __restrict__ total) {
+__global__ void k_index_count(DParams prm, int vgrid, int32_t* __restrict__ cnt, IdxMemb* __restrict__ memb, int32_t* __restrict__ todo,
+                              int32_t* __restrict__ todo_n) {
     const int64_t id = (int64_t)blockIdx.x * blockDim.x + threadIdx.x;
-    int mine = 0;
+    bool need = false;
     if (id < prm.pool_n && (prm.pool[id].flags & 1)) {
         const DPatch* p = prm.pool + id;
         const F4 coord = ld4(p->coord);
-        const int n = cnt ? min(p->nimages, MVS_LISTCAP) : 0;
+        need = p->ncc < 0.0f;
+        const int n = vgrid ? min(p->nvimages, MVS_LISTCAP) : min(p->nimages, MVS_LISTCAP);
         for (int i = 0; i < n; ++i) {
-            const DView* vw = prm.views + p->images[i];
+            const DView* vw = prm.views + (vgrid ? p->vimages[i] : p->images[i]);
             int ix, iy;
             cell_of(prm, vw, coord, ix, iy);
-            if (ix < 0 || vw->gw <= ix || iy < 0 || vw->gh <= iy) continue;
-            atomicAdd(&cnt[vw->cell_base + iy * vw->gw + ix], 1);
-            ++mine;
-        }
-        if (vcnt) {
-            const int nv = min(p->nvimages, MVS_LISTCAP);
-            for (int i = 0; i < nv; ++i) {
-                const DView* vw = prm.views + p->vimages[i];
-                int ix, iy;
-                cell_of(prm, vw, coord, ix, iy);
-                if (ix < 0 || vw->gw <= ix || iy < 0 || vw->gh <= iy) continue;
-                atomicAdd(&vcnt[vw->cell_base + iy * vw->gw + ix], 1);
-                ++mine;
+            IdxMemb m;
+            m.g = -1; m.rank = 0;
+            if (!(ix < 0 || vw->gw <= ix || iy < 0 || vw->gh <= iy)) {
+                m.g = vw->cell_base + iy * vw->gw + ix;
+                m.rank = atomicAdd(&cnt[m.g], 1);
             }
-        }
-    }
-    for (int d = 32; d >= 1; d >>= 1) mine += __shfl_xor(mine, d);
-    if (total && (threadIdx.x & 63) == 0 && mine) atomicAdd(total, (unsigned long long)mine);
-}
-__global__ void k_index_fill(DParams prm, int vgrid, const csr_off_t* __restrict__ start, int32_t* __restrict__ cursor, unsigned long long* __restrict__ ids) {
+            memb[(int64_t)i * prm.pool_n + id] = m;
+        }
+    }
+    if (todo) {
+        const unsigned long long m = ballot(need);
+        if (m) {
+            const int lane = lane_id(), leader = __ffsll((long long)m) - 1;
+            int base = 0;
+            if (lane == leader) base = atomicAdd(todo_n, __popcll(m));
+            base = __shfl(base, leader);
+            if (need) todo[base + __popcll(m & ((1ull << lane) - 1ull))] = (int32_t)id;
+        }
+    }
+}
+DEV uint32_t key_ncc_bits(unsigned long long key) {
+    const uint32_t s = ~(uint32_t)(key >> 32);
+    return (s & 0x80000000u) ? (s & 0x7fffffffu) : ~s;
+}
+__global__ void k_index_fill(DParams prm, int vgrid, const csr_off_t* __restrict__ start, const IdxMemb* __restrict__ memb,
+                             unsigned long long* __restrict__ ids, int32_t* __restrict__ ref) {
     const int64_t id = (int64_t)blockIdx.x * blockDim.x + threadIdx.x;
     if (id >= prm.pool_n) return;
     const DPatch* p = prm.pool + id;
     if (!(p->flags & 1)) return;
-    const F4 coord = ld4(p->coord);
-    const unsigned long long key = list_key(p->ncc, id);
+    const float ncc = p->ncc;
+    const unsigned long long key = list_key(ncc, id);
+    const int32_t rw = (int32_t)((uint32_t)p->images[0] | (key_ncc_bits(key) == __float_as_uint(ncc) ? 0u : 0x80000000u));
     const int n = vgrid ? min(p->nvimages, MVS_LISTCAP) : min(p->nimages, MVS_LISTCAP);
     for (int i = 0; i < n; ++i) {
-        const DView* vw = prm.views + (vgrid ? p->vimages[i] : p->images[i]);
-        int ix, iy;
-        cell_of(prm, vw, coord, ix, iy);
-        if (ix < 0 || vw->gw <= ix || iy < 0 || vw->gh <= iy) continue;
-        const int g = vw->cell_base + iy * vw->gw + ix;
-        ids[start[g] + atomicAdd(&cursor[g], 1)] = key;
-    }
-}
-__global__ void k_index_fill_direct(DParams prm, int vgrid, const csr_off_t* __restrict__ start, int32_t* __restrict__ cursor, int32_t* __restrict__ id32) {
+        const IdxMemb m = memb[(int64_t)i * prm.pool_n + id];
+        if (m.g < 0) continue;
+        const csr_off_t slot = start[m.g] + m.rank;
+        ids[slot] = key;
+        ref[slot] = rw;
+    }
+}
+__global__ void k_index_fill_direct(DParams prm, int vgrid, const csr_off_t* __restrict__ start, const IdxMemb* __restrict__ memb, int32_t* __restrict__ id32) {
     const int64_t id = (int64_t)blockIdx.x * blockDim.x + threadIdx.x;
     if (id >= prm.pool_n) return;
     const DPatch* p = prm.pool + id;
     if (!(p->flags & 1)) return;
-    const F4 coord = ld4(p->coord);
     const int n = vgrid ? min(p->nvimages, MVS_LISTCAP) : min(p->nimages, MVS_LISTCAP);
     for (int i = 0; i < n; ++i) {
-        const DView* vw = prm.views + (vgrid ? p->vimages[i] : p->images[i]);
-        int ix, iy;
-        cell_of(prm, vw, coord, ix, iy);
-        if (ix < 0 || vw->gw <= ix || iy < 0 || vw->gh <= iy) continue;
-        const int g = vw->cell_base + iy * vw->gw + ix;
-        const csr_off_t slot = start[g] + atomicAdd(&cursor[g], 1);
-        id32[slot] = (int32_t)id;
-    }
-}
-__global__ void k_index_sort_trim(DParams prm, const csr_off_t* __restrict__ start, unsigned long long* __restrict__ ids, int do_trim,
-                                  unsigned long long* __restrict__ trimmed) {
-    const int g = blockIdx.x * blockDim.x + threadIdx.x;
+        const IdxMemb m = memb[(int64_t)i * prm.pool_n + id];
+        if (m.g < 0) continue;
+        id32[start[m.g] + m.rank] = (int32_t)id;
+    }
+}
+#define MVS_IDX_GROUP 8
+#define MVS_IDX_CELLS (256 / MVS_IDX_GROUP)
+__global__ __launch_bounds__(256) void k_index_sort_trim(DParams prm, const csr_off_t* __restrict__ start, unsigned long long* __restrict__ ids,
+                                                         int32_t* __restrict__ ref, int do_trim, unsigned long long* __restrict__ trimmed) {
+    __shared__ unsigned long long s_key[MVS_IDX_CELLS][MVS_CAPMAX];
+    __shared__ int32_t s_ref[MVS_IDX_CELLS][MVS_CAPMAX];
+    const int grp = (int)threadIdx.x / MVS_IDX_GROUP, gl = (int)threadIdx.x % MVS_IDX_GROUP;
+    const int64_t g = (int64_t)blockIdx.x * MVS_IDX_CELLS + grp;
     const bool in = g < prm.total_cells;
     const csr_off_t b = in ? start[g] : 0, e = in ? start[g + 1] : 0;
-    for (csr_off_t i = b + 1; i < e; ++i) {
-        const unsigned long long k = ids[i];
-        csr_off_t j = i - 1;
-        while (j >= b) {
-            const unsigned long long o = ids[j];
-            if (o < k) break;
-            ids[j + 1] = o;
-            --j;
-        }
-        ids[j + 1] = k;
+    const int n = (int)(e - b);
+    const int lim = do_trim ? min(prm.cap, MVS_CAPMAX) : MVS_CAPMAX;
+    const bool counting = n > 1 && (do_trim || n <= MVS_CAPMAX);
+    int mine = 0;
+    if (counting) {
+        for (int i = gl; i < n; i += MVS_IDX_GROUP) {
+            const unsigned long long k = ids[b + i];
+            const int32_t r = ref[b + i];
+            int rank = 0;
+            for (int j = 0; j < n; ++j) {
+                const unsigned long long o = ids[b + j];
+                rank += (o < k || (o == k && j < i)) ? 1 : 0;
+            }
+            if (rank < lim) { s_key[grp][rank] = k; s_ref[grp][rank] = r; }
+            else {
+                const int old = atomicAnd(&prm.pool[(uint32_t)k].flags, ~1);
+                mine += old & 1;
+            }
+        }
+    } else if (n > 1 && gl == 0) {
+        for (csr_off_t i = b + 1; i < e; ++i) {
+            const unsigned long long k = ids[i];
+            const int32_t r = ref[i];
+            csr_off_t j = i - 1;
+            while (j >= b) {
+                const unsigned long long o = ids[j];
+                if (o < k) break;
+                ids[j + 1] = o; ref[j + 1] = ref[j];
+                --j;
+            }
+            ids[j + 1] = k; ref[j + 1] = r;
+        }
+    }
+    __syncthreads();
+    if (counting) {
+        const int m = min(n, lim);
+        for (int k = gl; k < m; k += MVS_IDX_GROUP) { ids[b + k] = s_key[grp][k]; ref[b + k] = s_ref[grp][k]; }
     }
     if (do_trim) {
-        int mine = 0;
-        for (csr_off_t k = b + prm.cap; k < e; ++k) {
-            const int old = atomicAnd(&prm.pool[(uint32_t)ids[k]].flags, ~1);
-            mine += old & 1;
-        }
         for (int d = 32; d >= 1; d >>= 1) mine += __shfl_xor(mine, d);
         if ((threadIdx.x & 63) == 0 && mine) atomicAdd(trimmed + (blockIdx.x & 255u), (unsigned long long)mine);
     }
 }
-__global__ void k_index_finalize(DParams prm, int vgrid, const csr_off_t* __restrict__ start, unsigned long long* __restrict__ ids,
-                                 int32_t* __restrict__ id32, int32_t* __restrict__ cnt_alive) {
-    const int g = blockIdx.x * blockDim.x + threadIdx.x;
-    if (g >= prm.total_cells) return;
-    const csr_off_t b = start[g], e = start[g + 1];
-    int n = 0;
-    for (csr_off_t k = b; k < e; ++k) {
-        const int id = (int)(uint32_t)ids[k];
-        const DPatch* p = prm.pool + id;
-        if (!(p->flags & 1)) continue;
-        if (!vgrid) ids[b + n] = ((unsigned long long)(uint32_t)p->images[0] << 32) | (unsigned long long)__float_as_uint(p->ncc);
-        id32[b + n] = id;
-        ++n;
-    }
-    cnt_alive[g] = n;
-}
-__global__ void k_index_pack(DParams prm, const csr_off_t* __restrict__ start, const csr_off_t* __restrict__ start2, const int32_t* __restrict__ cnt_alive,
-                             const unsigned long long* __restrict__ ids, const int32_t* __restrict__ id32_in, ListKey* __restrict__ key, int32_t* __restrict__ id32_out) {
-    const int g = blockIdx.x * blockDim.x + threadIdx.x;
+__global__ __launch_bounds__(256) void k_index_finalize(DParams prm, const csr_off_t* __restrict__ start, const unsigned long long* __restrict__ ids,
+                                                        int do_trim, int32_t* __restrict__ cnt_alive, uint32_t* __restrict__ alive_mask) {
+    const int grp = (int)threadIdx.x / MVS_IDX_GROUP, gl = (int)threadIdx.x % MVS_IDX_GROUP;
+    const int64_t g = (int64_t)blockIdx.x * MVS_IDX_CELLS + grp;
+    const bool in = g < prm.total_cells;
+    const csr_off_t b = in ? start[g] : 0, e = in ? start[g + 1] : 0;
+    const int n = (int)(e - b);
+    if (!do_trim) {
+        if (in && gl == 0) cnt_alive[g] = n;
+        return;
+    }
+    const int m = min(n, min(prm.cap, MVS_CAPMAX));
+    const int sh = (lane_id() / MVS_IDX_GROUP) * MVS_IDX_GROUP;
+    uint32_t mask = 0;
+    for (int t = 0; t < MVS_CAPMAX / MVS_IDX_GROUP; ++t) {
+        const int k = t * MVS_IDX_GROUP + gl;
+        bool alive = false;
+        if (k < m) alive = (prm.pool[(uint32_t)ids[b + k]].flags & 1) != 0;
+        mask |= (uint32_t)((ballot(alive) >> sh) & ((1ull << MVS_IDX_GROUP) - 1ull)) << (t * MVS_IDX_GROUP);
+    }
+    if (in && gl == 0) { alive_mask[g] = mask; cnt_alive[g] = __popc(mask); }
+}
+__global__ __launch_bounds__(256) void k_index_pack(DParams prm, const csr_off_t* __restrict__ start, const csr_off_t* __restrict__ start2, int do_trim,
+                                                    const uint32_t* __restrict__ alive_mask, const unsigned long long* __restrict__ ids,
+                                                    const int32_t* __restrict__ ref, ListKey* __restrict__ key, int32_t* __restrict__ id32_out) {
+    const int gl = (int)threadIdx.x % MVS_IDX_GROUP;
+    const int64_t g = (int64_t)blockIdx.x * MVS_IDX_CELLS + (int)threadIdx.x / MVS_IDX_GROUP;
     if (g >= prm.total_cells) return;
     const csr_off_t b = start[g], b2 = start2[g];
-    const int n = cnt_alive[g];
-    for (int k = 0; k < n; ++k) {
-        id32_out[b2 + k] = id32_in[b + k];
+    const int n = (int)(start[g + 1] - b);
+    const uint32_t mask = do_trim ? alive_mask[g] : 0u;
+    const int m = do_trim ? min(n, MVS_CAPMAX) : n;
+    for (int k = gl; k < m; k += MVS_IDX_GROUP) {
+        int pos = k;
+        if (do_trim) {
+            if (!((mask >> k) & 1u)) continue;
+            pos = __popc(mask & ((1u << k) - 1u));
+        }
+        const unsigned long long w = ids[b + k];
+        const uint32_t id = (uint32_t)w;
+        id32_out[b2 + pos] = (int32_t)id;
         if (key) {
-            const unsigned long long w = ids[b + k];
+            const int32_t r = ref[b + k];
             ListKey lk;
-            lk.ncc = __uint_as_float((uint32_t)w); lk.ref = (int32_t)(w >> 32);
-            key[b2 + k] = lk;
+            lk.ncc = r < 0 ? prm.pool[id].ncc : __uint_as_float(key_ncc_bits(w));
+            lk.ref = r & 0x7fffffff;
+            key[b2 + pos] = lk;
         }
     }
 }
@@ -303,16 +351,12 @@
     ids[c] = (int32_t)id;
 }
 
-__global__ __launch_bounds__(64) void k_fill_ncc(DParams prm, unsigned long long* evals) {
+__global__ __launch_bounds__(64) void k_fill_ncc(DParams prm, const int32_t* __restrict__ todo, const int32_t* __restrict__ todo_n, unsigned long long* evals) {
+    const int n = *todo_n;
+    if ((int)blockIdx.x >= n) return;
     WaveCtx wc = make_wave_ctx(prm);
-    const int64_t mine = (int64_t)blockIdx.x * 64 + wc.lane;
-    bool need = false;
-    if (mine < prm.pool_n) need = (prm.pool[mine].flags & 1) && (prm.pool[mine].ncc < 0.0f);
-    unsigned long long todo = ballot(need);
-    while (todo) {
-        const int l = __ffsll((long long)todo) - 1;
-        todo &= todo - 1ull;
-        DPatch* p = prm.pool + ((int64_t)blockIdx.x * 64 + l);
+    for (int k = (int)blockIdx.x; k < n; k += (int)gridDim.x) {
+        DPatch* p = prm.pool + todo[k];
         Cand c;
         load_cand(p, wc, c);
         const float ncc = compute_ncc(prm, wc, c.coord, c.normal, c.img, c.nimg);
@@ -1103,24 +1147,24 @@
 void mvsk_mask_binarise(uint8_t* m, int64_t n, hipStream_t st) { hipLaunchKernelGGL(k_mask_binarise, dim3(nblk(n, 256)), dim3(256), 0, st, m, n); }
 void mvsk_exclusive_scan(const int32_t* in, int32_t* out, int64_t n, int32_t* tmp, hipStream_t st) { launch_exclusive_scan<int32_t, int32_t>(in, out, n, tmp, st); }
 void mvsk_exclusive_scan_off(const int32_t* in, csr_off_t* out, int64_t n, csr_off_t* tmp, hipStream_t st) { launch_exclusive_scan<int32_t, csr_off_t>(in, out, n, tmp, st); }
-void mvsk_index_count(const DParams& prm, int32_t* cnt, int32_t* vcnt, unsigned long long* total, hipStream_t st) {
-    if (prm.pool_n > 0) hipLaunchKernelGGL(k_index_count, dim3(nblk(prm.pool_n, 256)), dim3(256), 0, st, prm, cnt, vcnt, total);
-}
-void mvsk_index_fill(const DParams& prm, int vgrid, const csr_off_t* start, int32_t* cursor, unsigned long long* ids, hipStream_t st) {
-    if (prm.pool_n > 0) hipLaunchKernelGGL(k_index_fill, dim3(nblk(prm.pool_n, 256)), dim3(256), 0, st, prm, vgrid, start, cursor, ids);
-}
-void mvsk_index_fill_direct(const DParams& prm, int vgrid, const csr_off_t* start, int32_t* cursor, int32_t* id32, hipStream_t st) {
-    if (prm.pool_n > 0) hipLaunchKernelGGL(k_index_fill_direct, dim3(nblk(prm.pool_n, 256)), dim3(256), 0, st, prm, vgrid, start, cursor, id32);
-}
-void mvsk_index_sort_trim(const DParams& prm, const csr_off_t* start, unsigned long long* ids, int do_trim, unsigned long long* trimmed, hipStream_t st) {
-    hipLaunchKernelGGL(k_index_sort_trim, dim3(nblk(prm.total_cells, 256)), dim3(256), 0, st, prm, start, ids, do_trim, trimmed);
-}
-void mvsk_index_finalize(const DParams& prm, int vgrid, const csr_off_t* start, unsigned long long* ids, int32_t* id32, int32_t* cnt_alive, hipStream_t st) {
-    hipLaunchKernelGGL(k_index_finalize, dim3(nblk(prm.total_cells, 256)), dim3(256), 0, st, prm, vgrid, start, ids, id32, cnt_alive);
-}
-void mvsk_index_pack(const DParams& prm, const csr_off_t* start, const csr_off_t* start2, const int32_t* cnt_alive, const unsigned long long* ids, const int32_t* id32_in,
-                     ListKey* key, int32_t* id32_out, hipStream_t st) {
-    hipLaunchKernelGGL(k_index_pack, dim3(nblk(prm.total_cells, 256)), dim3(256), 0, st, prm, start, start2, cnt_alive, ids, id32_in, key, id32_out);
+void mvsk_index_count(const DParams& prm, int vgrid, int32_t* cnt, IdxMemb* memb, int32_t* todo, int32_t* todo_n, hipStream_t st) {
+    if (prm.pool_n > 0) hipLaunchKernelGGL(k_index_count, dim3(nblk(prm.pool_n, 256)), dim3(256), 0, st, prm, vgrid, cnt, memb, todo, todo_n);
+}
+void mvsk_index_fill(const DParams& prm, int vgrid, const csr_off_t* start, const IdxMemb* memb, unsigned long long* ids, int32_t* ref, hipStream_t st) {
+    if (prm.pool_n > 0) hipLaunchKernelGGL(k_index_fill, dim3(nblk(prm.pool_n, 256)), dim3(256), 0, st, prm, vgrid, start, memb, ids, ref);
+}
+void mvsk_index_fill_direct(const DParams& prm, int vgrid, const csr_off_t* start, const IdxMemb* memb, int32_t* id32, hipStream_t st) {
+    if (prm.pool_n > 0) hipLaunchKernelGGL(k_index_fill_direct, dim3(nblk(prm.pool_n, 256)), dim3(256), 0, st, prm, vgrid, start, memb, id32);
+}
+void mvsk_index_sort_trim(const DParams& prm, const csr_off_t* start, unsigned long long* ids, int32_t* ref, int do_trim, unsigned long long* trimmed, hipStream_t st) {
+    hipLaunchKernelGGL(k_index_sort_trim, dim3(nblk(prm.total_cells, MVS_IDX_CELLS)), dim3(256), 0, st, prm, start, ids, ref, do_trim, trimmed);
+}
+void mvsk_index_finalize(const DParams& prm, const csr_off_t* start, const unsigned long long* ids, int do_trim, int32_t* cnt_alive, uint32_t* alive_mask, hipStream_t st) {
+    hipLaunchKernelGGL(k_index_finalize, dim3(nblk(prm.total_cells, MVS_IDX_CELLS)), dim3(256), 0, st, prm, start, ids, do_trim, cnt_alive, alive_mask);
+}
+void mvsk_index_pack(const DParams& prm, const csr_off_t* start, const csr_off_t* start2, int do_trim, const uint32_t* alive_mask, const unsigned long long* ids,
+                     const int32_t* ref, ListKey* key, int32_t* id32_out, hipStream_t st) {
+    hipLaunchKernelGGL(k_index_pack, dim3(nblk(prm.total_cells, MVS_IDX_CELLS)), dim3(256), 0, st, prm, start, start2, do_trim, alive_mask, ids, ref, key, id32_out);
 }
 void mvsk_depth_maps(const DParams& prm, unsigned long long* dp, const uint32_t* dirty, hipStream_t st) {
     if (prm.pool_n > 0) hipLaunchKernelGGL(k_depth_maps, dim3(nblk(prm.pool_n, 64)), dim3(256), 0, st, prm, dp, dirty);
@@ -1134,8 +1178,9 @@
 void mvsk_map_extract(const DParams& prm, int view, int kind, const unsigned long long* sel, float* depth, float* normal, int32_t* ids, int ncells, hipStream_t st) {
     hipLaunchKernelGGL(k_map_extract, dim3(nblk(ncells, 256)), dim3(256), 0, st, prm, view, kind, sel, depth, normal, ids, ncells);
 }
-void mvsk_fill_ncc(const DParams& prm, unsigned long long* evals, hipStream_t st) {
-    if (prm.pool_n > 0) hipLaunchKernelGGL(k_fill_ncc, dim3((unsigned)((prm.pool_n + 63) / 64)), dim3(64), MVS_FRAME_LDS_BYTES, st, prm, evals);
+void mvsk_fill_ncc(const DParams& prm, const int32_t* todo, const int32_t* todo_n, unsigned long long* evals, hipStream_t st) {
+    const int64_t blocks = std::min<int64_t>(std::max<int64_t>(prm.pool_n / 16, 1), 16384);
+    if (prm.pool_n > 0) hipLaunchKernelGGL(k_fill_ncc, dim3((unsigned)blocks), dim3(64), MVS_FRAME_LDS_BYTES, st, prm, todo, todo_n, evals);
 }
 size_t mvsk_sweep_lds_bytes(const DParams& prm) {
 #if MVS_PAIR_MFMA
```

New measurement: 28.14 million (median of 6 runs). About the same (+0.9%).
